# zserge/grayskull

Measured on AMD Instinct MI355X. Metric: Mpix/s (and % HBM roofline) for gs_sobel+gs_blur on 4K uint8, 1/2/4/8 GPU, higher is better.
Workload: dtype u8; 1 GPU; configs[1]: gs_blur(r=2) -> gs_sobel -> gs_otsu_threshold -> gs_threshold, 3840x2160 uint8, 512 frames on this GPU resident in HBM (512 in the job, weak scaling); frames_per_gpu=512, global_frames=512, chain_algorithmic_bytes_per_px_unfused=7

## Files before the change

grayskull_amd/__init__.py:

```python
import ctypes as C
import os

import numpy as np

from ._abi import (BLOB_DTYPE, CONTOUR_DTYPE, GsImage, GsLbpCascade, GsPoint, GsRect, KEYPOINT_DTYPE, MATCH_DTYPE, POINT_DTYPE,
                   RECT_DTYPE)
from .cascade import Cascade

_HERE = os.path.dirname(os.path.abspath(__file__))
HIP_LIBRARY = os.path.join(_HERE, "libgrayskull_hip.so")

__all__ = ["Grayskull", "Cascade", "lib", "BLOB_DTYPE", "CONTOUR_DTYPE", "KEYPOINT_DTYPE", "MATCH_DTYPE", "POINT_DTYPE", "RECT_DTYPE"]


def _ptr(a):
    if a is None:
        return None
    if isinstance(a, np.ndarray):
        if not a.flags["C_CONTIGUOUS"]:
            raise ValueError("array must be C-contiguous")
        return a.ctypes.data
    if hasattr(a, "data_ptr"):
        if not a.is_contiguous():
            raise ValueError("tensor must be contiguous")
        return a.data_ptr()
    if isinstance(a, int):
        return a
    raise TypeError("expected numpy array, torch tensor or raw address, got %r" % type(a))


def _img(a):
    if a.ndim != 2:
        raise ValueError("expected a 2-D (h, w) uint8 image")
    return GsImage(int(a.shape[1]), int(a.shape[0]), _ptr(a))


_SIGS = {
    "gs_blur": (None, [GsImage, GsImage, C.c_uint]),
    "gs_sobel": (None, [GsImage, GsImage]),
    "gs_erode": (None, [GsImage, GsImage]),
    "gs_dilate": (None, [GsImage, GsImage]),
    "gs_histogram": (None, [GsImage, C.c_void_p]),
    "gs_otsu_threshold": (C.c_uint8, [GsImage]),
    "gs_threshold": (None, [GsImage, C.c_uint8]),
    "gs_integral": (None, [GsImage, C.c_void_p]),
    "gs_lbp_window": (C.c_uint, [C.c_void_p, C.c_void_p, C.c_uint, C.c_uint, C.c_int, C.c_int,
                                 C.c_float]),
    "gs_lbp_detect": (C.c_uint, [C.c_void_p, C.c_void_p, C.c_uint, C.c_uint, C.c_void_p, C.c_uint,
                                 C.c_float, C.c_float, C.c_float, C.c_int]),
    "gs_fast": (C.c_uint, [GsImage, GsImage, C.c_void_p, C.c_uint, C.c_uint]),
    "gs_compute_orientation": (C.c_float, [GsImage, C.c_uint, C.c_uint, C.c_uint]),
    "gs_brief_descriptor": (None, [GsImage, C.c_void_p]),
    "gs_orb_extract": (C.c_uint, [GsImage, C.c_void_p, C.c_uint, C.c_uint, C.c_void_p]),
    "gs_match_orb": (C.c_uint, [C.c_void_p, C.c_uint, C.c_void_p, C.c_uint, C.c_void_p, C.c_uint,
                                C.c_float]),
    "gs_compute_orientation_nostdlib": (C.c_float, [GsImage, C.c_uint, C.c_uint, C.c_uint]),
    "gs_brief_descriptor_nostdlib": (None, [GsImage, C.c_void_p]),
    "gs_orb_extract_nostdlib": (C.c_uint, [GsImage, C.c_void_p, C.c_uint, C.c_uint, C.c_void_p]),
    "gs_adaptive_threshold": (None, [GsImage, GsImage, C.c_uint, C.c_int]),
    "gs_filter": (None, [GsImage, GsImage, GsImage, C.c_uint]),
    "gs_downsample": (None, [GsImage, GsImage]),
    "gs_crop": (None, [GsImage, GsImage, GsRect]),
    "gs_copy": (None, [GsImage, GsImage]),
    "gs_resize_nn": (None, [GsImage, GsImage]),
    "gs_resize": (None, [GsImage, GsImage]),
    "gs_match_template": (None, [GsImage, GsImage, GsImage]),
    "gs_find_best_match": (GsPoint, [GsImage]),
    "gs_blobs": (C.c_uint, [GsImage, C.c_void_p, C.c_void_p, C.c_uint]),
    "gs_blob_corners": (None, [GsImage, C.c_void_p, C.c_void_p, C.c_void_p]),
    "gs_trace_contour": (None, [GsImage, GsImage, C.c_void_p]),
    "gs_perspective_correct": (None, [GsImage, GsImage, C.c_void_p]),
    "gsh_version": (C.c_char_p, []),
    "gsh_device_count": (C.c_int, []),
    "gsh_set_device": (None, [C.c_int]),
    "gsh_set_stream": (None, [C.c_void_p]),
    "gsh_get_stream": (C.c_void_p, []),
    "gsh_set_async": (None, [C.c_int]),
    "gsh_sync": (None, []),
    "gsh_tune": (None, [C.c_int, C.c_int]),
    "gsh_profile": (None, [C.c_int]),
    "gsh_profile_read": (C.c_uint, [C.POINTER(C.c_double)]),
    "gsh_fast_score_batch": (None, [C.c_void_p, C.c_void_p, C.c_uint, C.c_uint, C.c_uint, C.c_uint]),
    "gsh_shutdown": (None, []),
    "gsh_malloc": (C.c_void_p, [C.c_size_t]),
    "gsh_free": (None, [C.c_void_p]),
    "gsh_host_alloc": (C.c_void_p, [C.c_size_t]),
    "gsh_host_free": (None, [C.c_void_p]),
    "gsh_memset": (None, [C.c_void_p, C.c_int, C.c_size_t]),
    "gsh_upload": (None, [C.c_void_p, C.c_void_p, C.c_size_t]),
    "gsh_download": (None, [C.c_void_p, C.c_void_p, C.c_size_t]),
    "gsh_is_device_ptr": (C.c_int, [C.c_void_p]),
    "gsh_blur_batch": (None, [C.c_void_p, C.c_void_p, C.c_uint, C.c_uint, C.c_uint, C.c_uint]),
    "gsh_sobel_batch": (None, [C.c_void_p, C.c_void_p, C.c_uint, C.c_uint, C.c_uint]),
    "gsh_erode_batch": (None, [C.c_void_p, C.c_void_p, C.c_uint, C.c_uint, C.c_uint]),
    "gsh_dilate_batch": (None, [C.c_void_p, C.c_void_p, C.c_uint, C.c_uint, C.c_uint]),
    "gsh_morph_batch": (None, [C.c_void_p, C.c_void_p, C.c_void_p, C.c_uint, C.c_uint, C.c_uint, C.c_int, C.c_uint]),
    "gsh_histogram_batch": (None, [C.c_void_p, C.c_uint, C.c_uint, C.c_uint, C.c_void_p]),
    "gsh_otsu_batch": (None, [C.c_void_p, C.c_uint, C.c_uint, C.c_uint, C.c_void_p, C.c_void_p]),
    "gsh_threshold_batch": (None, [C.c_void_p, C.c_uint, C.c_uint, C.c_uint, C.c_uint8]),
    "gsh_threshold_batch_dev": (None, [C.c_void_p, C.c_uint, C.c_uint, C.c_uint, C.c_void_p]),
    "gsh_blur_sobel_batch": (None, [C.c_void_p, C.c_void_p, C.c_uint, C.c_uint, C.c_uint, C.c_uint]),
    "gsh_edge_pipeline_batch": (None, [C.c_void_p, C.c_void_p, C.c_void_p, C.c_uint, C.c_uint,
                                       C.c_uint, C.c_uint, C.c_void_p, C.c_void_p]),
    "gsh_integral_batch": (None, [C.c_void_p, C.c_uint, C.c_uint, C.c_uint, C.c_void_p]),
    "gsh_cascade_create": (C.c_void_p, [C.c_void_p]),
    "gsh_cascade_destroy": (None, [C.c_void_p]),
    "gsh_lbp_detect_batch": (None, [C.c_void_p, C.c_void_p, C.c_uint, C.c_uint, C.c_uint,
                                    C.c_void_p, C.c_void_p, C.c_uint, C.c_float, C.c_float,
                                    C.c_float, C.c_int]),
    "gsh_lbp_count_evaluated": (None, [C.c_void_p]),
    "gsh_lbp_window_count": (C.c_uint64, [C.c_void_p, C.c_uint, C.c_uint, C.c_float, C.c_float,
                                          C.c_float, C.c_int]),
    "gsh_fast_batch": (None, [C.c_void_p, C.c_void_p, C.c_uint, C.c_uint, C.c_uint, C.c_void_p,
                              C.c_void_p, C.c_uint, C.c_uint]),
    "gsh_orb_extract": (C.c_uint, [C.c_void_p, C.c_uint, C.c_uint, C.c_void_p, C.c_void_p,
                                   C.c_uint, C.c_uint]),
    "gsh_orb_extract_batch": (None, [C.c_void_p, C.c_uint, C.c_uint, C.c_uint, C.c_void_p, C.c_void_p, C.c_void_p,
                                     C.c_uint, C.c_uint]),
    "gsh_orb_extract_batch_nostdlib": (None, [C.c_void_p, C.c_uint, C.c_uint, C.c_uint, C.c_void_p, C.c_void_p, C.c_void_p,
                                              C.c_uint, C.c_uint]),
    "gsh_orb_pyramid_buffer_bytes": (C.c_size_t, [C.c_uint, C.c_uint, C.c_uint]),
    "gsh_orb_extract_pyramid": (C.c_uint, [C.c_void_p, C.c_uint, C.c_uint, C.c_void_p, C.c_void_p,
                                           C.c_uint, C.c_uint, C.c_uint]),
    "gsh_match_orb_dev": (None, [C.c_void_p, C.c_uint, C.c_void_p, C.c_uint, C.c_void_p,
                                 C.c_void_p, C.c_uint, C.c_float]),
    "gsh_adaptive_threshold_batch": (None, [C.c_void_p, C.c_void_p, C.c_uint, C.c_uint, C.c_uint,
                                            C.c_uint, C.c_int]),
    "gsh_filter_batch": (None, [C.c_void_p, C.c_void_p, C.c_uint, C.c_uint, C.c_uint, C.c_void_p,
                                C.c_uint, C.c_uint, C.c_uint]),
    "gsh_downsample_batch": (None, [C.c_void_p, C.c_void_p, C.c_uint, C.c_uint, C.c_uint]),
    "gsh_crop_batch": (None, [C.c_void_p, C.c_void_p, C.c_uint, C.c_uint, C.c_uint, GsRect]),
    "gsh_resize_batch": (None, [C.c_void_p, C.c_uint, C.c_uint, C.c_void_p, C.c_uint, C.c_uint, C.c_uint]),
    "gsh_resize_nn_batch": (None, [C.c_void_p, C.c_uint, C.c_uint, C.c_void_p, C.c_uint, C.c_uint, C.c_uint]),
    "gsh_crop_resize_batch": (None, [C.c_void_p, C.c_uint, C.c_uint, C.c_void_p, C.c_uint, C.c_uint, C.c_uint, C.c_void_p,
                                      C.c_void_p, C.c_uint, C.c_int]),
    "gsh_match_template_batch": (None, [C.c_void_p, C.c_uint, C.c_uint, C.c_uint, C.c_void_p, C.c_uint, C.c_uint, C.c_uint,
                                         C.c_void_p]),
    "gsh_find_best_match_batch": (None, [C.c_void_p, C.c_uint, C.c_uint, C.c_uint, C.c_void_p, C.c_void_p]),
    "gsh_locate_template_batch": (None, [C.c_void_p, C.c_uint, C.c_uint, C.c_uint, C.c_void_p, C.c_uint, C.c_uint, C.c_uint,
                                          C.c_void_p, C.c_void_p]),
    "gsh_blobs_batch": (None, [C.c_void_p, C.c_uint, C.c_uint, C.c_uint, C.c_void_p, C.c_void_p, C.c_void_p,
                                C.c_uint]),
    "gsh_blob_corners_batch": (None, [C.c_void_p, C.c_void_p, C.c_uint, C.c_uint, C.c_uint, C.c_void_p,
                                       C.c_void_p]),
    "gsh_perspective_correct_batch": (None, [C.c_void_p, C.c_uint, C.c_uint, C.c_void_p, C.c_uint, C.c_uint,
                                              C.c_uint, C.c_void_p]),
    "gsh_blob_largest_batch": (None, [C.c_void_p, C.c_uint, C.c_void_p, C.c_uint, C.c_void_p, C.c_void_p]),
    "gsh_blob_paint_batch": (None, [C.c_void_p, C.c_void_p, C.c_uint, C.c_uint, C.c_uint, C.c_void_p, C.c_uint,
                                    C.c_void_p]),
    "gsh_threshold_batch_dev_offset": (None, [C.c_void_p, C.c_uint, C.c_uint, C.c_uint, C.c_void_p, C.c_int]),
    "gsh_trace_contours_batch": (None, [C.c_void_p, C.c_void_p, C.c_uint, C.c_uint, C.c_uint, C.c_void_p, C.c_uint,
                                         C.c_void_p, C.c_void_p]),
    "gsh_blob_contour_starts_batch": (None, [C.c_void_p, C.c_uint, C.c_uint, C.c_uint, C.c_void_p, C.c_uint,
                                              C.c_void_p, C.c_void_p]),
    "gsh_synth_batch": (None, [C.c_void_p, C.c_uint, C.c_uint, C.c_uint, C.c_uint32]),
    "gsh_checksum_batch": (None, [C.c_void_p, C.c_size_t, C.c_uint, C.c_void_p]),
    "gsh_comm_init_all": (C.c_int, [C.POINTER(C.c_void_p), C.c_int, C.POINTER(C.c_int)]),
    "gsh_comm_destroy_all": (None, [C.POINTER(C.c_void_p), C.c_int]),
    "gsh_comm_rank": (C.c_int, [C.c_void_p]),
    "gsh_comm_world": (C.c_int, [C.c_void_p]),
    "gsh_comm_backend": (C.c_char_p, [C.c_void_p]),
    "gsh_comm_broadcast": (None, [C.c_void_p, C.c_void_p, C.c_size_t, C.c_int]),
    "gsh_comm_all_gather": (None, [C.c_void_p, C.c_void_p, C.c_void_p, C.c_size_t]),
    "gsh_comm_all_reduce_u64": (None, [C.c_void_p, C.c_void_p, C.c_size_t, C.c_int]),
    "gsh_comm_all_reduce_f64": (None, [C.c_void_p, C.c_void_p, C.c_size_t, C.c_int]),
}
EXPORTED_SYMBOLS = tuple(sorted(_SIGS))
_EXPERIMENT_SIGS = {
    "gsh_probe_strip_copy": (None, [C.c_void_p, C.c_void_p, C.c_uint, C.c_uint, C.c_uint]),
}


def _share_torch_hip_runtime():
    import importlib.util
    import sys
    if "torch" in sys.modules:
        return
    try:
        spec = importlib.util.find_spec("torch")
    except (ImportError, ValueError):
        spec = None
    if not spec or not spec.origin:
        return
    libdir = os.path.join(os.path.dirname(spec.origin), "lib")
    for name in ("libhsa-runtime64.so", "libamdhip64.so"):
        f = os.path.join(libdir, name)
        if os.path.exists(f):
            try:
                C.CDLL(f, mode=C.RTLD_GLOBAL)
            except OSError:
                return


class Grayskull:

    def __init__(self, path=None):
        path = path or HIP_LIBRARY
        if not os.path.exists(path):
            raise ImportError(
                "%s not found: build it with `python -c 'import __graft_entry__ as g; g.build()'` "
                "(hipcc --offload-arch=gfx950). grayskull_amd has no CPU fallback." % path)
        self.path = path
        if os.path.abspath(path) == os.path.abspath(HIP_LIBRARY):
            _share_torch_hip_runtime()
        self.c = C.CDLL(path)
        for name, (res, args) in _SIGS.items():
            f = getattr(self.c, name)
            f.restype, f.argtypes = res, args
        for name, (res, args) in _EXPERIMENT_SIGS.items():
            if hasattr(self.c, name):
                f = getattr(self.c, name)
                f.restype, f.argtypes = res, args

    def version(self):
        return self.c.gsh_version().decode()

    def device_count(self):
        return int(self.c.gsh_device_count())

    def set_device(self, i):
        self.c.gsh_set_device(int(i))

    def use_torch_stream(self):
        import torch
        self.c.gsh_set_stream(C.c_void_p(torch.cuda.current_stream().cuda_stream))

    def set_stream(self, handle):
        self.c.gsh_set_stream(C.c_void_p(handle))

    def set_async(self, on):
        self.c.gsh_set_async(1 if on else 0)

    def shutdown(self):
        self.c.gsh_shutdown()

    def sync(self):
        self.c.gsh_sync()

    def tune(self, key, value):
        self.c.gsh_tune(int(key), int(value))

    def profile(self, on):
        self.c.gsh_profile(int(on))

    def profile_read(self):
        ms = C.c_double(0.0)
        n = self.c.gsh_profile_read(C.byref(ms))
        return int(n), float(ms.value)

    def fast_score_batch(self, score, img, threshold):
        n, h, w = self._nhw(img)
        self.c.gsh_fast_score_batch(_ptr(score), _ptr(img), w, h, n, threshold)

    probe_fast_score = fast_score_batch

    @property
    def experiment(self):
        return hasattr(self.c, "gsh_probe_strip_copy")

    def probe_strip_copy(self, dst, src):
        n, h, w = self._nhw(src)
        self.c.gsh_probe_strip_copy(_ptr(dst), _ptr(src), w, h, n)

    def blur(self, dst, src, radius):
        self.c.gs_blur(_img(dst), _img(src), radius)

    def sobel(self, dst, src):
        self.c.gs_sobel(_img(dst), _img(src))

    def erode(self, dst, src):
        self.c.gs_erode(_img(dst), _img(src))

    def dilate(self, dst, src):
        self.c.gs_dilate(_img(dst), _img(src))

    def histogram(self, img):
        hist = np.zeros(256, np.uint32)
        self.c.gs_histogram(_img(img), hist.ctypes.data)
        return hist

    def otsu_threshold(self, img):
        return int(self.c.gs_otsu_threshold(_img(img)))

    def threshold(self, img, t):
        self.c.gs_threshold(_img(img), t)

    def adaptive_threshold(self, dst, src, radius, c):
        self.c.gs_adaptive_threshold(_img(dst), _img(src), radius, c)

    def filter(self, dst, src, kernel, norm):
        k = np.ascontiguousarray(kernel).astype(np.int8).view(np.uint8)
        self.c.gs_filter(_img(dst), _img(src), _img(k), norm)

    def downsample(self, dst, src):
        self.c.gs_downsample(_img(dst), _img(src))

    def crop(self, dst, src, x, y, w, h):
        self.c.gs_crop(_img(dst), _img(src), GsRect(x, y, w, h))

    def copy(self, dst, src):
        self.c.gs_copy(_img(dst), _img(src))

    def resize(self, dst, src, nearest=False):
        (self.c.gs_resize_nn if nearest else self.c.gs_resize)(_img(dst), _img(src))

    def match_template(self, img, tmpl, result):
        self.c.gs_match_template(_img(img), _img(tmpl), _img(result))

    def find_best_match(self, result):
        p = self.c.gs_find_best_match(_img(result))
        return int(p.x), int(p.y)

    def blobs(self, img, nblobs, labels=None):
        if labels is None:
            labels = np.zeros(img.shape, np.uint16)
        recs = np.zeros(max(nblobs, 1), BLOB_DTYPE)
        m = self.c.gs_blobs(_img(img), _ptr(labels), recs.ctypes.data, nblobs)
        return recs[:m].copy(), labels

    def blob_corners(self, img, labels, blob):
        b = np.ascontiguousarray(np.asarray(blob, BLOB_DTYPE).reshape(1))
        c = np.zeros(4, POINT_DTYPE)
        self.c.gs_blob_corners(_img(img), _ptr(labels), b.ctypes.data, c.ctypes.data)
        return [(int(p["x"]), int(p["y"])) for p in c]

    def perspective_correct(self, dst, src, corners):
        c = np.ascontiguousarray(np.asarray(corners, np.uint32).reshape(4, 2))
        self.c.gs_perspective_correct(_img(dst), _img(src), c.ctypes.data)

    def trace_contour(self, img, visited, start):
        c = np.zeros(1, CONTOUR_DTYPE)
        c["sx"], c["sy"] = int(start[0]) & 0xFFFFFFFF, int(start[1]) & 0xFFFFFFFF
        self.c.gs_trace_contour(_img(img), _img(visited), c.ctypes.data)
        return c[0]

    def integral(self, src, ii=None):
        if ii is None:
            ii = np.zeros(src.shape, np.uint32)
        self.c.gs_integral(_img(src), _ptr(ii))
        return ii

    def lbp_window(self, cascade, ii, x, y, scale):
        ih, iw = ii.shape
        return int(self.c.gs_lbp_window(C.addressof(cascade.as_struct()), _ptr(ii), iw, ih, x, y,
                                        scale))

    def lbp_detect(self, cascade, ii, max_rects, scale_factor, min_scale, max_scale, step):
        ih, iw = ii.shape
        rects = np.zeros(max(max_rects, 1), RECT_DTYPE)
        n = self.c.gs_lbp_detect(C.addressof(cascade.as_struct()), _ptr(ii), iw, ih,
                                 rects.ctypes.data, max_rects, scale_factor, min_scale, max_scale,
                                 step)
        return rects[:n].copy()

    def fast(self, img, scoremap, nkps, threshold):
        kps = np.zeros(max(nkps, 1), KEYPOINT_DTYPE)
        n = self.c.gs_fast(_img(img), _img(scoremap), kps.ctypes.data, nkps, threshold)
        return kps[:n].copy()

    def compute_orientation(self, img, x, y, r=15):
        return float(self.c.gs_compute_orientation(_img(img), x, y, r))

    def brief_descriptor(self, img, x, y, angle):
        kp = np.zeros(1, KEYPOINT_DTYPE)
        kp["x"], kp["y"], kp["angle"] = x, y, angle
        self.c.gs_brief_descriptor(_img(img), kp.ctypes.data)
        return kp["desc"][0].copy()

    def orb_extract(self, img, nkps, threshold, scoremap):
        kps = np.zeros(max(nkps, 1), KEYPOINT_DTYPE)
        n = self.c.gs_orb_extract(_img(img), kps.ctypes.data, nkps, threshold, _ptr(scoremap))
        return kps[:n].copy()

    def compute_orientation_nostdlib(self, img, x, y, r=15):
        return float(self.c.gs_compute_orientation_nostdlib(_img(img), x, y, r))

    def brief_descriptor_nostdlib(self, img, x, y, angle):
        kp = np.zeros(1, KEYPOINT_DTYPE)
        kp["x"], kp["y"], kp["angle"] = x, y, angle
        self.c.gs_brief_descriptor_nostdlib(_img(img), kp.ctypes.data)
        return kp["desc"][0].copy()

    def orb_extract_nostdlib(self, img, nkps, threshold, scoremap):
        kps = np.zeros(max(nkps, 1), KEYPOINT_DTYPE)
        n = self.c.gs_orb_extract_nostdlib(_img(img), kps.ctypes.data, nkps, threshold, _ptr(scoremap))
        return kps[:n].copy()

    def match_orb(self, k1, k2, max_matches, max_distance):
        k1 = np.ascontiguousarray(k1, KEYPOINT_DTYPE)
        k2 = np.ascontiguousarray(k2, KEYPOINT_DTYPE)
        out = np.zeros(max(max_matches, 1), MATCH_DTYPE)
        n = self.c.gs_match_orb(k1.ctypes.data, len(k1), k2.ctypes.data, len(k2), out.ctypes.data,
                                max_matches, max_distance)
        return out[:n].copy()

    @staticmethod
    def _nhw(a):
        if a.ndim != 3:
            raise ValueError("expected (n, h, w)")
        return int(a.shape[0]), int(a.shape[1]), int(a.shape[2])

    def blur_batch(self, dst, src, radius):
        n, h, w = self._nhw(src)
        self.c.gsh_blur_batch(_ptr(dst), _ptr(src), w, h, n, radius)

    def sobel_batch(self, dst, src):
        n, h, w = self._nhw(src)
        self.c.gsh_sobel_batch(_ptr(dst), _ptr(src), w, h, n)

    def erode_batch(self, dst, src):
        n, h, w = self._nhw(src)
        self.c.gsh_erode_batch(_ptr(dst), _ptr(src), w, h, n)

    def dilate_batch(self, dst, src):
        n, h, w = self._nhw(src)
        self.c.gsh_dilate_batch(_ptr(dst), _ptr(src), w, h, n)

    def morph_batch(self, dst, src, iterations, dilate, tmp=None):
        n, h, w = self._nhw(src)
        self.c.gsh_morph_batch(_ptr(dst), _ptr(src), _ptr(tmp), w, h, n, 1 if dilate else 0, int(iterations))

    def histogram_batch(self, img, hist):
        n, h, w = self._nhw(img)
        self.c.gsh_histogram_batch(_ptr(img), w, h, n, _ptr(hist))

    def otsu_batch(self, img, hist_scratch, thr):
        n, h, w = self._nhw(img)
        self.c.gsh_otsu_batch(_ptr(img), w, h, n, _ptr(hist_scratch), _ptr(thr))

    def threshold_batch(self, img, t):
        n, h, w = self._nhw(img)
        if isinstance(t, int):
            self.c.gsh_threshold_batch(_ptr(img), w, h, n, t)
        else:
            self.c.gsh_threshold_batch_dev(_ptr(img), w, h, n, _ptr(t))

    def blur_sobel_batch(self, dst, src, radius):
        n, h, w = self._nhw(src)
        self.c.gsh_blur_sobel_batch(_ptr(dst), _ptr(src), w, h, n, radius)

    def edge_pipeline_batch(self, dst, tmp, src, radius, hist_scratch, thr):
        n, h, w = self._nhw(src)
        self.c.gsh_edge_pipeline_batch(_ptr(dst), _ptr(tmp) if tmp is not None else None, _ptr(src), w, h, n, radius,
                                       _ptr(hist_scratch), _ptr(thr))

    def integral_batch(self, src, ii):
        n, h, w = self._nhw(src)
        self.c.gsh_integral_batch(_ptr(src), w, h, n, _ptr(ii))

    def cascade_create(self, cascade):
        return DeviceCascade(self, cascade)

    def lbp_detect_batch(self, dcascade, ii, rects, counts, max_rects, scale_factor, min_scale,
                         max_scale, step):
        n, h, w = self._nhw(ii)
        self.c.gsh_lbp_detect_batch(dcascade.handle, _ptr(ii), w, h, n, _ptr(rects), _ptr(counts),
                                    max_rects, scale_factor, min_scale, max_scale, step)

    def lbp_count_evaluated(self, counter):
        self.c.gsh_lbp_count_evaluated(_ptr(counter) if counter is not None else None)

    def lbp_window_count(self, cascade, iw, ih, scale_factor, min_scale, max_scale, step):
        return int(self.c.gsh_lbp_window_count(C.addressof(cascade.as_struct()), iw, ih,
                                               scale_factor, min_scale, max_scale, step))

    def fast_batch(self, img, scoremap, kps, counts, nkps, threshold):
        n, h, w = self._nhw(img)
        self.c.gsh_fast_batch(_ptr(img), _ptr(scoremap), w, h, n, _ptr(kps), _ptr(counts), nkps,
                              threshold)

    def orb_extract_dev(self, img, scoremap, nkps, threshold):
        h, w = int(img.shape[0]), int(img.shape[1])
        kps = np.zeros(max(nkps, 1), KEYPOINT_DTYPE)
        n = self.c.gsh_orb_extract(_ptr(img), w, h, _ptr(scoremap), kps.ctypes.data, nkps, threshold)
        return kps[:n].copy()

    def orb_extract_batch_dev(self, imgs, scoremaps, nkps, threshold):
        n, h, w = self._nhw(imgs)
        kps = np.zeros((n, max(nkps, 1)), KEYPOINT_DTYPE)
        counts = np.zeros(n, np.uint32)
        self.c.gsh_orb_extract_batch(_ptr(imgs), w, h, n, _ptr(scoremaps), kps.ctypes.data, counts.ctypes.data, nkps,
                                     threshold)
        return [kps[f, :int(counts[f])].copy() for f in range(n)]

    def orb_pyramid_buffer_bytes(self, w, h, n_levels):
        return int(self.c.gsh_orb_pyramid_buffer_bytes(w, h, n_levels))

    def orb_extract_batch_nostdlib(self, imgs, scoremaps, kps, counts, nkps, threshold):
        n, h, w = self._nhw(imgs)
        self.c.gsh_orb_extract_batch_nostdlib(_ptr(imgs), w, h, n, _ptr(scoremaps), _ptr(kps), _ptr(counts), nkps,
                                              threshold)

    def orb_extract_pyramid_dev(self, img, buffer, nkps, threshold, n_levels):
        h, w = int(img.shape[0]), int(img.shape[1])
        kps = np.zeros(max(nkps, 1), KEYPOINT_DTYPE)
        n = self.c.gsh_orb_extract_pyramid(_ptr(img), w, h, _ptr(buffer), kps.ctypes.data, nkps, threshold,
                                           n_levels)
        return kps[:n].copy()

    def match_orb_dev(self, k1, n1, k2, n2, matches, count, max_matches, max_distance):
        self.c.gsh_match_orb_dev(_ptr(k1), n1, _ptr(k2), n2, _ptr(matches), _ptr(count),
                                 max_matches, max_distance)

    def adaptive_threshold_batch(self, dst, src, radius, c):
        n, h, w = self._nhw(src)
        self.c.gsh_adaptive_threshold_batch(_ptr(dst), _ptr(src), w, h, n, radius, c)

    def filter_batch(self, dst, src, kernel, norm):
        n, h, w = self._nhw(src)
        k = np.ascontiguousarray(kernel).astype(np.int8)
        self.c.gsh_filter_batch(_ptr(dst), _ptr(src), w, h, n, k.ctypes.data, k.shape[1], k.shape[0],
                                norm)

    def downsample_batch(self, dst, src):
        n, h, w = self._nhw(src)
        self.c.gsh_downsample_batch(_ptr(dst), _ptr(src), w, h, n)

    def crop_batch(self, dst, src, x, y, w, h):
        n, sh, sw = self._nhw(src)
        self.c.gsh_crop_batch(_ptr(dst), _ptr(src), sw, sh, n, GsRect(x, y, w, h))

    def resize_batch(self, dst, src, nearest=False):
        n, sh, sw = self._nhw(src)
        _, dh, dw = self._nhw(dst)
        (self.c.gsh_resize_nn_batch if nearest else self.c.gsh_resize_batch)(_ptr(dst), dw, dh, _ptr(src), sw, sh, n)

    def crop_resize_batch(self, dst, src, rois, frame_of=None, nearest=False):
        n, sh, sw = self._nhw(src)
        npatches, dh, dw = self._nhw(dst)
        self.c.gsh_crop_resize_batch(_ptr(dst), dw, dh, _ptr(src), sw, sh, n, _ptr(rois), _ptr(frame_of), npatches,
                                     1 if nearest else 0)

    @staticmethod
    def _templates(tmpl, n):
        if tmpl.ndim == 2:
            return int(tmpl.shape[1]), int(tmpl.shape[0]), 1
        if tmpl.ndim != 3:
            raise ValueError("expected a (th, tw) or an (n, th, tw) uint8 template")
        return int(tmpl.shape[2]), int(tmpl.shape[1]), int(tmpl.shape[0])

    def match_template_batch(self, result, img, tmpl):
        n, ih, iw = self._nhw(img)
        tw, th, ntmpl = self._templates(tmpl, n)
        self.c.gsh_match_template_batch(_ptr(img), iw, ih, n, _ptr(tmpl), tw, th, ntmpl, _ptr(result))

    def find_best_match_batch(self, result, best, score=None):
        n, rh, rw = self._nhw(result)
        self.c.gsh_find_best_match_batch(_ptr(result), rw, rh, n, _ptr(best), _ptr(score))

    def locate_template_batch(self, img, tmpl, best, score=None):
        n, ih, iw = self._nhw(img)
        tw, th, ntmpl = self._templates(tmpl, n)
        self.c.gsh_locate_template_batch(_ptr(img), iw, ih, n, _ptr(tmpl), tw, th, ntmpl, _ptr(best), _ptr(score))

    def blobs_batch(self, img, labels, blobs, counts, nblobs):
        n, h, w = self._nhw(img)
        self.c.gsh_blobs_batch(_ptr(img), w, h, n, _ptr(labels), _ptr(blobs), _ptr(counts), nblobs)

    def blob_corners_batch(self, img, labels, blobs, corners):
        n, h, w = self._nhw(img)
        self.c.gsh_blob_corners_batch(_ptr(img), _ptr(labels), w, h, n, _ptr(blobs), _ptr(corners))

    def perspective_correct_batch(self, dst, src, corners):
        n, sh, sw = self._nhw(src)
        _, dh, dw = self._nhw(dst)
        self.c.gsh_perspective_correct_batch(_ptr(dst), dw, dh, _ptr(src), sw, sh, n, _ptr(corners))

    def blob_largest_batch(self, blobs, counts, largest, index=None):
        self.c.gsh_blob_largest_batch(_ptr(blobs), int(blobs.shape[1]), _ptr(counts), int(blobs.shape[0]), _ptr(largest),
                                      _ptr(index))

    def threshold_batch_dev_offset(self, img, thr, offset):
        n, h, w = self._nhw(img)
        self.c.gsh_threshold_batch_dev_offset(_ptr(img), w, h, n, _ptr(thr), int(offset))

    def blob_paint_batch(self, dst, img, blobs, counts):
        n, h, w = self._nhw(img)
        self.c.gsh_blob_paint_batch(_ptr(dst), _ptr(img), w, h, n, _ptr(blobs), int(blobs.shape[1]), _ptr(counts))

    def trace_contours_batch(self, img, visited, contours, counts=None, status=None):
        n, h, w = self._nhw(img)
        self.c.gsh_trace_contours_batch(_ptr(img), _ptr(visited), w, h, n, _ptr(contours), int(contours.shape[1]),
                                        _ptr(counts), _ptr(status))

    def blob_contour_starts_batch(self, labels, blobs, counts, contours):
        n, h, w = self._nhw(labels)
        self.c.gsh_blob_contour_starts_batch(_ptr(labels), w, h, n, _ptr(blobs), int(blobs.shape[1]), _ptr(counts),
                                             _ptr(contours))

    def synth_batch(self, dst, seed0):
        n, h, w = self._nhw(dst)
        self.c.gsh_synth_batch(_ptr(dst), w, h, n, seed0)

    def checksum_batch(self, img, sums):
        n = int(img.shape[0])
        frame_bytes = int(np.prod(img.shape[1:])) * (img.element_size() if hasattr(img, "element_size") else img.itemsize)
        self.c.gsh_checksum_batch(_ptr(img), frame_bytes, n, _ptr(sums))


class DeviceCascade:

    def __init__(self, gs, cascade):
        self._gs, self._keep = gs, cascade
        self.handle = gs.c.gsh_cascade_create(C.addressof(cascade.as_struct()))

    def close(self):
        if self.handle:
            self._gs.c.gsh_cascade_destroy(self.handle)
            self.handle = None

    def __del__(self):
        try:
            self.close()
        except Exception:
            pass


_default = None


def lib():
    global _default
    if _default is None:
        _default = Grayskull()
    return _default


def __getattr__(name):
    if name.startswith("_"):
        raise AttributeError(name)
    return getattr(lib(), name)
```

grayskull_amd/csrc/gs_fused.cpp:

```cpp
#include "k_fused.h"

#ifndef GS_FUSED_MINW
#define GS_FUSED_MINW 1
#endif

namespace gs {

void launch_blur_sobel_hist(unsigned radius, dim3 grid, dim3 block, hipStream_t st, uint8_t *dst,
                            const uint8_t *src, unsigned w, unsigned h, unsigned T, size_t frame_bytes,
                            unsigned *partial) {
  if (radius == 1) GS_LAUNCH(k_blur_sobel_hist16<1>, grid, block, 0, st, dst, src, w, h, T, frame_bytes, partial);
  else if (radius == 2) GS_LAUNCH(k_blur_sobel_hist16<2>, grid, block, 0, st, dst, src, w, h, T, frame_bytes, partial);
  else GS_LAUNCH(k_blur_sobel_hist16<3>, grid, block, 0, st, dst, src, w, h, T, frame_bytes, partial);
}

void launch_blur_sobel(unsigned radius, dim3 grid, dim3 block, hipStream_t st, uint8_t *dst, const uint8_t *src,
                       unsigned w, unsigned h, unsigned T, size_t frame_bytes, int rg) {
  unsigned *none = nullptr;
  if (rg == 1) {
    if (radius == 1) GS_LAUNCH((k_blur_sobel_hist16<1, false, 1>), grid, block, 0, st, dst, src, w, h, T, frame_bytes, none);
    else if (radius == 2) GS_LAUNCH((k_blur_sobel_hist16<2, false, 1>), grid, block, 0, st, dst, src, w, h, T, frame_bytes, none);
    else GS_LAUNCH((k_blur_sobel_hist16<3, false, 1>), grid, block, 0, st, dst, src, w, h, T, frame_bytes, none);
    return;
  }
  if (rg == 2) {
    if (radius == 1) GS_LAUNCH((k_blur_sobel_hist16<1, false, 2>), grid, block, 0, st, dst, src, w, h, T, frame_bytes, none);
    else if (radius == 2) GS_LAUNCH((k_blur_sobel_hist16<2, false, 2>), grid, block, 0, st, dst, src, w, h, T, frame_bytes, none);
    else GS_LAUNCH((k_blur_sobel_hist16<3, false, 2>), grid, block, 0, st, dst, src, w, h, T, frame_bytes, none);
    return;
  }
  if (radius == 1) GS_LAUNCH((k_blur_sobel_hist16<1, false>), grid, block, 0, st, dst, src, w, h, T, frame_bytes, none);
  else if (radius == 2) GS_LAUNCH((k_blur_sobel_hist16<2, false, 0, GS_FUSED_MINW>), grid, block, 0, st, dst, src, w, h, T, frame_bytes, none);
  else GS_LAUNCH((k_blur_sobel_hist16<3, false>), grid, block, 0, st, dst, src, w, h, T, frame_bytes, none);
}

}
```

grayskull_amd/csrc/gs_internal.h:

```cpp
#ifndef GS_INTERNAL_H
#define GS_INTERNAL_H
#include <math.h>
#include <stdio.h>
#include <stdlib.h>
#include <string.h>

#include <algorithm>
#include <atomic>
#include <condition_variable>
#include <functional>
#include <map>
#include <mutex>
#include <thread>
#include <vector>


#include "../../include/grayskull_hip.h"

#define GS_COMMA ,
#define GS_ASSERT(cond)                                 \
  do {                                                  \
    if (!(cond)) {                                      \
      fprintf(stderr, "Assertion failed: %s\n", #cond); \
      abort();                                          \
    }                                                   \
  } while (0)

#define GS_HIP(call)                                                                   \
  do {                                                                                 \
    hipError_t e_ = (call);                                                            \
    if (e_ != hipSuccess) {                                                            \
      fprintf(stderr, "grayskull_hip: %s failed: %s (%s:%d)\n", #call,                 \
              hipGetErrorString(e_), __FILE__, __LINE__);                              \
      abort();                                                                         \
    }                                                                                  \
  } while (0)

#include "prims.h"
#include "lbp_types.h"
#include "k_strip.h"

namespace gs {
void launch_blur_sobel_hist(unsigned radius, dim3 grid, dim3 block, hipStream_t st, uint8_t *dst,
                            const uint8_t *src, unsigned w, unsigned h, unsigned T, size_t frame_bytes,
                            unsigned *partial);
void launch_blur_sobel(unsigned radius, dim3 grid, dim3 block, hipStream_t st, uint8_t *dst, const uint8_t *src,
                       unsigned w, unsigned h, unsigned T, size_t frame_bytes, int rg);
void launch_box(int mode, unsigned ring_radius, dim3 grid, unsigned threads, hipStream_t st, uint8_t *dst, const uint8_t *src, unsigned w,
                unsigned h, unsigned T, size_t frame_bytes, unsigned r, int c);
void launch_box_edge(int mode, dim3 grid, hipStream_t st, uint8_t *dst, const uint8_t *src, unsigned w, unsigned h, unsigned T,
                     size_t frame_bytes, unsigned r, int c);
unsigned box_blocks_per_cu(int mode, unsigned ring_radius, unsigned threads);
unsigned box_ring_max();
}
using namespace gs;

namespace gsi {

enum Slot { SL_IN = 0, SL_OUT, SL_AUX, SL_AUX2, SL_II, SL_PAD, SL_MASK, SL_CNT, SL_PFX, SL_TOT, SL_PRE,
            SL_HISTP, SL_HIST, SL_THR, SL_KPS, SL_MOM, SL_KIN, SL_DESC, SL_TAB, SL_JUMP, SL_LEV,
            SL_BEST, SL_NZ,
            SL_BLOB_BITS, SL_BLOB_PAR, SL_BLOB_STAT, SL_BLOB_ROW, SL_BLOB_LAB, SL_BLOB_REC, SL_COUNT };

constexpr unsigned kChunkFrames = 32, kMaxChunks = 256;
struct LbpGeomCache {
  unsigned iw = 0, ih = 0;
  float sf = 0, mn = 0, mx = 0;
  int step = 0;
  std::vector<LbpScale> scales;
  LbpScale *d_scales = nullptr;
  LbpGeom *d_geom = nullptr;
  size_t d_scales_cap = 0, d_geom_cap = 0;
  unsigned total_chunks = 0, max_chunks = 0;
  bool guard = false;
  unsigned long long nwindows = 0;
};
struct gsh_cascade_tables_deleter { void operator()(struct ::gsh_cascade *dc) const; };
#ifndef GS_EMU
#ifndef GS_EVENT_FLAGS
#define GS_EVENT_FLAGS hipEventDisableSystemFence
#endif
inline unsigned sync_event_flags() { return GS_EVENT_FLAGS; }
#ifndef GS_ORDER_EVENT_FLAGS
#define GS_ORDER_EVENT_FLAGS 0
#endif
inline unsigned order_event_flags() { return hipEventDisableTiming | GS_ORDER_EVENT_FLAGS; }
#endif
struct Topo {
  unsigned cus = 256, xcds = 8;
  unsigned simds() const { return cus * 4u; }
  bool eight_xcds() const { return xcds == 8u; }
};
struct Ctx {
  int device = 0;
  bool device_set = false;
  Topo topo;
  hipStream_t stream = nullptr;
  bool own_stream = false, user_stream = false, async = false;
  struct Buf { void *p = nullptr; size_t cap = 0; } slot[SL_COUNT];
  enum { PIN_A = 0, PIN_B, PIN_C, PIN_D, PIN_COUNT };
  Buf pin[PIN_COUNT];
  void *pinned(int i, size_t bytes) {
    ensure_device();
    Buf &b = pin[i];
    if (b.cap < bytes) {
      if (b.p) {
        sync();
        GS_HIP(hipHostFree(b.p));
      }
      const size_t cap = bytes + bytes / 4 + 256;
      GS_HIP(hipHostMalloc(&b.p, cap, 0));
      b.cap = cap;
    }
    return b.p;
  }
  bool jump_ready = false;
  bool lbp_lds_raised = false;
  std::map<unsigned long long, LbpGeomCache> geom_cache;
  struct ::gsh_cascade *dropin_cascade = nullptr;
  uint64_t dropin_cascade_hash = 0;
  void drop_geom() {
    for (auto &kv : geom_cache) {
      if (kv.second.d_scales) (void)hipFree(kv.second.d_scales);
      if (kv.second.d_geom) (void)hipFree(kv.second.d_geom);
    }
    geom_cache.clear();
  }
  ~Ctx() { release(); }
#ifndef GS_EMU
  static constexpr int kProfPairs = 4096;
  bool prof_on = false;
  hipEvent_t prof_ev[2 * kProfPairs] = {};
  unsigned prof_n = 0;
  void prof_mark(int which, hipStream_t on) {
    if (!prof_on || prof_n >= (unsigned)kProfPairs) return;
    hipEvent_t &e = prof_ev[2 * prof_n + which];
    if (!e) GS_HIP(hipEventCreateWithFlags(&e, sync_event_flags()));
    GS_HIP(hipEventRecord(e, on));
    if (which) prof_n++;
  }
  hipStream_t side = nullptr;
  hipEvent_t ev_join = nullptr, ev_chunk[kMaxChunks] = {};
  hipEvent_t ev_switch = nullptr;
  void ensure_side() {
    if (side) return;
    {
      int lo = 0, hi = 0, mine = 0;
      GS_HIP(hipDeviceGetStreamPriorityRange(&lo, &hi));
      if (hipStreamGetPriority(s(), &mine) != hipSuccess) mine = 0;
      GS_HIP(hipStreamCreateWithPriority(&side, hipStreamNonBlocking, mine == lo && lo != hi ? hi : lo));
    }
    GS_HIP(hipEventCreateWithFlags(&ev_join, order_event_flags()));
    for (auto &e : ev_chunk) GS_HIP(hipEventCreateWithFlags(&e, order_event_flags()));
  }
#endif

  void ensure_device() {
    if (device_set) return;
    int n = 0;
#ifndef GS_EMU
    hipError_t e = hipGetDeviceCount(&n);
    if (e != hipSuccess || n <= 0) {
      fprintf(stderr, "grayskull_hip: no HIP device visible (%s); there is no CPU fallback\n",
              e == hipSuccess ? "device count 0" : hipGetErrorString(e));
      abort();
    }
#endif
    GS_HIP(hipSetDevice(device));
    device_set = true;
#ifndef GS_EMU
    int v = 0;
    if (hipDeviceGetAttribute(&v, hipDeviceAttributeMultiprocessorCount, device) == hipSuccess && v > 0) topo.cus = (unsigned)v;
    if (hipDeviceGetAttribute(&v, hipDeviceAttributeNumberOfXccs, device) == hipSuccess && v > 0) topo.xcds = (unsigned)v;
    else (void)hipGetLastError();
#endif
  }
  hipStream_t s() {
    ensure_device();
    if (user_stream) return stream;
    if (!own_stream) {
      GS_HIP(hipStreamCreate(&stream));
      own_stream = true;
    }
    return stream;
  }
  void sync() { GS_HIP(hipStreamSynchronize(s())); }
  void *scratch(int i, size_t bytes) {
    ensure_device();
    Buf &b = slot[i];
    if (b.cap < bytes) {
      if (b.p) {
        sync();
        GS_HIP(hipFree(b.p));
      }
      size_t cap = bytes + bytes / 4 + 256;
      GS_HIP(hipMalloc(&b.p, cap));
      b.cap = cap;
    }
    return b.p;
  }
  void release() {
    for (auto &b : slot) {
      if (b.p) (void)hipFree(b.p);
      b.p = nullptr, b.cap = 0;
    }
    for (auto &b : pin) {
      if (b.p) (void)hipHostFree(b.p);
      b.p = nullptr, b.cap = 0;
    }
    jump_ready = false;
    lbp_lds_raised = false;
    drop_geom();
    if (dropin_cascade) gsh_cascade_tables_deleter()(dropin_cascade);
    dropin_cascade = nullptr;
#ifndef GS_EMU
    for (auto &e : prof_ev) {
      if (e) (void)hipEventDestroy(e);
      e = nullptr;
    }
    prof_n = 0;
    if (ev_switch) (void)hipEventDestroy(ev_switch);
    ev_switch = nullptr;
    if (side) {
      (void)hipStreamDestroy(side), (void)hipEventDestroy(ev_join);
      for (auto &e : ev_chunk) (void)hipEventDestroy(e), e = nullptr;
      side = nullptr, ev_join = nullptr;
    }
#endif
    if (own_stream) (void)hipStreamDestroy(stream);
    own_stream = false;
    if (!user_stream) stream = nullptr;
  }
};
Ctx &ctx();

#ifdef GS_EMU
extern "C" void emu_device_pointers(int on);
extern "C" int emu_device_pointers_on(void);
#endif
inline bool is_dev(const void *p) {
#ifdef GS_EMU
  return p && emu_device_pointers_on();
#else
  if (!p) return false;
  ctx().ensure_device();
  hipPointerAttribute_t a;
  hipError_t e = hipPointerGetAttributes(&a, p);
  if (e != hipSuccess) {
    (void)hipGetLastError();
    return false;
  }
  return a.type == hipMemoryTypeDevice || a.type == hipMemoryTypeManaged;
#endif
}

inline const void *stage_in(const void *p, size_t bytes, int slot) {
  if (is_dev(p)) return p;
  void *d = ctx().scratch(slot, bytes);
  GS_HIP(hipMemcpyAsync(d, p, bytes, hipMemcpyHostToDevice, ctx().s()));
  return d;
}
inline void finish(bool any_host_output) {
  if (any_host_output || !ctx().async) ctx().sync();
}
inline dim3 grid2d(unsigned w, unsigned h, unsigned n) { return dim3((w + 63) / 64, (h + 3) / 4, n); }
inline bool al16(const void *p) { return ((uintptr_t)p & 15) == 0; }

struct TuneTable {
  std::atomic<int> v[32];
  TuneTable() {
    for (auto &e : v) e.store(0, std::memory_order_relaxed);
  }
  int operator[](int k) const { return v[k].load(std::memory_order_relaxed); }
  void set(int k, int x) { v[k].store(x, std::memory_order_relaxed); }
};
extern TuneTable g_tune;
inline const Topo &topo() {
  ctx().ensure_device();
  return ctx().topo;
}
extern thread_local unsigned long long *g_lbp_evaluated;

struct StripCfg {
  dim3 grid, block;
  unsigned T;
  size_t xcd_flag = 0;
};
StripCfg strip_cfg(unsigned w, unsigned rows, unsigned n, unsigned waves_per_simd = 5, unsigned halo_rows = 2,
                   unsigned short_T = 8, int rg = -1);
inline bool strip_ok(unsigned w, unsigned h) {
  return w >= 32 && (unsigned long long)w * h < 0x7fff0000ull;
}
inline bool ragged(unsigned w) { return (w & 15u) != 0u; }
inline int strip_mode(unsigned w, const void *src) {
  const int direct = ragged(w) ? 1 : 0;
  if ((w & 3u) == 0u && ((uintptr_t)src & 3u) == 0u) return direct;
  const unsigned strips = (w + 15) / 16;
  const unsigned lanes2 = strips + strip_realign_shift(w) + strip_realign_helper(w), lanes1 = strips + (direct ? strip_ragged_shift(w) : 0u);
  if ((lanes2 + 63) / 64 > (lanes1 + 63) / 64) return direct;
  return 2;
}
inline bool strip_ok16(unsigned w, unsigned h, const void *a, const void *b) {
  return w % 16 == 0 && (unsigned long long)w * h < 0x7fffffffull && al16(a) && al16(b);
}
inline unsigned max_frames_per_launch() { return g_tune[8] > 0 ? (unsigned)g_tune[8] : 32768u; }
#define kMaxZ (max_frames_per_launch())

#define GS_VALID(i) ((i).data && (i).w > 0 && (i).h > 0)

void launch_sobel(uint8_t *dst, const uint8_t *src, unsigned w, unsigned h, unsigned n, bool keep_cols = true);
void launch_blur(uint8_t *dst, const uint8_t *src, unsigned w, unsigned h, unsigned n, unsigned radius);
bool launch_integral(const uint8_t *src, unsigned w, unsigned h, unsigned n, unsigned *ii, bool sq = false);
void launch_integral_pad(dim3 grid, hipStream_t st, const unsigned *ii, unsigned w, unsigned h, unsigned *padded);

}
using namespace gs;
using namespace gsi;
#endif
```

grayskull_amd/csrc/gs_stencil.cpp:

```cpp
#include "gs_internal.h"

#include "k_geom.h"
#include "k_integral.h"
#include "k_pointwise.h"
#include "k_resize.h"
#include "k_stencil.h"
#include "k_tmatch.h"

namespace gsi {

StripCfg strip_cfg(unsigned w, unsigned rows, unsigned n, unsigned waves_per_simd, unsigned halo_rows, unsigned short_T, int rg) {
  StripCfg c;
  const unsigned strips = (w + 15) / 16 + (rg == 2 ? strip_realign_shift(w) + strip_realign_helper(w) : rg == 1 ? strip_ragged_shift(w) : (w & 15u) ? 1u : 0u);
  const unsigned long long waves_x = (strips + 63) / 64;
  unsigned long long t;
  if (g_tune[0] > 0) {
    t = (unsigned long long)g_tune[0];
  } else if (waves_per_simd >= 5) {
    t = std::max(short_T, 2u * halo_rows);
  } else {
    const unsigned long long cap = (unsigned long long)topo().simds() * waves_per_simd, wn = waves_x * n;
    const unsigned long long nb_max = rows / 8 ? rows / 8 : 1;
    unsigned long long nb = cap / wn;
    if (nb < 1) nb = 1;
// ... 341 lines not shown
    x ^= x >> 17;
    x ^= x << 5;
    return x;
  };
  for (int b = 0; b < 32; b++) J.col[0][b] = step(1u << b);
  for (int k = 1; k < 32; k++)
    for (int b = 0; b < 32; b++) {
      uint32_t v = J.col[k - 1][b], r = 0;
      for (int q = 0; q < 32; q++)
        if ((v >> q) & 1u) r ^= J.col[k - 1][q];
      J.col[k][b] = r;
    }
}

void launch_integral_pad(dim3 grid, hipStream_t st, const unsigned *ii, unsigned w, unsigned h, unsigned *padded) {
  GS_LAUNCH(k_integral_pad, grid, dim3(64, 4), 0, st, ii, w, h, padded);
}

constexpr unsigned kResizeLdsSmall = 16u * 1024u, kResizeLdsMax = 48u * 1024u;
static unsigned resize_extent(unsigned c, unsigned s, unsigned d) {
  return (unsigned)std::min<unsigned long long>(s, ((unsigned long long)c * s + d - 1) / d + 3);
}
struct ResizePlan { unsigned band, lds; };
static ResizePlan resize_plan(unsigned dw, unsigned dh, unsigned sw, unsigned sh, bool windows) {
  ResizePlan pl = {16u, 0u};
  const bool dense = (unsigned long long)sw * sh <= 4ull * dw * dh || g_tune[25] == 2;
  if (g_tune[25] != 1 && (windows || dense)) {
    if (windows) {
      pl.lds = kResizeLdsSmall;
    } else {
      const unsigned pitch = (resize_extent(std::min(dw, 256u), sw, dw) + 3u) & ~3u;
      for (unsigned band = 16; band >= 4 && !pl.lds; band >>= 1) {
        const unsigned long long need = (unsigned long long)pitch * resize_extent(std::min(band, dh), sh, dh);
        if (need <= (band > 4 ? kResizeLdsSmall : kResizeLdsMax)) pl.band = band, pl.lds = (unsigned)need;
      }
    }
  }
  if ((dh + pl.band - 1) / pl.band > 65535u) pl.band = (((dh + 65534u) / 65535u) + 3u) & ~3u;
  return pl;
}
static void launch_resize(uint8_t *dst, unsigned dw, unsigned dh, const uint8_t *src, unsigned sw, unsigned sh, unsigned n,
                          const unsigned *rois, const unsigned *frame_of, unsigned count, bool nearest) {
  const ResizePlan pl = resize_plan(dw, dh, sw, sh, rois != nullptr);
  ResizeArgs a;
  a.dst = dst, a.src = src, a.rois = rois, a.frame_of = frame_of;
  a.dw = dw, a.dh = dh, a.sw = sw, a.sh = sh, a.n = n;
  a.band = pl.band, a.lds = pl.lds, a.any_density = g_tune[25] == 2 ? 1u : 0u;
  const bool nt = (unsigned long long)dw * dh * count > (256ull << 20);
  hipStream_t st = ctx().s();
  for (unsigned f0 = 0; f0 < count; f0 += kMaxZ) {
    const dim3 grid((dw + 255) / 256, (dh + pl.band - 1) / pl.band, std::min(kMaxZ, count - f0));
    a.z0 = f0;
    if (nearest && nt) GS_LAUNCH((k_resize_tile<true, true>), grid, dim3(64, 4), pl.lds, st, a);
    else if (nearest) GS_LAUNCH((k_resize_tile<true, false>), grid, dim3(64, 4), pl.lds, st, a);
    else if (nt) GS_LAUNCH((k_resize_tile<false, true>), grid, dim3(64, 4), pl.lds, st, a);
    else GS_LAUNCH((k_resize_tile<false, false>), grid, dim3(64, 4), pl.lds, st, a);
  }
}
static void launch_crop(uint8_t *dst, const uint8_t *src, unsigned sw, unsigned sh, unsigned n, struct gs_rect roi) {
  GS_ASSERT(roi.x <= sw && roi.w <= sw - roi.x && roi.y <= sh && roi.h <= sh - roi.y);
  const size_t sfb = (size_t)sw * sh, dfb = (size_t)roi.w * roi.h;
  const bool nt = (unsigned long long)dfb * n > (256ull << 20);
  hipStream_t st = ctx().s();
  for (unsigned f0 = 0; f0 < n; f0 += kMaxZ) {
    const dim3 grid(((roi.w + 15) / 16 + 63) / 64, (roi.h + 3) / 4, std::min(kMaxZ, n - f0));
    if (nt) GS_LAUNCH(k_crop_rows<true>, grid, dim3(64, 4), 0, st, dst + dfb * f0, src + sfb * f0, sw, sh, roi.x, roi.y, roi.w, roi.h);
    else GS_LAUNCH(k_crop_rows<false>, grid, dim3(64, 4), 0, st, dst + dfb * f0, src + sfb * f0, sw, sh, roi.x, roi.y, roi.w, roi.h);
  }
}
static bool apart(const uint8_t *a, size_t na, const uint8_t *b, size_t nb) { return a + na <= b || b + nb <= a; }

struct TmForm {
  bool split, band;
  unsigned istride;
  size_t lds;
};
static TmForm tm_form(unsigned tw, unsigned th, unsigned rw, unsigned rh, unsigned frames) {
  TmForm f;
  const unsigned nkc = (tw + 31 + 31) / 32;
  f.split = g_tune[20] == 3 || (g_tune[20] != 2 && g_tune[20] != 8 && (unsigned long long)((rw + 127) / 128) * ((rh + 63) / 64) * frames < 512);
  f.istride = (f.split ? 32 : 96) + 32 * nkc + 16;
  f.band = !f.split && g_tune[20] != 2 && th > kTmBand;
  const unsigned rows = f.band ? kTmBand : th;
  f.lds = std::max<size_t>((size_t)((f.split ? 31 : 63) + rows) * f.istride + (size_t)rows * (32 * nkc + 48) + 16, f.split ? 32768 : 0);
  return f;
}
enum TmRoute { TM_MFMA, TM_DOT, TM_PX };
static TmRoute tm_route(unsigned iw, unsigned ih, unsigned tw, unsigned th) {
  const size_t ib = (size_t)iw * ih, tb = (size_t)tw * th;
  const unsigned nkc = (tw + 31 + 31) / 32;
  const TmForm one = tm_form(tw, th, iw - tw + 1, ih - th + 1, 1);
  if (g_tune[20] != 1 && tw >= 16 && nkc <= 9 && th >= 4 && (tb >= 512 || g_tune[20] == 2 || g_tune[20] == 3 || g_tune[20] == 8) && tb <= 32768 &&
      one.lds <= 150 * 1024 && ib < 0x7fffffffull)
    return TM_MFMA;
  return tw <= kTmplTile - 3 ? TM_DOT : TM_PX;
}
constexpr size_t kTmScratchBudget = (size_t)128 << 20;
static unsigned tm_chunk_frames(TmRoute route, unsigned iw, unsigned ih, unsigned rw, unsigned rh, unsigned n, bool locate) {
  const size_t per = route == TM_MFMA ? ((size_t)ih * (iw + 1) + (size_t)rw * rh) * 4 : locate ? (size_t)rw * rh : 0;
  size_t c = std::min<size_t>(n, kMaxZ);
  if (per) c = std::min(c, std::max<size_t>(1, kTmScratchBudget / per));
  if (g_tune[26] > 0) c = std::min<size_t>(c, (size_t)g_tune[26]);
  return (unsigned)c;
}
static void tm_launch(const uint8_t *s, unsigned iw, unsigned ih, unsigned nn, const uint8_t *t, unsigned tw, unsigned th, unsigned ntmpl,
                      uint8_t *d, unsigned long long *keys) {
  const unsigned rw = iw - tw + 1, rh = ih - th + 1;
  const size_t ib = (size_t)iw * ih, tb = (size_t)tw * th, rb = (size_t)rw * rh;
  const TmRoute route = tm_route(iw, ih, tw, th);
  hipStream_t st = ctx().s();
  if (route == TM_MFMA) {
    TmForm f = tm_form(tw, th, rw, rh, nn);
    if (f.lds > 150 * 1024) f = tm_form(tw, th, rw, rh, 1);
    const bool tm_split = f.split, tm_band = f.band;
    const unsigned nkc = (tw + 31 + 31) / 32, istride = f.istride, tstride = 32 * nkc + 48;
    const size_t tm_lds = f.lds, tpb = (size_t)th * tstride;
    unsigned *rowp = (unsigned *)ctx().scratch(SL_II, (size_t)nn * ih * (iw + 1) * 4);
    unsigned *s2 = (unsigned *)ctx().scratch(SL_PAD, (size_t)nn * rb * 4);
    uint8_t *tpad = (uint8_t *)ctx().scratch(SL_PRE, ntmpl * tpb + (size_t)ntmpl * 4 + 16);
    unsigned *tsqp = (unsigned *)(tpad + ((ntmpl * tpb + 3) & ~(size_t)3));
    GS_LAUNCH(k_tm_prep, dim3(ntmpl), dim3(1024), 0, st, t, tw, th, tstride, tpad, tsqp);
    if (g_tune[20] != 4 && (ib >= (4u << 20) || g_tune[20] == 5) && launch_integral(s, iw, ih, nn, rowp, true)) {
      GS_LAUNCH(k_tm_s2_corners, dim3((rw + 255) / 256, rh, nn), dim3(256), 0, st, (const unsigned *)rowp, iw, ih, tw, th, rw, rh, s2);
    } else {
      GS_LAUNCH(k_tm_rowprefix, dim3((ih + 3) / 4, 1, nn), dim3(64, 4), 0, st, s, iw, ih, rowp);
      GS_LAUNCH(k_tm_colsq, dim3((rw + 63) / 64, (rh + kTmRun - 1) / kTmRun, nn), dim3(64), 0, st, (const unsigned *)rowp, iw, ih, tw, th,
                rw, rh, s2);
    }
#ifndef GS_EMU
    static std::atomic<unsigned long long> lds_raised{0};
    const unsigned long long dev_bit = 1ull << ((unsigned)ctx().device & 63u);
    if (ctx().device >= 64 || !(lds_raised.load(std::memory_order_acquire) & dev_bit)) {
#define GS_TM_FNS(S) (const void *)k_match_template_mfma<S, 2>, (const void *)k_match_template_mfma<S, 3>, (const void *)k_match_template_mfma<S, 4>, \
                     (const void *)k_match_template_mfma<S, 5>, (const void *)k_match_template_mfma<S, 6>, (const void *)k_match_template_mfma<S, 7>, \
                     (const void *)k_match_template_mfma<S, 8>, (const void *)k_match_template_mfma<S, 9>
      const void *fns[] = {GS_TM_FNS(1), GS_TM_FNS(4),
                           (const void *)k_match_template_mfma<1, 2, true>, (const void *)k_match_template_mfma<1, 3, true>, (const void *)k_match_template_mfma<1, 4, true>,
                           (const void *)k_match_template_mfma<1, 5, true>, (const void *)k_match_template_mfma<1, 6, true>, (const void *)k_match_template_mfma<1, 7, true>,
                           (const void *)k_match_template_mfma<1, 8, true>, (const void *)k_match_template_mfma<1, 9, true>};
#undef GS_TM_FNS
      for (const void *fn : fns) GS_HIP(hipFuncSetAttribute(fn, hipFuncAttributeMaxDynamicSharedMemorySize, 160 * 1024));
      lds_raised.fetch_or(dev_bit, std::memory_order_release);
    }
#endif
    TmArgs ta{s, iw, ih, (const uint8_t *)tpad, (const unsigned *)tsqp, tw, th, s2, d, rw, rh, nkc, istride, tstride,
              ntmpl > 1 ? (unsigned)tpb : 0u, ntmpl > 1 ? 1u : 0u, keys};
    const dim3 gs4((rw + 63) / 64, (rh + 31) / 32, nn), gs1((rw + 127) / 128, (rh + 63) / 64, nn);
    GS_ASSERT(nkc >= 2 && nkc <= 9);
    switch (nkc * 4 + (tm_split ? 1u : tm_band ? 2u : 0u)) {
#define GS_TM_CASE(K)                                                                                   \
  case K * 4: GS_LAUNCH((k_match_template_mfma<1, K>), gs1, dim3(256), tm_lds, st, ta); break;          \
  case K * 4 + 1: GS_LAUNCH((k_match_template_mfma<4, K>), gs4, dim3(256), tm_lds, st, ta); break;      \
  case K * 4 + 2: GS_LAUNCH((k_match_template_mfma<1, K, true>), gs1, dim3(256), tm_lds, st, ta); break;
      GS_TM_CASE(2) GS_TM_CASE(3) GS_TM_CASE(4) GS_TM_CASE(5) GS_TM_CASE(6) GS_TM_CASE(7) GS_TM_CASE(8) GS_TM_CASE(9)
#undef GS_TM_CASE
    }
    return;
  }
  GS_ASSERT(d != nullptr);
  const dim3 g((rw + 63) / 64, (rh + 3) / 4, nn);
  const unsigned tstep = ntmpl > 1 ? (unsigned)tb : 0u;
  if (route == TM_DOT) {
    unsigned long long *tsq = (unsigned long long *)ctx().scratch(SL_PFX, (size_t)ntmpl * 8);
    GS_LAUNCH(k_sum_squares, dim3(ntmpl), dim3(256), 0, st, t, (unsigned long long)tb, tsq);
    const size_t twp = ((size_t)tw + 3) & ~(size_t)3;
    const size_t lds = std::min<size_t>(twp * th, (kTmplTile / twp) * twp);
    if (iw % 4 == 0 && ((uintptr_t)s & 3) == 0 && ib < 0x7fffffffull)
      GS_LAUNCH(k_match_template4, dim3((rw + 255) / 256, (rh + 3) / 4, nn), dim3(64, 4), lds, st, s, iw, ih, t, tw, th, tstep,
                (const unsigned long long *)tsq, d, rw, rh);
    else
      GS_LAUNCH(k_match_template, g, dim3(64, 4), lds, st, s, iw, ih, t, tw, th, tstep, (const unsigned long long *)tsq, d, rw, rh);
  } else {
    GS_LAUNCH(k_match_template_px, g, dim3(64, 4), 0, st, s, iw, ih, t, tw, th, tstep, d, rw, rh);
  }
}
static void tm_argmax(const uint8_t *maps, unsigned rw, unsigned rh, unsigned n, unsigned long long *keys) {
  const unsigned long long rb = (unsigned long long)rw * rh;
  for (unsigned f0 = 0; f0 < n; f0 += kMaxZ) {
    const unsigned nn = std::min(kMaxZ, n - f0);
    GS_LAUNCH(k_argmax_first, dim3((unsigned)((rb + 2047) / 2048), nn), dim3(256), 0, ctx().s(), maps + (size_t)rb * f0, rb,
              (unsigned long long *)nullptr, keys + f0);
  }
}
static void tm_batch(const uint8_t *img, unsigned iw, unsigned ih, unsigned n, const uint8_t *tmpl, unsigned tw, unsigned th, unsigned ntmpl,
                     uint8_t *result, struct gs_point *best, uint8_t *score) {
  if (n == 0) return;
  GS_ASSERT(img && iw > 0 && ih > 0 && tmpl && tw > 0 && th > 0 && (result || best));
  GS_ASSERT(iw >= tw && ih >= th);
  GS_ASSERT(ntmpl == 1 || ntmpl == n);
  const unsigned rw = iw - tw + 1, rh = ih - th + 1;
  const size_t ib = (size_t)iw * ih, tb = (size_t)tw * th, rb = (size_t)rw * rh;
  const TmRoute route = tm_route(iw, ih, tw, th);
  const unsigned chunk = tm_chunk_frames(route, iw, ih, rw, rh, n, result == nullptr);
  hipStream_t st = ctx().s();
  unsigned long long *keys = nullptr;
  if (!result) {
    keys = (unsigned long long *)ctx().scratch(SL_BEST, (size_t)n * 8);
    GS_HIP(hipMemsetAsync(keys, 0, (size_t)n * 8, st));
  }
  for (unsigned f0 = 0; f0 < n; f0 += chunk) {
    const unsigned nn = std::min(chunk, n - f0);
    const uint8_t *s = img + ib * f0, *t = ntmpl > 1 ? tmpl + tb * f0 : tmpl;
    const unsigned nt = ntmpl > 1 ? nn : 1u;
    if (result) tm_launch(s, iw, ih, nn, t, tw, th, nt, result + rb * f0, nullptr);
    else if (route == TM_MFMA) tm_launch(s, iw, ih, nn, t, tw, th, nt, nullptr, keys + f0);
    else {
      uint8_t *maps = (uint8_t *)ctx().scratch(SL_OUT, (size_t)nn * rb);
      tm_launch(s, iw, ih, nn, t, tw, th, nt, maps, nullptr);
      tm_argmax(maps, rw, rh, nn, keys + f0);
    }
  }
  if (!result) GS_LAUNCH(k_best_from_keys, dim3((n + 255) / 256), dim3(256), 0, st, (const unsigned long long *)keys, n, rw, (unsigned *)best, score);
}

}

extern "C" {

#ifdef GS_EXPERIMENT
void gsh_probe_strip_copy(uint8_t *dst, const uint8_t *src, unsigned w, unsigned h, unsigned n) {
  GS_ASSERT(dst && src && w >= 32);
  const StripCfg c = strip_cfg(w, h, n, 5, 2, g_tune[0] > 0 ? (unsigned)g_tune[0] : 8u, ragged(w) ? 1 : 0);
  if (g_tune[23] == 1) GS_LAUNCH((k_strip_copy<0, true>), c.grid, c.block, 0, ctx().s(), dst, src, w, h, c.T, (size_t)w * h | c.xcd_flag);
  else if (ragged(w)) GS_LAUNCH(k_strip_copy<1>, c.grid, c.block, 0, ctx().s(), dst, src, w, h, c.T, (size_t)w * h | c.xcd_flag);
  else GS_LAUNCH(k_strip_copy<0>, c.grid, c.block, 0, ctx().s(), dst, src, w, h, c.T, (size_t)w * h | c.xcd_flag);
}
#endif
void gsh_blur_batch(uint8_t *dst, const uint8_t *src, unsigned w, unsigned h, unsigned n,
                    unsigned radius) {
  GS_ASSERT(dst && src && w > 0 && h > 0);
  launch_blur(dst, src, w, h, n, radius);
}
void gsh_sobel_batch(uint8_t *dst, const uint8_t *src, unsigned w, unsigned h, unsigned n) {
  GS_ASSERT(dst && src && w > 0 && h > 0);
  launch_sobel(dst, src, w, h, n);
}
void gsh_erode_batch(uint8_t *dst, const uint8_t *src, unsigned w, unsigned h, unsigned n) {
  GS_ASSERT(dst && src && w > 0 && h > 0);
  launch_morph<false>(dst, src, w, h, n);
}
void gsh_dilate_batch(uint8_t *dst, const uint8_t *src, unsigned w, unsigned h, unsigned n) {
  GS_ASSERT(dst && src && w > 0 && h > 0);
  launch_morph<true>(dst, src, w, h, n);
}
void gsh_morph_batch(uint8_t *dst, const uint8_t *src, uint8_t *tmp, unsigned w, unsigned h, unsigned n, int dilate,
                     unsigned iterations) {
  GS_ASSERT(dst && src && w > 0 && h > 0);
  GS_ASSERT(iterations >= 1);
  if (n == 0) return;
  const size_t nb = (size_t)w * h * n;
  GS_ASSERT(dst + nb <= src || src + nb <= dst);
  if (tmp && iterations > 4) {
    GS_ASSERT(tmp + nb <= dst || dst + nb <= tmp);
    GS_ASSERT(tmp + nb <= src || src + nb <= tmp);
  }
  if (dilate) launch_morph_iter<true>(dst, src, tmp, w, h, n, iterations);
  else launch_morph_iter<false>(dst, src, tmp, w, h, n, iterations);
}

void gsh_histogram_batch(const uint8_t *img, unsigned w, unsigned h, unsigned n, unsigned *hist) {
  GS_ASSERT(img && hist && w > 0 && h > 0);
  launch_histogram(img, (size_t)(w * h), n, hist);
}
void gsh_otsu_batch(const uint8_t *img, unsigned w, unsigned h, unsigned n, unsigned *hist_scratch,
                    uint8_t *thr) {
  GS_ASSERT(img && hist_scratch && thr && w > 0 && h > 0);
  launch_otsu(img, w, h, n, hist_scratch, thr);
}
void gsh_threshold_batch(uint8_t *img, unsigned w, unsigned h, unsigned n, uint8_t thresh) {
  GS_ASSERT(img && w > 0 && h > 0);
  launch_threshold(img, (size_t)(w * h), n, nullptr, thresh);
}
void gsh_threshold_batch_dev(uint8_t *img, unsigned w, unsigned h, unsigned n, const uint8_t *thr) {
  GS_ASSERT(img && thr && w > 0 && h > 0);
  launch_threshold(img, (size_t)(w * h), n, thr, 0);
}
void gsh_threshold_batch_dev_offset(uint8_t *img, unsigned w, unsigned h, unsigned n, const uint8_t *thr, int offset) {
  GS_ASSERT(img && thr && w > 0 && h > 0);
  launch_threshold(img, (size_t)(w * h), n, thr, 0, nullptr, offset);
}
void gsh_blur_sobel_batch(uint8_t *dst, const uint8_t *src, unsigned w, unsigned h, unsigned n,
                          unsigned radius) {
  GS_ASSERT(dst && src && w > 0 && h > 0);
  if (n == 0) return;
  const size_t fb = (size_t)w * h;
  hipStream_t st = ctx().s();
  if (radius >= 1 && radius <= 3 && strip_ok(w, h) && h >= 3 &&
      h > 2 * radius) {
    for (unsigned f0 = 0; f0 < n; f0 += kMaxZ) {
      const unsigned nn = std::min(kMaxZ, n - f0);
      const int rg = strip_mode(w, src + fb * f0);
      const StripCfg c = strip_cfg(w, h - 2, nn, 3, 2, 8, rg);
      launch_blur_sobel(radius, dim3(c.grid.x, c.grid.y, nn), c.block, st, dst + fb * f0, src + fb * f0, w, h,
                        c.T, fb, rg);
      GS_LAUNCH(k_zero_frame, dim3((2 * w + 2 * h + 255) / 256, nn), dim3(256), 0, st, dst + fb * f0, w, h, fb);
    }
    return;
  }
  uint8_t *t = (uint8_t *)ctx().scratch(SL_AUX, fb * n);
  launch_blur(t, src, w, h, n, radius);
  GS_HIP(hipMemsetAsync(dst, 0, fb * n, st));
  if (w >= 3 && h >= 3) launch_sobel(dst, t, w, h, n, true);
}
void gsh_edge_pipeline_batch(uint8_t *dst, uint8_t *tmp, const uint8_t *src, unsigned w, unsigned h,
                             unsigned n, unsigned radius, unsigned *hist_scratch, uint8_t *thr) {
  GS_ASSERT(dst && src && hist_scratch && thr && w > 0 && h > 0);
  const size_t fb = (size_t)w * h;
  hipStream_t st = ctx().s();
  auto zero_frame = [&]() {
    for (unsigned f0 = 0; f0 < n; f0 += kMaxZ)
      GS_LAUNCH(k_zero_frame, dim3((2 * w + 2 * h + 255) / 256, std::min(kMaxZ, n - f0)), dim3(256), 0,
                st, dst + fb * f0, w, h, fb);
  };
  if (!tmp && radius >= 1 && radius <= 3 && strip_ok16(w, h, dst, src) && w >= 32 &&
      h >= 3 && h > 2 * radius) {
    const int tune_chunk = g_tune[5];
    const unsigned per = tune_chunk < 0 ? n : tune_chunk > 0 ? (unsigned)tune_chunk : kChunkFrames;
    std::vector<unsigned> sizes;
    for (unsigned rem = n; rem; rem -= std::min(rem, per)) sizes.push_back(std::min(rem, per));
    auto cfg_for = [&](unsigned nn) { return strip_cfg(w, h - 2, std::min(kMaxZ, nn), 3);  };
    unsigned bpf_max = 0;
    for (unsigned nn : sizes) {
      const StripCfg c = cfg_for(nn);
      bpf_max = std::max(bpf_max, c.grid.x * c.grid.y);
    }
    unsigned *partial = (unsigned *)ctx().scratch(SL_HISTP, (size_t)n * bpf_max * 256 * 4);
    auto run_fused = [&](hipStream_t on, unsigned f0, unsigned nn) {
      const StripCfg c = cfg_for(nn);
      for (unsigned g0 = f0; g0 < f0 + nn; g0 += kMaxZ) {
        const unsigned m = std::min(kMaxZ, f0 + nn - g0);
        const dim3 grid(c.grid.x, c.grid.y, m);
        uint8_t *d = dst + fb * g0;
        const uint8_t *sp = src + fb * g0;
        unsigned *pp = partial + (size_t)g0 * bpf_max * 256;
#ifndef GS_EMU
        ctx().prof_mark(0, on);
#endif
        launch_blur_sobel_hist(radius, grid, c.block, on, d, sp, w, h, c.T, fb, pp);
#ifndef GS_EMU
        ctx().prof_mark(1, on);
#endif
      }
    };
    auto run_rest = [&](hipStream_t on, unsigned f0, unsigned nn) {
      const StripCfg c = cfg_for(nn);
      const unsigned bpf = c.grid.x * c.grid.y;
      for (unsigned g0 = f0; g0 < f0 + nn; g0 += kMaxZ) {
        const unsigned m = std::min(kMaxZ, f0 + nn - g0);
        const unsigned *pp = partial + (size_t)g0 * bpf_max * 256;
        GS_LAUNCH(k_otsu, dim3(m), dim3(256), 0, on, hist_scratch + (size_t)g0 * 256, w * h, thr + g0, pp, bpf,
                  2 * w + 2 * (h - 2));
      }
      launch_threshold(dst + fb * f0, fb, nn, thr + f0, 0, on);
      for (unsigned g0 = f0; g0 < f0 + nn; g0 += kMaxZ) {
        const unsigned m = std::min(kMaxZ, f0 + nn - g0);
        GS_LAUNCH(k_zero_frame, dim3((2 * w + 2 * h + 255) / 256, m), dim3(256), 0, on, dst + fb * g0, w, h, fb);
      }
    };
#ifdef GS_EMU
    const bool split = false;
#else
    const bool split = sizes.size() > 1 && sizes.size() <= kMaxChunks;
#endif
    if (!split) {
      run_fused(st, 0, n);
      run_rest(st, 0, n);
      return;
    }
#ifndef GS_EMU
    Ctx &cx = ctx();
    cx.ensure_side();
    unsigned f0 = 0;
    for (size_t i = 0; i < sizes.size(); i++) {
      const unsigned nn = sizes[i];
      run_fused(st, f0, nn);
      if (i + 1 == sizes.size()) {
        GS_HIP(hipEventRecord(cx.ev_join, cx.side));
        GS_HIP(hipStreamWaitEvent(st, cx.ev_join, 0));
        run_rest(st, f0, nn);
      } else {
        GS_HIP(hipEventRecord(cx.ev_chunk[i], st));
        GS_HIP(hipStreamWaitEvent(cx.side, cx.ev_chunk[i], 0));
        run_rest(cx.side, f0, nn);
      }
      f0 += nn;
    }
#endif
    return;
  }
  if (!tmp && radius >= 1 && radius <= 3 && strip_ok(w, h) && h >= 3 &&
      h > 2 * radius) {
    gsh_blur_sobel_batch(dst, src, w, h, n, radius);
    launch_otsu(dst, w, h, n, hist_scratch, thr);
    launch_threshold(dst, fb, n, thr, 0);
    return;
  }
  uint8_t *t = tmp ? tmp : (uint8_t *)ctx().scratch(SL_AUX, fb * n);
  launch_blur(t, src, w, h, n, radius);
  if (w < 3 || h < 3) GS_HIP(hipMemsetAsync(dst, 0, fb * n, st));
  launch_sobel(dst, t, w, h, n, false);
  if (w >= 3 && h >= 3) zero_frame();
  launch_otsu(dst, w, h, n, hist_scratch, thr);
  launch_threshold(dst, fb, n, thr, 0);
}

void gsh_integral_batch(const uint8_t *src, unsigned w, unsigned h, unsigned n, unsigned *ii) {
  GS_ASSERT(src && ii && w > 0 && h > 0);
  launch_integral(src, w, h, n, ii);
}

void gsh_adaptive_threshold_batch(uint8_t *dst, const uint8_t *src, unsigned w, unsigned h,
                                  unsigned n, unsigned radius, int c) {
  GS_ASSERT(dst && src && w > 0 && h > 0);
  if (n) launch_box_generic<1>(dst, src, w, h, n, radius, c);
}
void gsh_filter_batch(uint8_t *dst, const uint8_t *src, unsigned w, unsigned h, unsigned n,
                      const int8_t *kernel_host, unsigned kw, unsigned kh, unsigned norm) {
  GS_ASSERT(dst && src && kernel_host && w > 0 && h > 0 && kw > 0 && kh > 0 && norm > 0);
  hipStream_t st = ctx().s();
  int8_t *dk = (int8_t *)ctx().scratch(SL_TAB, (size_t)kw * kh);
  GS_HIP(hipMemcpyAsync(dk, kernel_host, (size_t)kw * kh, hipMemcpyHostToDevice, st));
  ctx().sync();
  const size_t fb = (size_t)w * h;
  unsigned abs_sum = 0;
  for (unsigned i = 0; i < kw * kh; i++) abs_sum += (unsigned)std::abs((int)kernel_host[i]);
  if (kw == 3 && kh == 3 && abs_sum <= 128 && norm <= 256 && strip_ok(w, h)) {
    FilterK fk;
    for (int r = 0; r < 3; r++)
      for (int c = 0; c < 3; c++) fk.k[r][c] = ((uint32_t)(uint16_t)(int16_t)kernel_host[r * 3 + c]) * 0x10001u;
    fk.mul = (0x1000000u + norm - 1u) / norm;
    fk.cap = std::min(255u * norm, 32767u) * 0x10001u;
    fk.neg_is_255 = norm > 1 ? 0xffffffffu : 0u;
    for (unsigned f0 = 0; f0 < n; f0 += kMaxZ) {
      const unsigned nn = std::min(kMaxZ, n - f0);
      const int rg = strip_mode(w, src + fb * f0);
      const StripCfg c = strip_cfg(w, h, nn, 6, 2, 8, rg);
      uint8_t *d = dst + fb * f0;
      const uint8_t *s = src + fb * f0;
      const size_t fa = fb | c.xcd_flag;
      if (norm == 1) {
        if (rg == 1) GS_LAUNCH((k_filter16<1, true>), c.grid, c.block, 0, st, d, s, w, h, c.T, fa, fk);
        else if (rg == 2) GS_LAUNCH((k_filter16<2, true>), c.grid, c.block, 0, st, d, s, w, h, c.T, fa, fk);
        else GS_LAUNCH((k_filter16<0, true>), c.grid, c.block, 0, st, d, s, w, h, c.T, fa, fk);
      } else if (rg == 1) GS_LAUNCH(k_filter16<1>, c.grid, c.block, 0, st, d, s, w, h, c.T, fa, fk);
      else if (rg == 2) GS_LAUNCH(k_filter16<2>, c.grid, c.block, 0, st, d, s, w, h, c.T, fa, fk);
      else GS_LAUNCH(k_filter16<0>, c.grid, c.block, 0, st, d, s, w, h, c.T, fa, fk);
    }
    return;
  }
  for (unsigned f0 = 0; f0 < n; f0 += kMaxZ) {
    const unsigned nn = std::min(kMaxZ, n - f0);
    GS_LAUNCH(k_filter_px, grid2d(w, h, nn), dim3(64, 4), 0, st, dst + fb * f0, src + fb * f0, w, h,
              fb, (const int8_t *)dk, kw, kh, norm);
  }
}
void gsh_downsample_batch(uint8_t *dst, const uint8_t *src, unsigned sw, unsigned sh, unsigned n) {
  GS_ASSERT(dst && src && sw > 1 && sh > 1);
  hipStream_t st = ctx().s();
  const size_t sfb = (size_t)sw * sh, dfb = (size_t)(sw / 2) * (sh / 2);
  for (unsigned f0 = 0; f0 < n; f0 += kMaxZ) {
    const unsigned nn = std::min(kMaxZ, n - f0);
    if (sw >= 16)
      GS_LAUNCH(k_downsample8, dim3(((sw / 2 + 7) / 8 + 63) / 64, (sh / 2 + 3) / 4, nn), dim3(64, 4), 0, st,
                dst + dfb * f0, src + sfb * f0, sw, sh);
    else
      GS_LAUNCH(k_downsample_px, grid2d(sw / 2, sh / 2, nn), dim3(64, 4), 0, st, dst + dfb * f0,
                src + sfb * f0, sw, sh);
  }
}

void gsh_crop_batch(uint8_t *dst, const uint8_t *src, unsigned sw, unsigned sh, unsigned n, struct gs_rect roi) {
  if (n == 0) return;
  GS_ASSERT(dst && src && sw > 0 && sh > 0 && roi.w > 0 && roi.h > 0);
  GS_ASSERT(roi.x <= sw && roi.w <= sw - roi.x && roi.y <= sh && roi.h <= sh - roi.y);
  GS_ASSERT(apart(dst, (size_t)roi.w * roi.h * n, src, (size_t)sw * sh * n));
  launch_crop(dst, src, sw, sh, n, roi);
}
static void resize_batch(uint8_t *dst, unsigned dw, unsigned dh, const uint8_t *src, unsigned sw, unsigned sh, unsigned n,
                         bool nearest) {
  if (n == 0) return;
  GS_ASSERT(dst && src && dw > 0 && dh > 0 && sw > 0 && sh > 0);
  GS_ASSERT(apart(dst, (size_t)dw * dh * n, src, (size_t)sw * sh * n));
  launch_resize(dst, dw, dh, src, sw, sh, n, nullptr, nullptr, n, nearest);
}
void gsh_resize_batch(uint8_t *dst, unsigned dw, unsigned dh, const uint8_t *src, unsigned sw, unsigned sh, unsigned n) {
  resize_batch(dst, dw, dh, src, sw, sh, n, false);
}
void gsh_resize_nn_batch(uint8_t *dst, unsigned dw, unsigned dh, const uint8_t *src, unsigned sw, unsigned sh, unsigned n) {
  resize_batch(dst, dw, dh, src, sw, sh, n, true);
}
void gsh_crop_resize_batch(uint8_t *dst, unsigned dw, unsigned dh, const uint8_t *src, unsigned sw, unsigned sh, unsigned n,
                           const struct gs_rect *rois_dev, const unsigned *frame_of_dev, unsigned npatches, int nearest) {
  if (n == 0 || npatches == 0) return;
  GS_ASSERT(dst && src && rois_dev && dw > 0 && dh > 0 && sw > 0 && sh > 0);
  GS_ASSERT(apart(dst, (size_t)dw * dh * npatches, src, (size_t)sw * sh * n));
  launch_resize(dst, dw, dh, src, sw, sh, n, (const unsigned *)rois_dev, frame_of_dev, npatches, nearest != 0);
}

void gsh_match_template_batch(const uint8_t *img, unsigned iw, unsigned ih, unsigned n, const uint8_t *tmpl, unsigned tw, unsigned th,
                              unsigned ntmpl, uint8_t *result) {
  if (n == 0) return;
  GS_ASSERT(result != NULL);
  tm_batch(img, iw, ih, n, tmpl, tw, th, ntmpl, result, nullptr, nullptr);
}
void gsh_find_best_match_batch(const uint8_t *result, unsigned rw, unsigned rh, unsigned n, struct gs_point *best, uint8_t *score) {
  if (n == 0) return;
  GS_ASSERT(result && rw > 0 && rh > 0 && best);
  hipStream_t st = ctx().s();
  unsigned long long *keys = (unsigned long long *)ctx().scratch(SL_BEST, (size_t)n * 8);
  GS_HIP(hipMemsetAsync(keys, 0, (size_t)n * 8, st));
  tm_argmax(result, rw, rh, n, keys);
  GS_LAUNCH(k_best_from_keys, dim3((n + 255) / 256), dim3(256), 0, st, (const unsigned long long *)keys, n, rw, (unsigned *)best, score);
}
void gsh_locate_template_batch(const uint8_t *img, unsigned iw, unsigned ih, unsigned n, const uint8_t *tmpl, unsigned tw, unsigned th,
                               unsigned ntmpl, struct gs_point *best, uint8_t *score) {
  if (n == 0) return;
  GS_ASSERT(best != NULL);
  tm_batch(img, iw, ih, n, tmpl, tw, th, ntmpl, nullptr, best, score);
}


void gsh_synth_batch(uint8_t *dst, unsigned w, unsigned h, unsigned n, uint32_t seed0) {
  GS_ASSERT(dst && w > 0 && h > 0);
  if (!n) return;
  hipStream_t st = ctx().s();
  bool &jump_ready = ctx().jump_ready;
  SynthJump *dj = (SynthJump *)ctx().scratch(SL_JUMP, sizeof(SynthJump));
  if (!jump_ready) {
    SynthJump J;
    synth_jump_table(J);
    GS_HIP(hipMemcpyAsync(dj, &J, sizeof J, hipMemcpyHostToDevice, st));
    ctx().sync();
    jump_ready = true;
  }
  const unsigned nlev = ((w + 31) / 32) * ((h + 31) / 32);
  const size_t npx = (size_t)w * h;
  for (unsigned f0 = 0; f0 < n; f0 += kMaxZ) {
    const unsigned nn = std::min(kMaxZ, n - f0);
    uint8_t *lev = (uint8_t *)ctx().scratch(SL_LEV, (size_t)nlev * nn);
    const unsigned per = 256 * kSynthRun;
    GS_LAUNCH(k_synth_levels, dim3((nlev + per - 1) / per, nn), dim3(256), 0, st, lev, nlev,
              seed0 + f0, (const SynthJump *)dj);
    GS_LAUNCH(k_synth_pixels, dim3((unsigned)((npx + per - 1) / per), nn), dim3(256), 0, st,
              dst + npx * f0, (const uint8_t *)lev, w, h, seed0 + f0, (const SynthJump *)dj);
  }
}
void gsh_checksum_batch(const uint8_t *img, size_t frame_bytes, unsigned n, uint64_t *sums) {
  GS_ASSERT(img && sums && frame_bytes > 0);
  if (!n) return;
  hipStream_t st = ctx().s();
  GS_HIP(hipMemsetAsync(sums, 0, (size_t)n * 8, st));
  const unsigned bx = (unsigned)std::max<size_t>(1, std::min<size_t>((frame_bytes + 4095) / 4096, 256));
  for (unsigned f0 = 0; f0 < n; f0 += kMaxZ) {
    const unsigned nn = std::min(kMaxZ, n - f0);
    GS_LAUNCH(k_checksum, dim3(bx, nn), dim3(256), 0, st, img + frame_bytes * f0, frame_bytes,
              (unsigned long long *)sums + f0);
  }
}


static void unary_full(struct gs_image dst, struct gs_image src,
                       void (*run)(uint8_t *, const uint8_t *, unsigned, unsigned, unsigned,
                                   unsigned, int),
                       unsigned p0, int p1) {
  const size_t nb = (size_t)src.w * src.h;
  const uint8_t *s = (const uint8_t *)stage_in(src.data, nb, SL_IN);
  const bool dhost = !is_dev(dst.data);
  uint8_t *d = dhost ? (uint8_t *)ctx().scratch(SL_OUT, nb) : dst.data;
  run(d, s, src.w, src.h, 1, p0, p1);
  if (dhost) GS_HIP(hipMemcpyAsync(dst.data, d, nb, hipMemcpyDeviceToHost, ctx().s()));
  finish(dhost);
}

void gs_blur(struct gs_image dst, struct gs_image src, unsigned radius) {
  GS_ASSERT(GS_VALID(src) && GS_VALID(dst) && dst.w == src.w && dst.h == src.h);
  unary_full(dst, src, [](uint8_t *d, const uint8_t *s, unsigned w, unsigned h, unsigned n,
                          unsigned r, int) { launch_blur(d, s, w, h, n, r); }, radius, 0);
}
void gs_erode(struct gs_image dst, struct gs_image src) {
  GS_ASSERT(GS_VALID(dst) && GS_VALID(src) && dst.w == src.w && dst.h == src.h);
  unary_full(dst, src, [](uint8_t *d, const uint8_t *s, unsigned w, unsigned h, unsigned n,
                          unsigned, int) { launch_morph<false>(d, s, w, h, n); }, 0, 0);
}
void gs_dilate(struct gs_image dst, struct gs_image src) {
  GS_ASSERT(GS_VALID(dst) && GS_VALID(src) && dst.w == src.w && dst.h == src.h);
  unary_full(dst, src, [](uint8_t *d, const uint8_t *s, unsigned w, unsigned h, unsigned n,
                          unsigned, int) { launch_morph<true>(d, s, w, h, n); }, 0, 0);
}
void gs_adaptive_threshold(struct gs_image dst, struct gs_image src, unsigned radius, int c) {
  GS_ASSERT(GS_VALID(dst) && GS_VALID(src) && dst.w == src.w && dst.h == src.h);
  unary_full(dst, src, [](uint8_t *d, const uint8_t *s, unsigned w, unsigned h, unsigned n,
                          unsigned r, int cc) { launch_box_generic<1>(d, s, w, h, n, r, cc); },
             radius, c);
}

void gs_sobel(struct gs_image dst, struct gs_image src) {
  GS_ASSERT(GS_VALID(dst) && GS_VALID(src) && dst.w == src.w && dst.h == src.h);
  const unsigned w = src.w, h = src.h;
  if (w < 3 || h < 3) return;
  const size_t nb = (size_t)w * h;
  const uint8_t *s = (const uint8_t *)stage_in(src.data, nb, SL_IN);
  const bool dhost = !is_dev(dst.data);
  uint8_t *d = dhost ? (uint8_t *)ctx().scratch(SL_OUT, nb) : dst.data;
  if (dhost) {
    std::vector<uint8_t> cols(2 * (size_t)h);
    for (unsigned y = 1; y + 1 < h; y++) cols[2 * y] = dst.data[(size_t)y * w], cols[2 * y + 1] = dst.data[(size_t)y * w + w - 1];
    uint8_t *dc = (uint8_t *)ctx().scratch(SL_AUX2, 2 * (size_t)h);
    GS_HIP(hipMemcpyAsync(dc, cols.data(), 2 * (size_t)h, hipMemcpyHostToDevice, ctx().s()));
    GS_LAUNCH(k_put_cols, dim3((2 * h + 255) / 256), dim3(256), 0, ctx().s(), d, (const uint8_t *)dc, w, h);
    ctx().sync();
  }
  launch_sobel(d, s, w, h, 1, true);
  if (dhost)
    GS_HIP(hipMemcpyAsync(dst.data + w, d + w, (size_t)w * (h - 2), hipMemcpyDeviceToHost, ctx().s()));
  finish(dhost);
}

void gs_filter(struct gs_image dst, struct gs_image src, struct gs_image kernel, unsigned norm) {
  GS_ASSERT(GS_VALID(src) && GS_VALID(dst) && dst.w == src.w && dst.h == src.h && norm > 0);
  const size_t nb = (size_t)src.w * src.h, kb = (size_t)kernel.w * kernel.h;
  std::vector<int8_t> k(std::max<size_t>(1, kb), 0);
  unsigned kw = kernel.w, kh = kernel.h;
  if (GS_VALID(kernel)) {
    if (is_dev(kernel.data)) gsh_download(k.data(), kernel.data, kb);
    else memcpy(k.data(), kernel.data, kb);
  } else {
    kw = kh = 1;
    k[0] = 0;
  }
  const uint8_t *s = (const uint8_t *)stage_in(src.data, nb, SL_IN);
  const bool dhost = !is_dev(dst.data);
  uint8_t *d = dhost ? (uint8_t *)ctx().scratch(SL_OUT, nb) : dst.data;
  gsh_filter_batch(d, s, src.w, src.h, 1, k.data(), kw, kh, norm);
  if (dhost) GS_HIP(hipMemcpyAsync(dst.data, d, nb, hipMemcpyDeviceToHost, ctx().s()));
  finish(dhost);
}

void gs_downsample(struct gs_image dst, struct gs_image src) {
  GS_ASSERT(GS_VALID(src) && GS_VALID(dst) && dst.w == src.w / 2 && dst.h == src.h / 2);
  const size_t nb = (size_t)src.w * src.h, db = (size_t)dst.w * dst.h;
  const uint8_t *s = (const uint8_t *)stage_in(src.data, nb, SL_IN);
  const bool dhost = !is_dev(dst.data);
  uint8_t *d = dhost ? (uint8_t *)ctx().scratch(SL_OUT, db) : dst.data;
  gsh_downsample_batch(d, s, src.w, src.h, 1);
  if (dhost) GS_HIP(hipMemcpyAsync(dst.data, d, db, hipMemcpyDeviceToHost, ctx().s()));
  finish(dhost);
}

void gs_crop(struct gs_image dst, struct gs_image src, struct gs_rect roi) {
  GS_ASSERT(GS_VALID(dst) && GS_VALID(src) && roi.x + roi.w <= src.w && roi.y + roi.h <= src.h &&
            dst.w == roi.w && dst.h == roi.h);
  const size_t nb = (size_t)src.w * src.h, db = (size_t)dst.w * dst.h;
  const uint8_t *s = (const uint8_t *)stage_in(src.data, nb, SL_IN);
  const bool dhost = !is_dev(dst.data);
  uint8_t *d = dhost ? (uint8_t *)ctx().scratch(SL_OUT, db) : dst.data;
  if (roi.x <= src.w && roi.w <= src.w - roi.x && roi.y <= src.h && roi.h <= src.h - roi.y)
    launch_crop(d, s, src.w, src.h, 1, roi);
  else
    GS_LAUNCH(k_crop_wrapped, dim3((roi.w + 63) / 64, (roi.h + 3) / 4), dim3(64, 4), 0, ctx().s(), d, s, src.w, src.h, roi.x,
              roi.y, roi.w, roi.h);
  if (dhost) GS_HIP(hipMemcpyAsync(dst.data, d, db, hipMemcpyDeviceToHost, ctx().s()));
  finish(dhost);
}
void gs_copy(struct gs_image dst, struct gs_image src) {
  const struct gs_rect all = {0, 0, src.w, src.h};
  gs_crop(dst, src, all);
}
static void resize_common(struct gs_image dst, struct gs_image src, bool nearest) {
  const size_t nb = (size_t)src.w * src.h, db = (size_t)dst.w * dst.h;
  const uint8_t *s = (const uint8_t *)stage_in(src.data, nb, SL_IN);
  const bool dhost = !is_dev(dst.data);
  uint8_t *d = dhost ? (uint8_t *)ctx().scratch(SL_OUT, db) : dst.data;
  launch_resize(d, dst.w, dst.h, s, src.w, src.h, 1, nullptr, nullptr, 1, nearest);
  if (dhost) GS_HIP(hipMemcpyAsync(dst.data, d, db, hipMemcpyDeviceToHost, ctx().s()));
  finish(dhost);
}
void gs_resize_nn(struct gs_image dst, struct gs_image src) {
  GS_ASSERT(GS_VALID(dst) && GS_VALID(src));
  resize_common(dst, src, true);
}
void gs_resize(struct gs_image dst, struct gs_image src) {
  GS_ASSERT(GS_VALID(dst) && GS_VALID(src));
  resize_common(dst, src, false);
}
void gs_match_template(struct gs_image img, struct gs_image tmpl, struct gs_image result) {
  GS_ASSERT(GS_VALID(img) && GS_VALID(tmpl) && GS_VALID(result));
// ... 79 lines not shown
```

grayskull_amd/csrc/k_fused.h:

```cpp
#ifndef GS_K_FUSED_H
#define GS_K_FUSED_H
#include "k_strip.h"

namespace gs {

constexpr uint32_t blur_k24(unsigned cx, unsigned cy) { return (0x1000000u + cx * cy - 1u) / (cx * cy); }

template <int R, unsigned CX>
GS_DEV uint32_t blur_mul_for_rows(unsigned cy) {
  uint32_t m = blur_k24(CX, 2 * R + 1);
#pragma unroll
  for (unsigned c = R + 1; c < 2 * R + 1; c++) m = cy == c ? blur_k24(CX, c) : m;
  return m;
}

template <int R>
GS_DEV void blur_hsum10(const uint32_t (&U)[12], uint32_t (&H)[10]) {
  uint32_t A[13];
  if constexpr (R >= 3) A[0] = alignbit(U[0], 0u, 16), A[12] = alignbit(0u, U[11], 16);
#pragma unroll
  for (int j = 0; j <= 10; j++) A[j + 1] = alignbit(U[j + 1], U[j], 16);
  if constexpr (R == 1) {
#pragma unroll
    for (int k = 0; k < 10; k++) H[k] = add2(A[k + 1], U[k + 1], A[k + 2]);
  } else {
    uint32_t Q[11];
#pragma unroll
    for (int j = 0; j <= 10; j++) Q[j] = add2(U[j], A[j + 1]);
#pragma unroll
    for (int k = 0; k < 10; k++) {
      const int j = k + 1;
      uint32_t t = add2(Q[j - 1], Q[j], U[j + 1]);
      if constexpr (R >= 3) t = add2(t, A[j - 1], A[j + 2]);
      H[k] = t;
    }
  }
}

#ifndef GS_FUSED_SPARE
#define GS_FUSED_SPARE(hist) true
#endif
#ifndef GS_FUSED_VGPR_ATTR
#define GS_FUSED_VGPR_ATTR
#endif
template <int R, bool HIST = true, int RG = 0, int MINW = 1>
__global__ __launch_bounds__(256, MINW) GS_FUSED_VGPR_ATTR void k_blur_sobel_hist16(uint8_t *dst, const uint8_t *src,
                                                           unsigned w, unsigned h, unsigned T,
                                                           size_t frame_bytes, unsigned *partial) {
  constexpr bool RAGGED = RG != 0;
  static_assert(!(HIST && RAGGED), "ragged rows take the histogram as a separate pass");
  constexpr int N = 2 * R + 1;
  __shared__ unsigned lh[HIST ? 256 * 32 : 1];
  const unsigned tid = threadIdx.y * blockDim.x + threadIdx.x, copy = tid & 31u;
  if constexpr (HIST) {
    for (unsigned i = tid; i < 256 * 32; i += 256) lh[i] = 0;
    __syncthreads();
  }
  const Strip<false, RG> S(src, dst, w, h, frame_bytes);
  const int y0 = 1 + (int)(S.band * T);
  if (y0 < (int)h - 1 && !S.wave_outside()) {
    const int nrows = ((int)h - 1 - y0) < (int)T ? ((int)h - 1 - y0) : (int)T;
    const bool first = S.x0 == 0, last = S.x0 + 16 == w, inimg = S.in_image();
    bool edge[R + 2][R];
    if constexpr (RAGGED) {
      static_for<R + 2>([&](auto Q) {
        constexpr int q = decltype(Q)::value;
        const int d = (int)w - 1 - (int)(S.x0 + 16 - R + q);
        static_for<R>([&](auto I) { edge[q][decltype(I)::value] = inimg && d == decltype(I)::value; });
      });
    }
    constexpr bool SPARE = R <= 2 && GS_FUSED_SPARE(HIST);
    constexpr int NS = SPARE ? N + 1 : N, P0 = SPARE ? 1 : 0;
    uint32_t ring[NS][10], V[10];
    SobelState st;
    auto blurred = [&](int b, uint32_t(&UB)[12]) {
      const int ya = b - R < 0 ? 0 : b - R, yb = b + R > (int)h - 1 ? (int)h - 1 : b + R;
      const unsigned cy = (unsigned)(yb - ya + 1);
      const uint32_t mC = blur_mul_for_rows<R, N>(cy);
      uint32_t mL[R], mR[R + 2];
      static_for<R>([&](auto Q) {
        constexpr int q = decltype(Q)::value;
        mL[q] = first ? blur_mul_for_rows<R, R + 1 + q>(cy) : mC;
        mR[q] = last ? blur_mul_for_rows<R, 2 * R - q>(cy) : mC;
      });
      mR[R] = mR[R + 1] = mC;
      if constexpr (RAGGED) {
        static_for<R + 2>([&](auto Q) {
          constexpr int q = decltype(Q)::value;
          uint32_t m = mC;
          static_for<R>([&](auto I) { m = edge[q][decltype(I)::value] ? blur_mul_for_rows<R, R + 1 + decltype(I)::value>(cy) : m; });
          mR[q] = m;
        });
      }
      UB[0] = 0, UB[11] = 0;
#pragma unroll
      for (int k = 0; k < 10; k++) {
        uint32_t pr[2];
#pragma unroll
        for (int hlf = 0; hlf < 2; hlf++) {
          const int q = 2 * k - 2 + hlf;
          const uint32_t sv = hlf ? (V[k] >> 16) : (V[k] & 0xffffu);
          constexpr int qr = RAGGED ? 18 : 16;
          const uint32_t m = (q >= 0 && q < R) ? mL[(q >= 0 && q < R) ? q : 0]
                             : (q >= 16 - R && q < qr) ? mR[(q >= 16 - R && q < qr) ? q - (16 - R) : 0]
                                                       : mC;
          pr[hlf] = sv * m;
        }
        UB[k + 1] = perm_b32(pr[1], pr[0], 0x0c070c03u);
      }
    };
#pragma unroll
    for (int k = 0; k < 10; k++) V[k] = 0;
    uint32_t UB0[12], UB1[12];
    static_for<N>([&](auto K) {
      constexpr int kk = decltype(K)::value;
      uint32_t U[12];
      S.unpack(S.load(y0 - 1 - R + kk), U);
      blur_hsum10<R>(U, ring[kk + P0]);
#pragma unroll
      for (int k = 0; k < 10; k++) V[k] = add2(V[k], ring[kk + P0][k]);
    });
    blurred(y0 - 1, UB0);
    {
      uint32_t U[12], Hn[10];
      S.unpack(S.load(y0 + R), U);
      blur_hsum10<R>(U, Hn);
#pragma unroll
      for (int k = 0; k < 10; k++) V[k] = sub2(add2(V[k], Hn[k]), ring[P0][k]), ring[0][k] = Hn[k];
    }
    blurred(y0, UB1);
    st.init(UB0, UB1);
    const uint32_t cb = copy << 2;
    const unsigned inc_in = inimg ? 1u : 0u, inc_first = (inimg && !first) ? 1u : 0u, inc_last = (inimg && !last) ? 1u : 0u;

    uint32_t Mp[8] = {0, 0, 0, 0, 0, 0, 0, 0};
    unsigned livep = 0;
    auto hist_lo = [&](int k, uint32_t &through) {
      const unsigned inc = (k == 0 ? inc_first : inc_in) & livep;
      lds_add_through(lh, mad_u32_u16_lo(Mp[k], 128u, cb), inc, through);
    };
    auto hist_hi = [&](int k, uint32_t &through) {
      const unsigned inc = (k == 7 ? inc_last : inc_in) & livep;
      lds_add_through(lh, mad_u32_u16_hi(Mp[k], 128u, cb), inc, through);
    };

    strip_rows<NS, false, false>(S, y0, nrows, R + 1, S.load(y0 + R + 1), [&](auto I, int i, const uint32_t(&U)[12]) {
      constexpr int fr = (decltype(I)::value + 1) % NS, old = (decltype(I)::value + 1 + P0) % NS;
      uint32_t UB[12], M[8], Hn[10];
      blur_hsum10<R>(U, Hn);
#pragma unroll
      for (int k = 0; k < 10; k++) {
        V[k] = sub2(add2(V[k], Hn[k]), ring[old][k]), ring[fr][k] = Hn[k];
        if constexpr (HIST) {
          if (k >= 1 && k <= 8) hist_lo(k - 1, V[k]);
        }
      }
      blurred(y0 + i + 1, UB);
      auto hook = [&](int j, uint32_t &c) {
        if (j <= 8) hist_hi(j - 1, c);
      };
      U4 o;
      if constexpr (NS % 2 == 0) {
        if constexpr (HIST) o = st.template step<decltype(I)::value & 1>(UB, M, hook);
        else o = st.template step<decltype(I)::value & 1>(UB);
      } else {
        if constexpr (HIST) o = st.step_shift(UB, M, hook);
        else o = st.step_shift(UB);
      }
      if constexpr (HIST) {
#pragma unroll
        for (int k = 0; k < 8; k++) Mp[k] = M[k];
        livep = i < nrows ? 1u : 0u;
      }
      return o;
    });
    if constexpr (HIST) {
      uint32_t t = 0;
#pragma unroll
      for (int k = 0; k < 8; k++) hist_lo(k, t), hist_hi(k, t);
    }
  }
  if constexpr (HIST) {
    lds_drain();
    __syncthreads();
    unsigned acc = 0;
#pragma unroll 8
    for (unsigned k = 0; k < 32; k++) acc += lh[tid * 32u + ((k + tid) & 31u)];
    const size_t blk = (size_t)blockIdx.z * gridDim.x * gridDim.y + (size_t)blockIdx.y * gridDim.x + blockIdx.x;
    partial[blk * 256u + tid] = acc;
  }
}

}
#endif
```

grayskull_amd/csrc/k_pointwise.h:

```cpp
#ifndef GS_K_POINTWISE_H
#define GS_K_POINTWISE_H
#include "k_stencil.h"

namespace gs {

struct Chunking {
  uintptr_t a0;
  size_t lo, hi;
  size_t nchunks;
};
__host__ __device__ inline Chunking make_chunking(const void *base, size_t n) {
  Chunking c;
  c.a0 = (uintptr_t)base & ~(uintptr_t)15;
  c.lo = (uintptr_t)base - c.a0;
  c.hi = c.lo + n;
  c.nchunks = (c.hi + 15) / 16;
  return c;
}

GS_DEV uint32_t swar_gt_u8(uint32_t x, uint32_t trep) {
  const uint32_t Hb = 0x80808080u;
  uint32_t d = (trep | Hb) - (x & ~Hb);
  uint32_t ge = ((trep & ~x) | (~(trep ^ x) & d)) & Hb;
  uint32_t gt = ~ge & Hb;
  return (gt >> 7) * 0xffu;
}

__global__ __launch_bounds__(256) void k_threshold(uint8_t *img, size_t frame_bytes,
                                                   const uint8_t *thr_dev, unsigned thr_const, int thr_off = 0) {
  uint8_t *base = img + (size_t)blockIdx.y * frame_bytes;
  const unsigned t = thr_dev ? ((unsigned)((int)thr_dev[blockIdx.y] + thr_off) & 0xffu) : thr_const;
  const uint32_t trep = t * 0x01010101u;
  const Chunking c = make_chunking(base, frame_bytes);
  for (size_t i = (size_t)blockIdx.x * 256u + threadIdx.x; i < c.nchunks;
       i += (size_t)gridDim.x * 256u) {
    const size_t b0 = i * 16, b1 = b0 + 16;
    uint8_t *p = (uint8_t *)(c.a0 + b0);
    if (b0 >= c.lo && b1 <= c.hi) {
#ifndef GS_EMU
      typedef unsigned int v4u __attribute__((ext_vector_type(4)));
      const v4u q = __builtin_nontemporal_load((const v4u *)p);
      U4 v{q.x, q.y, q.z, q.w};
#else
      U4 v = *(U4 *)p;
#endif
      v.x = swar_gt_u8(v.x, trep), v.y = swar_gt_u8(v.y, trep);
      v.z = swar_gt_u8(v.z, trep), v.w = swar_gt_u8(v.w, trep);
#ifndef GS_EMU
      __builtin_nontemporal_store(v4u{v.x, v.y, v.z, v.w}, (v4u *)p);
#else
      *(U4 *)p = v;
#endif
    } else {
      const size_t s = b0 < c.lo ? c.lo : b0, e = b1 > c.hi ? c.hi : b1;
      for (size_t k = s; k < e; k++) {
        uint8_t *q = (uint8_t *)(c.a0 + k);
        *q = *q > t ? 255 : 0;
      }
    }
  }
}

#ifndef GS_HIST_DEPTH
#define GS_HIST_DEPTH 3
#endif
constexpr unsigned kHistDepth = GS_HIST_DEPTH;
constexpr size_t kHistMaxFrame = (size_t)1 << 30;
GS_DEV void hist_count16(unsigned *lh, unsigned copy, const U4 &v, unsigned inc) {
  const uint32_t d[4] = {v.x, v.y, v.z, v.w};
#pragma unroll
  for (int k = 0; k < 16; k++) atomicAdd(&lh[((d[k >> 2] >> (8 * (k & 3))) & 0xffu) * 32u + copy], inc);
}
template <unsigned BT, bool NT = false>
__global__ __launch_bounds__(BT) void k_hist_partial(const uint8_t *img, size_t frame_bytes,
                                                     unsigned *partial) {
  __shared__ unsigned lh[256 * 32];
  const unsigned tid = threadIdx.x, copy = tid & 31u;
  for (unsigned i = tid; i < 256 * 32 / 4; i += BT) ((U4 *)lh)[i] = U4{0, 0, 0, 0};
  __syncthreads();
  const uint8_t *base = img + (size_t)blockIdx.y * frame_bytes;
  const Chunking c = make_chunking(base, frame_bytes);
  const size_t c0 = c.lo ? 1 : 0, c1 = c.hi / 16;
  const size_t stride = (size_t)gridDim.x * BT, first = c0 + (size_t)blockIdx.x * BT;
  if (first < c1) {
    const uintptr_t b0 = c.a0 + c0 * 16;
    const uint32_t end = uniform((uint32_t)(c1 - c0) * 16u);
    const BufRsrc src = make_buf((const void *)(((uintptr_t)uniform((uint32_t)(b0 >> 32)) << 32) | uniform((uint32_t)b0)), end);
    const unsigned iters = (unsigned)((c1 - first + stride - 1) / stride);
    const unsigned padded = (iters + kHistDepth - 1) / kHistDepth * kHistDepth;
    const uint32_t mine = ((uint32_t)blockIdx.x * BT + tid) * 16u, step = (uint32_t)stride * 16u;
    U4 q[kHistDepth];
#pragma unroll
    for (unsigned k = 0; k < kHistDepth; k++) {
      q[k] = buf_load16_pol<NT>(src, mine + k * step);
      sched_fence();
    }
    uint32_t off = mine;
    for (unsigned it = 0; it < padded; it += kHistDepth) {
#pragma unroll
      for (unsigned k = 0; k < kHistDepth; k++) {
        hist_count16(lh, copy, q[k], off < end ? 1u : 0u);
        q[k] = buf_load16_pol<NT>(src, off + kHistDepth * step);
        off += step;
        sched_fence();
      }
    }
  }
  if (blockIdx.x == 0 && tid < 16) {
    const size_t head_end = c.hi < 16 ? c.hi : 16;
    if (c.lo && c.lo + tid < head_end) atomicAdd(&lh[(unsigned)*(const uint8_t *)(c.a0 + c.lo + tid) * 32u + copy], 1u);
    if (c1 >= c0 && c1 * 16 + tid < c.hi) atomicAdd(&lh[(unsigned)*(const uint8_t *)(c.a0 + c1 * 16 + tid) * 32u + copy], 1u);
  }
  __syncthreads();
  if (tid < 256u) {
    unsigned s = 0;
#pragma unroll 8
    for (unsigned k = 0; k < 32; k++) s += lh[tid * 32u + ((k + tid) & 31u)];
    partial[((size_t)blockIdx.y * gridDim.x + blockIdx.x) * 256u + tid] = s;
  }
}

__global__ __launch_bounds__(256) void k_hist_reduce(const unsigned *partial, unsigned bpf,
                                                     unsigned *hist, unsigned extra0) {
  const unsigned *p = partial + (size_t)blockIdx.x * bpf * 256u + threadIdx.x;
  unsigned acc[8] = {threadIdx.x == 0 ? extra0 : 0u, 0, 0, 0, 0, 0, 0, 0};
  unsigned b = 0;
  for (; b + 8 <= bpf; b += 8) {
#pragma unroll
    for (unsigned k = 0; k < 8; k++) acc[k] += p[(size_t)(b + k) * 256u];
  }
  for (; b < bpf; b++) acc[0] += p[(size_t)b * 256u];
  hist[(size_t)blockIdx.x * 256u + threadIdx.x] = ((acc[0] + acc[1]) + (acc[2] + acc[3])) + ((acc[4] + acc[5]) + (acc[6] + acc[7]));
}

__global__ __launch_bounds__(256) void k_otsu(unsigned *hist, unsigned npix, uint8_t *thr,
                                              const unsigned *partial = nullptr, unsigned bpf = 0, unsigned extra0 = 0) {
#ifndef GS_EMU
#pragma clang fp contract(off)
#endif
  __shared__ float prod[256];
  __shared__ float pre[256];
  __shared__ unsigned wsum[4];
  __shared__ float bv[4];
  __shared__ unsigned bt[4];
  const unsigned t = threadIdx.x, lane = t & 63u, wv = t >> 6;
  unsigned hv;
  if (partial) {
    const unsigned *p = partial + (size_t)blockIdx.x * bpf * 256u + t;
    unsigned acc[8] = {t == 0 ? extra0 : 0u, 0, 0, 0, 0, 0, 0, 0};
    unsigned b = 0;
    for (; b + 8 <= bpf; b += 8) {
#pragma unroll
      for (unsigned k = 0; k < 8; k++) acc[k] += p[(size_t)(b + k) * 256u];
    }
    for (; b < bpf; b++) acc[0] += p[(size_t)b * 256u];
    hv = ((acc[0] + acc[1]) + (acc[2] + acc[3])) + ((acc[4] + acc[5]) + (acc[6] + acc[7]));
    hist[(size_t)blockIdx.x * 256u + t] = hv;
  } else {
    hv = hist[(size_t)blockIdx.x * 256u + t];
  }
  prod[t] = (float)t * (float)hv;
  const unsigned inc = wave_incl_scan(hv);
  if (lane == 63) wsum[wv] = inc;
  __syncthreads();
  if (t == 0) {
    float s = 0;
    for (int i = 0; i < 256; i += 8) {
      float v[8];
#pragma unroll
      for (int k = 0; k < 8; k++) v[k] = prod[i + k];
#pragma unroll
      for (int k = 0; k < 8; k++) {
        s += v[k];
        pre[i + k] = s;
      }
    }
  }
  unsigned wb = inc;
  for (unsigned k = 0; k < wv; k++) wb += wsum[k];
  __syncthreads();
  const float sum = pre[255], sumB = pre[t];
  const unsigned wf = npix - wb;
  float var = -2.0f;
  if (wb != 0 && wf != 0) {
    const float mB = sumB / (float)wb;
    const float mF = (sum - sumB) / (float)wf;
    var = (float)wb * (float)wf * (mB - mF) * (mB - mF);
  }
  float v = var;
  unsigned a = t;
#pragma unroll
  for (int d = 32; d >= 1; d >>= 1) {
    const float ov = __builtin_bit_cast(float, shfl(__builtin_bit_cast(uint32_t, v), (int)(lane ^ (unsigned)d)));
    const unsigned oa = shfl(a, (int)(lane ^ (unsigned)d));
    if (ov > v || (ov == v && oa < a)) v = ov, a = oa;
  }
  if (lane == 0) bv[wv] = v, bt[wv] = a;
  __syncthreads();
  if (t == 0) {
    for (int k = 1; k < 4; k++)
      if (bv[k] > v || (bv[k] == v && bt[k] < a)) v = bv[k], a = bt[k];
    thr[blockIdx.x] = (uint8_t)(v > -1.0f ? a : 0u);
  }
}

__global__ __launch_bounds__(256) void k_zero_frame(uint8_t *img, unsigned w, unsigned h,
                                                    size_t frame_bytes) {
  const unsigned i = blockIdx.x * 256u + threadIdx.x;
  uint8_t *f = img + (size_t)blockIdx.y * frame_bytes;
  if (i < w) f[i] = 0;
  else if (i < 2 * w) f[(size_t)(h - 1) * w + (i - w)] = 0;
  else if (i < 2 * w + h) f[(size_t)(i - 2 * w) * w] = 0;
  else if (i < 2 * w + 2 * h) f[(size_t)(i - 2 * w - h) * w + (w - 1)] = 0;
}

__global__ __launch_bounds__(256) void k_checksum(const uint8_t *img, size_t frame_bytes,
                                                  unsigned long long *sums) {
  const uint8_t *base = img + (size_t)blockIdx.y * frame_bytes;
  unsigned long long acc = 0;
  for (size_t i = (size_t)blockIdx.x * 256u + threadIdx.x; i < frame_bytes;
       i += (size_t)gridDim.x * 256u)
    acc += (unsigned long long)(i + 1) * ((unsigned long long)base[i] + 1ull);
  uint32_t lo = (uint32_t)acc, hi = (uint32_t)(acc >> 32);
#pragma unroll
  for (int d = 32; d >= 1; d >>= 1) {
    const uint32_t olo = shfl(lo, (int)(lane_id() ^ (unsigned)d));
    const uint32_t ohi = shfl(hi, (int)(lane_id() ^ (unsigned)d));
    const unsigned long long t =
        (((unsigned long long)hi << 32) | lo) + (((unsigned long long)ohi << 32) | olo);
    lo = (uint32_t)t, hi = (uint32_t)(t >> 32);
  }
  if (lane_id() == 0) atomicAdd(&sums[blockIdx.y], ((unsigned long long)hi << 32) | lo);
}

struct SynthJump { uint32_t col[32][32]; };

GS_DEV uint32_t xs32(uint32_t x) {
  x ^= x << 13;
  x ^= x >> 17;
  x ^= x << 5;
  return x;
}
GS_DEV uint32_t xs_jump(const SynthJump *J, uint32_t s, uint64_t steps) {
  for (int k = 0; k < 32 && steps; k++, steps >>= 1)
    if (steps & 1) {
      uint32_t r = 0;
      for (int b = 0; b < 32; b++)
        if ((s >> b) & 1u) r ^= J->col[k][b];
      s = r;
    }
  return s;
}
constexpr unsigned kSynthRun = 256;
__global__ __launch_bounds__(256) void k_synth_levels(uint8_t *levels, unsigned nlev,
                                                      uint32_t seed0, const SynthJump *J) {
  const unsigned f = blockIdx.y;
  const unsigned i0 = (blockIdx.x * 256u + threadIdx.x) * kSynthRun;
  if (i0 >= nlev) return;
  uint32_t seed = seed0 + f;
  uint32_t s = xs_jump(J, seed ? seed : 1u, i0);
  for (unsigned i = i0; i < i0 + kSynthRun && i < nlev; i++) {
    s = xs32(s);
    levels[(size_t)f * nlev + i] = (uint8_t)(s & 0xff);
  }
}
__global__ __launch_bounds__(256) void k_synth_pixels(uint8_t *dst, const uint8_t *levels,
                                                      unsigned w, unsigned h, uint32_t seed0,
                                                      const SynthJump *J) {
  const unsigned f = blockIdx.y;
  const unsigned bw = (w + 31) / 32, bh = (h + 31) / 32, nlev = bw * bh;
  const size_t npx = (size_t)w * h;
  const size_t i0 = ((size_t)blockIdx.x * 256u + threadIdx.x) * kSynthRun;
  if (i0 >= npx) return;
  uint32_t seed = seed0 + f;
  uint32_t s = xs_jump(J, seed ? seed : 1u, (uint64_t)nlev + i0);
  const uint8_t *lv = levels + (size_t)f * nlev;
  uint8_t *out = dst + (size_t)f * npx;
  const bool aligned = (((uintptr_t)out) & 3) == 0;
  uint32_t packed = 0;
  for (size_t i = i0; i < i0 + kSynthRun && i < npx; i++) {
    s = xs32(s);
    const unsigned x = (unsigned)(i % w), y = (unsigned)(i / w);
    int v = (int)lv[(y / 32) * bw + x / 32] + (int)(s & 15u) - 8;
    const uint32_t b = (uint32_t)(v < 0 ? 0 : v > 255 ? 255 : v);
    if (aligned && i0 + kSynthRun <= npx) {
      packed |= b << (8 * (i & 3));
      if ((i & 3) == 3) *(uint32_t *)(out + i - 3) = packed, packed = 0;
    } else {
      out[i] = (uint8_t)b;
    }
  }
}

}
#endif
```

grayskull_amd/csrc/k_strip.h:

```cpp
#ifndef GS_K_STRIP_H
#define GS_K_STRIP_H
#include <type_traits>

#include "prims.h"

#ifndef GS_SOBEL_SAT
#define GS_SOBEL_SAT 1
#endif
#ifndef GS_BLUR_NOEXIT
#define GS_BLUR_NOEXIT 0
#endif
#ifndef GS_STRIP_PF
#define GS_STRIP_PF 1
#endif
#ifndef GS_SOBEL_NOEXIT
#define GS_SOBEL_NOEXIT 1
#endif

namespace gs {

template <int N, class F> GS_DEV void static_for(F &&f) {
  if constexpr (N > 0) {
    static_for<N - 1>(f);
    f(std::integral_constant<int, N - 1>{});
  }
}


constexpr uint32_t kRowOOB = 0x7fffffffu;
constexpr size_t kStripXcdFlag = (size_t)1 << 63;
__host__ __device__ inline unsigned strip_ragged_shift(unsigned w) {
  const unsigned t = (w - 1u) >> 4;
  return ((w & 15u) != 0u && (t & 63u) == 1u && t > 1u) ? 1u : 0u;
}
__host__ __device__ inline unsigned strip_realign_shift(unsigned w) {
  const unsigned t = (w - 1u) >> 4, l = t & 63u;
  return ((w & 15u) != 0u && (l == 1u || l == 63u) && t > 1u) ? 1u : 0u;
}
__host__ __device__ inline unsigned strip_realign_helper(unsigned w) {
  return ((w & 15u) != 0u || (((w - 1u) >> 4) & 63u) == 0u) ? 1u : 0u;
}
struct RawRow { U4 v; uint32_t hh; uint32_t hh2 = 0, p = 0; };

template <bool INVERT = false, int RG = 0> struct Strip {
  static constexpr bool RAGGED = RG != 0;
  BufRsrc src, dst;
  unsigned w, h, x0, lane, band, gid;
  uint32_t col_off, halo_off;
  bool sel_l = false, sel_r = false;
  uint32_t halo_shift = 0;
  uint32_t keep_r = 0xffffffffu;
  uint32_t src_off = kOOB, bp = 0, mask_l = 0xffffffffu, mask_r = 0xffffffffu;
  GS_DEV Strip(const uint8_t *s, uint8_t *d, unsigned w_, unsigned h_, size_t frame_bytes)
      : src(make_buf(s + (size_t)blockIdx.z * (frame_bytes & ~kStripXcdFlag), frame_bytes & ~kStripXcdFlag)),
        dst(make_buf(d + (size_t)blockIdx.z * (frame_bytes & ~kStripXcdFlag), frame_bytes & ~kStripXcdFlag)), w(w_), h(h_) {
    lane = threadIdx.x & 63u;
    gid = blockIdx.x * blockDim.x + threadIdx.x;
    band = uniform(blockIdx.y * blockDim.y + threadIdx.y);
    if (frame_bytes & kStripXcdFlag) band = (blockIdx.y & 7u) * (gridDim.y >> 3) + (blockIdx.y >> 3);
    if constexpr (RG == 0) {
      x0 = gid * 16u;
      col_off = x0 < w ? x0 : kOOB;
      halo_off = kOOB;
      if (lane == 0 && x0 > 0 && x0 < w) halo_off = x0 - 4;
      if (lane == 63 && x0 + 16 < w) halo_off = x0 + 16;
    } else {
      const unsigned t = (w - 1u) >> 4, m = w & 15u;
      gid -= RG == 2 ? strip_realign_shift(w) : strip_ragged_shift(w);
      const bool tail = m != 0u && gid == t, in = gid <= t;
      x0 = tail ? w - 16u : gid * 16u;
      keep_r = tail ? 0u : 0xffffffffu;
      col_off = in ? x0 : kOOB;
      halo_off = kOOB;
      uint32_t right = kOOB;
      if (in && x0 > 0 && (lane == 0 || tail)) halo_off = x0 - 4, sel_l = lane != 0;
      if (gid < t && (lane == 63 || (m != 0u && gid + 1u == t))) right = x0 + 16, sel_r = lane != 63;
      if (RG == 2 && m == 0u && gid == t && lane != 0u) right = x0 + 16, sel_r = lane != 63;
      if constexpr (RG == 1) {
        if (right != kOOB) {
          const uint32_t at = right + 4u > w ? w - 4u : right;
          halo_off = at, halo_shift = 8u * (right - at);
        }
      } else {
        if (right != kOOB) halo_off = right;
        const size_t fb = frame_bytes & ~kStripXcdFlag;
        const uint8_t *base = s + (size_t)blockIdx.z * fb;
        bp = (uint32_t)((uintptr_t)base & 3u);
        src = make_buf(base - bp, (fb + bp + 3u) & ~(size_t)3u);
        src_off = in ? x0 : (strip_realign_helper(w) && gid == t + 1u) ? w : kOOB;
        mask_l = (in && x0 == 0u) ? 0u : 0xffffffffu;
        const int nv = (int)w - (int)(x0 + 16u);
        mask_r = !in || nv <= 0 ? 0u : nv >= 4 ? 0xffffffffu : (1u << (8 * nv)) - 1u;
      }
    }
  }
  GS_DEV bool wave_outside() const {
    if constexpr (RAGGED) return (int)uniform(gid - lane) > (int)((w - 1u) >> 4) + (RG == 2 ? 1 : 0);
    else return uniform(x0 - lane * 16u) >= w;
  }
  GS_DEV bool in_image() const { return col_off != kOOB; }
  GS_DEV uint32_t row_off(int y, bool ok = true) const {
    return (ok && (unsigned)y < h) ? (uint32_t)y * w : (RG == 2 ? kRowOOB - 3u : kRowOOB);
  }
  GS_DEV RawRow load(int y) const {
    const uint32_t row = row_off(y);
    RawRow r;
    if constexpr (RG == 2) {
      const uint32_t a = row + bp + src_off;
      r.v = buf_load16(src, a & ~3u);
      const U2 hx = buf_load8(src, (row + bp + halo_off) & ~3u);
      r.hh = hx.x, r.hh2 = hx.y, r.p = a & 3u;
      if (INVERT) {
        const uint32_t m = (unsigned)y < h ? 0xffffffffu : 0u;
        r.v = U4{r.v.x ^ m, r.v.y ^ m, r.v.z ^ m, r.v.w ^ m};
        r.hh ^= m, r.hh2 ^= m;
      }
      return r;
    }
    r.v = buf_load16(src, row + col_off);
    r.hh = buf_load4(src, row + halo_off);
    if (INVERT) {
      const bool ok = (unsigned)y < h && in_image();
      const uint32_t m = ok ? 0xffffffffu : 0u, hm = (ok && halo_off != kOOB) ? 0xffffffffu : 0u;
      r.v = U4{r.v.x ^ m, r.v.y ^ m, r.v.z ^ m, r.v.w ^ m};
      r.hh ^= hm;
    }
    if constexpr (RG == 1) r.hh >>= halo_shift;
    return r;
  }
  GS_DEV void store(int y, bool ok, U4 o) const {
    if (INVERT) o = U4{~o.x, ~o.y, ~o.z, ~o.w};
    buf_store16(dst, row_off(y, ok) + col_off, o);
  }
  GS_DEV void unpack(const RawRow &r, uint32_t (&U)[12]) const {
    uint32_t L = wave_shr1(r.v.w, r.hh);
    uint32_t R = wave_shl1(r.v.x, r.hh);
    if constexpr (RG == 2) {
      uint32_t R2 = wave_shl1(r.v.y, r.hh2);
      L = sel_l ? r.hh : L, R = sel_r ? r.hh : R, R2 = sel_r ? r.hh2 : R2;
      const uint32_t d0 = alignbyte(r.v.x, L, r.p) & mask_l, d1 = alignbyte(r.v.y, r.v.x, r.p), d2 = alignbyte(r.v.z, r.v.y, r.p),
                     d3 = alignbyte(r.v.w, r.v.z, r.p), d4 = alignbyte(R, r.v.w, r.p), d5 = alignbyte(R2, R, r.p) & mask_r;
      U[0] = unpack_lo(d0), U[1] = unpack_hi(d0);
      U[2] = unpack_lo(d1), U[3] = unpack_hi(d1);
      U[4] = unpack_lo(d2), U[5] = unpack_hi(d2);
      U[6] = unpack_lo(d3), U[7] = unpack_hi(d3);
      U[8] = unpack_lo(d4), U[9] = unpack_hi(d4);
      U[10] = unpack_lo(d5), U[11] = unpack_hi(d5);
      return;
    }
    if constexpr (RG == 1) L = sel_l ? r.hh : L, R = (sel_r ? r.hh : R) & keep_r;
    U[0] = unpack_lo(L), U[1] = unpack_hi(L);
    U[2] = unpack_lo(r.v.x), U[3] = unpack_hi(r.v.x);
    U[4] = unpack_lo(r.v.y), U[5] = unpack_hi(r.v.y);
    U[6] = unpack_lo(r.v.z), U[7] = unpack_hi(r.v.z);
    U[8] = unpack_lo(r.v.w), U[9] = unpack_hi(r.v.w);
    U[10] = unpack_lo(R), U[11] = unpack_hi(R);
  }
};

struct NoFin {
  GS_DEV U4 operator()(const U4 &o, int) const { return o; }
  GS_DEV void prefetch(int) {}
};
template <int RING, bool INVERT, bool EXITS = true, int RG = 0, class Body, class Fin = NoFin>
GS_DEV void strip_rows(const Strip<INVERT, RG> &S, int y0, int nrows, int lead, RawRow first, Body &&body,
                       Fin fin = Fin()) {
  RawRow raw = first;
#if GS_STRIP_PF == 2
  RawRow raw2 = S.load(y0 + lead + 1);
#endif
  U4 o_prev{0, 0, 0, 0};
  fin.prefetch(y0);
  int base = 0;
  for (; base < nrows; base += RING) {
    static_for<RING>([&](auto I) {
      const int i = base + decltype(I)::value;
      if constexpr (EXITS) {
        if (i >= nrows) return;
      }
      if constexpr (!EXITS) sched_fence();
      uint32_t U[12];
      S.unpack(raw, U);
      S.store(y0 + i - 1, i > 0 && i <= nrows, fin(o_prev, y0 + i - 1));
#if GS_STRIP_PF == 2
      raw = raw2, raw2 = S.load(y0 + i + lead + 2);
#else
      raw = S.load(y0 + i + lead + 1);
#endif
      fin.prefetch(y0 + i);
      if constexpr (!EXITS) sched_fence();
      o_prev = body(I, i, U);
    });
  }
  if constexpr (EXITS) S.store(y0 + nrows - 1, nrows > 0, fin(o_prev, y0 + nrows - 1));
  else S.store(y0 + base - 1, base == nrows && nrows > 0, fin(o_prev, y0 + base - 1));
}

GS_DEV void sobel_apairs(const uint32_t (&U)[12], uint32_t (&A)[10]) {
#pragma unroll
  for (int j = 1; j <= 9; j++) A[j] = alignbit(U[j + 1], U[j], 16);
}
GS_DEV void sobel_h1(const uint32_t (&U)[12], const uint32_t (&A)[10], uint32_t (&H1)[8]) {
#pragma unroll
  for (int k = 0; k < 8; k++) H1[k] = pk_mad2_u16(U[k + 2], add2(A[k + 1], A[k + 2]));
}

struct SobelKeepCols {
  BufRsrc dst;
  unsigned w, x0;
  bool first, last;
  uint32_t keep_off;
  uint32_t e = 0;
  bool bytes = false;
  template <int RG> GS_DEV SobelKeepCols(const Strip<false, RG> &S) : dst(S.dst), w(S.w), x0(S.x0) {
    first = S.in_image() && x0 == 0, last = S.in_image() && x0 + 16 == w;
    bytes = RG == 2;
    keep_off = first ? x0 : last ? x0 + (RG == 2 ? 15u : 12u) : kOOB;
  }
  GS_DEV void prefetch(int y) {
    if (bytes) e = buf_load1(dst, (uint32_t)y * w + keep_off);
    else e = buf_load4(dst, (uint32_t)y * w + keep_off);
  }
  GS_DEV U4 operator()(U4 o, int) const {
    o.x = first ? perm_b32(o.x, e, 0x07060500u) : o.x;
    o.w = last ? perm_b32(o.w, e, bytes ? 0x00060504u : 0x03060504u) : o.w;
    return o;
  }
};

struct SobelState {
  uint32_t Ap[10], Tp[10], H1[2][8];
  GS_DEV void init(const uint32_t (&U0)[12], const uint32_t (&U1)[12]) {
    uint32_t A0[10];
    sobel_apairs(U0, A0);
    sobel_apairs(U1, Ap);
    sobel_h1(U0, A0, H1[0]);
    sobel_h1(U1, Ap, H1[1]);
#pragma unroll
    for (int j = 1; j <= 9; j++) Tp[j] = add2(A0[j], Ap[j]);
  }
  struct NoHook { GS_DEV void operator()(int, uint32_t &) const {} };
  template <int PAR, class Hook = NoHook> GS_DEV void magnitude(const uint32_t (&U)[12], uint32_t (&m)[8], Hook hook = Hook()) {
    uint32_t A[10], C[10], H1n[8];
    sobel_apairs(U, A);
#pragma unroll
    for (int j = 1; j <= 9; j++) {
      const uint32_t Tn = add2(Ap[j], A[j]);
      C[j] = add2(Tp[j], Tn);
      Tp[j] = Tn, Ap[j] = A[j];
      hook(j, C[j]);
    }
    sobel_h1(U, A, H1n);
#pragma unroll
    for (int k = 0; k < 8; k++) {
      m[k] = add2(absdiff2(C[k + 2], C[k + 1]), absdiff2(H1n[k], H1[PAR][k]));
      H1[PAR][k] = H1n[k];
    }
  }
  template <int PAR> GS_DEV U4 step(const uint32_t (&U)[12]) {
#if GS_SOBEL_SAT
    uint32_t M[8];
    magnitude<PAR>(U, M);
#pragma unroll
    for (int k = 0; k < 8; k++) M[k] = pk_shl7_sat_u16(M[k]);
    return U4{pack_lohi_b1(M[0], M[1]), pack_lohi_b1(M[2], M[3]), pack_lohi_b1(M[4], M[5]),
              pack_lohi_b1(M[6], M[7])};
#else
    uint32_t M[8];
    return step<PAR>(U, M);
#endif
  }
  template <int PAR, class Hook = NoHook> GS_DEV U4 step(const uint32_t (&U)[12], uint32_t (&M)[8], Hook hook = Hook()) {
    magnitude<PAR>(U, M, hook);
#pragma unroll
    for (int k = 0; k < 8; k++) M[k] = pk_min_u16(pk_shr_u16(M[k], 1), 0x00ff00ffu);
    return U4{pack_lohi(M[0], M[1]), pack_lohi(M[2], M[3]), pack_lohi(M[4], M[5]),
              pack_lohi(M[6], M[7])};
  }
  GS_DEV void shift_history() {
#pragma unroll
    for (int k = 0; k < 8; k++) {
      const uint32_t t = H1[0][k];
      H1[0][k] = H1[1][k], H1[1][k] = t;
    }
  }
  template <class Hook = NoHook> GS_DEV U4 step_shift(const uint32_t (&U)[12], uint32_t (&M)[8], Hook hook = Hook()) {
    const U4 o = step<0>(U, M, hook);
    shift_history();
    return o;
  }
  GS_DEV U4 step_shift(const uint32_t (&U)[12]) {
    const U4 o = step<0>(U);
    shift_history();
    return o;
  }
};

template <int R> struct BlurMagic;
template <> struct BlurMagic<1> { static constexpr uint32_t mul = 1864136; };
template <> struct BlurMagic<2> { static constexpr uint32_t mul = 671089; };
template <> struct BlurMagic<3> { static constexpr uint32_t mul = 342393; };

template <int R>
GS_DEV void blur_hsum(const uint32_t (&U)[12], uint32_t (&H)[8]) {
  uint32_t A[11], P[11];
  constexpr int jlo = R >= 3 ? 0 : 1, jhi = R >= 3 ? 10 : 9;
#pragma unroll
  for (int j = jlo; j <= jhi; j++) {
    A[j] = alignbit(U[j + 1], U[j], 16);
    P[j] = add2(U[j], A[j]);
  }
#pragma unroll
  for (int k = 0; k < 8; k++) {
    const int j = k + 2;
    if constexpr (R == 1) H[k] = add2(A[j - 1], P[j]);
    else if constexpr (R == 2) H[k] = add2(P[j - 1], P[j], U[j + 1]);
    else H[k] = add2(add2(A[j - 2], P[j - 1], P[j]), P[j + 1]);
  }
}

}
#endif
```

grayskull_amd/csrc/prims.h:

```cpp
#ifndef GS_PRIMS_H
#define GS_PRIMS_H

#if !defined(GS_EXPERIMENT) && (defined(GS_FUSED_SPARE) || defined(GS_FUSED_VGPR_ATTR) || defined(GS_EVENT_FLAGS) ||       \
                                defined(GS_ORDER_EVENT_FLAGS) || defined(GS_LOAD_AUX) || defined(GS_STORE_AUX) ||         \
                                defined(GS_LBP_PREFETCH) || defined(GS_MAD2_OPAQUE) || defined(GS_LBP_TILE_ODD_STRIDE) ||   \
                                defined(GS_LBP_SENS))
#error "experiment hook set without -DGS_EXPERIMENT (make variant / make experiment add it)"
#endif

#ifdef GS_EMU
#include "hip_emu.h"
#define GS_DYN_LDS(name) char *name = emu::S().dyn_lds
#else
#include <hip/hip_runtime.h>
#define GS_LAUNCH(kernel, grid, block, shmem, stream, ...) \
  hipLaunchKernelGGL(kernel, (grid), (block), (shmem), (stream), __VA_ARGS__)
#define GS_DYN_LDS(name) extern __shared__ __attribute__((aligned(16))) char name[]
#endif

#include <stdint.h>
#include <string.h>

#define GS_DEV __device__ __forceinline__
#define GS_HD __host__ __device__ __forceinline__
#ifndef GS_MAD2_OPAQUE
#define GS_MAD2_OPAQUE 1
#endif

namespace gs {

constexpr int kWave = 64;

struct alignas(16) U4 { uint32_t x, y, z, w; };

constexpr uint32_t kOOB = 0x80000000u;

#ifdef GS_EMU
GS_DEV unsigned lane_id() { return emu::lane_id(); }
GS_DEV unsigned mbcnt(uint64_t m) { return (unsigned)__builtin_popcountll(m & ((1ull << emu::lane_id()) - 1ull)); }
GS_DEV uint64_t ballot(bool p) {
  return emu::wave_exchange(p ? 1 : 0, [](const uint64_t *s, const bool *v) {
    uint64_t m = 0;
    for (int i = 0; i < 64; i++)
      if (v[i] && s[i]) m |= 1ull << i;
    return m;
  });
}
GS_DEV uint32_t wave_shr1(uint32_t x, uint32_t fill) {
  unsigned l = lane_id();
  return emu::wave_exchange(x, [=](const uint64_t *s, const bool *v) {
    return (l > 0 && v[l - 1]) ? (uint32_t)s[l - 1] : fill;
  });
}
GS_DEV uint32_t wave_shl1(uint32_t x, uint32_t fill) {
  unsigned l = lane_id();
  return emu::wave_exchange(x, [=](const uint64_t *s, const bool *v) {
    return (l < 63 && v[l + 1]) ? (uint32_t)s[l + 1] : fill;
  });
}
GS_DEV uint32_t shfl(uint32_t x, int src) {
  return emu::wave_exchange(x, [=](const uint64_t *s, const bool *v) {
    return v[src & 63] ? (uint32_t)s[src & 63] : 0u;
  });
}
GS_DEV uint32_t perm_b32(uint32_t hi, uint32_t lo, uint32_t sel) {
  uint64_t src = ((uint64_t)hi << 32) | lo;
  uint32_t r = 0;
  for (int i = 0; i < 4; i++) {
    unsigned s = (sel >> (8 * i)) & 0xff;
    unsigned b = s <= 7 ? (unsigned)(src >> (8 * s)) & 0xff : (s == 0x0c ? 0u : (s >= 0x0d ? 0xffu : 0u));
    r |= b << (8 * i);
  }
  return r;
}
GS_DEV uint32_t alignbit(uint32_t hi, uint32_t lo, uint32_t sh) {
  return (uint32_t)((((uint64_t)hi << 32) | lo) >> (sh & 31));
}
struct BufRsrc { uint8_t *base; uint32_t n; };
GS_DEV BufRsrc make_buf(const void *base, size_t bytes) {
  return BufRsrc{(uint8_t *)base, (uint32_t)(bytes > 0x7fffffffu ? 0x7fffffffu : bytes)};
}
GS_DEV void emu_buf_check(const BufRsrc &b, uint32_t off, uint32_t sz) {
  if (off < b.n && off + sz > b.n) { fprintf(stderr, "emu: partially out-of-range buffer access\n"); abort(); }
}
GS_DEV U4 buf_load16(const BufRsrc &b, uint32_t off) {
  uint32_t d[4] = {0, 0, 0, 0};
  for (uint32_t k = 0; k < 4; k++) {
    const uint64_t o = (uint64_t)off + 4u * k;
    if (o >= b.n) continue;
    emu_buf_check(b, (uint32_t)o, 4);
    memcpy(&d[k], b.base + o, 4);
  }
  return U4{d[0], d[1], d[2], d[3]};
}
struct U2 { uint32_t x, y; };
GS_DEV U2 buf_load8(const BufRsrc &b, uint32_t off) {
  uint32_t d[2] = {0, 0};
  for (uint32_t k = 0; k < 2; k++) {
    const uint64_t o = (uint64_t)off + 4u * k;
    if (o >= b.n) continue;
    emu_buf_check(b, (uint32_t)o, 4);
    memcpy(&d[k], b.base + o, 4);
  }
  return U2{d[0], d[1]};
}
GS_DEV uint32_t buf_load1(const BufRsrc &b, uint32_t off) { return off < b.n ? b.base[off] : 0u; }
GS_DEV uint32_t buf_load4(const BufRsrc &b, uint32_t off) {
  uint32_t v = 0;
  emu_buf_check(b, off, 4);
  if (off < b.n) memcpy(&v, b.base + off, 4);
  return v;
}
template <bool NT> GS_DEV U4 buf_load16_pol(const BufRsrc &b, uint32_t off) { return buf_load16(b, off); }
template <bool NT> GS_DEV uint32_t buf_load4_pol(const BufRsrc &b, uint32_t off) { return buf_load4(b, off); }
GS_DEV void store_u32x4(void *p, const U4 &v) { memcpy(p, &v, 16); }
GS_DEV void store_u32x4_any(void *p, const U4 &v) { memcpy(p, &v, 16); }
GS_DEV U4 load_u32x4_any(const void *p) { U4 v; memcpy(&v, p, 16); return v; }
GS_DEV void store_u32x2_any(void *p, uint32_t lo, uint32_t hi) { memcpy(p, &lo, 4), memcpy((char *)p + 4, &hi, 4); }
GS_DEV void buf_store16(const BufRsrc &b, uint32_t off, const U4 &v) {
  emu_buf_check(b, off, 16);
  if (off < b.n) memcpy(b.base + off, &v, 16);
}
GS_DEV void buf_store16_wb(const BufRsrc &b, uint32_t off, const U4 &v) { buf_store16(b, off, v); }
GS_DEV void buf_store_n(const BufRsrc &b, uint32_t off, uint64_t v, uint32_t n) {
  emu_buf_check(b, off, n);
  if (off < b.n) memcpy(b.base + off, &v, n);
}
GS_DEV void buf_store8(const BufRsrc &b, uint32_t off, uint32_t lo, uint32_t hi) { buf_store_n(b, off, lo | ((uint64_t)hi << 32), 8); }
GS_DEV void buf_store4(const BufRsrc &b, uint32_t off, uint32_t v) { buf_store_n(b, off, v, 4); }
GS_DEV void buf_store2(const BufRsrc &b, uint32_t off, uint32_t v) { buf_store_n(b, off, v, 2); }
GS_DEV void buf_store1(const BufRsrc &b, uint32_t off, uint32_t v) { buf_store_n(b, off, v, 1); }
GS_DEV uint32_t alignbyte(uint32_t hi, uint32_t lo, uint32_t sh) {
  return (uint32_t)((((uint64_t)hi << 32) | lo) >> (8 * (sh & 3)));
}
GS_DEV uint32_t buf_gather4(const BufRsrc &b, uint32_t voff, uint32_t soff) { return buf_load4(b, voff + soff); }
GS_DEV uint32_t uniform(uint32_t x) { return x; }
#define GS_PK2(expr_lo, expr_hi) ((uint32_t)((expr_lo) & 0xffffu) | ((uint32_t)((expr_hi) & 0xffffu) << 16))
GS_DEV uint32_t pk_add_u16(uint32_t a, uint32_t b) { return GS_PK2((a & 0xffff) + (b & 0xffff), (a >> 16) + (b >> 16)); }
GS_DEV uint32_t pk_sub_u16(uint32_t a, uint32_t b) { return GS_PK2((a & 0xffff) - (b & 0xffff), (a >> 16) - (b >> 16)); }
GS_DEV uint32_t pk_mul_u16(uint32_t a, uint32_t b) { return GS_PK2((a & 0xffff) * (b & 0xffff), (a >> 16) * (b >> 16)); }
GS_DEV uint32_t pk_mad_u16(uint32_t a, uint32_t b, uint32_t c) { return GS_PK2((a & 0xffff) * (b & 0xffff) + (c & 0xffff), (a >> 16) * (b >> 16) + (c >> 16)); }
GS_DEV uint32_t pk_mad2_u16(uint32_t a, uint32_t c) { return GS_PK2(2 * (a & 0xffff) + (c & 0xffff), 2 * (a >> 16) + (c >> 16)); }
GS_DEV uint32_t pk_mad_u16_s(uint32_t a, uint32_t b, uint32_t c) { return pk_mad_u16(a, b, c); }
GS_DEV uint32_t udot4(uint32_t a, uint32_t b, uint32_t c) {
  for (int i = 0; i < 4; i++) c += ((a >> (8 * i)) & 0xffu) * ((b >> (8 * i)) & 0xffu);
  return c;
}
GS_DEV uint32_t udot2_ones(uint32_t a, uint32_t c) { return (a & 0xffffu) + (a >> 16) + c; }
GS_DEV uint32_t load_u32_unaligned(const uint8_t *p) {
  uint32_t v;
  memcpy(&v, p, 4);
  return v;
}
GS_DEV uint32_t mad_u32_u16_lo(uint32_t a, uint32_t b, uint32_t c) { return (a & 0xffffu) * (b & 0xffffu) + c; }
GS_DEV uint32_t mad_u32_u16_hi(uint32_t a, uint32_t b, uint32_t c) { return (a >> 16) * (b & 0xffffu) + c; }
GS_DEV void sched_fence() {}
#define GS_SCHED_GROUP(mask, n) ((void)0)
GS_DEV uint32_t opaque(uint32_t x) { return x; }
GS_DEV uint32_t push_ge_u32(uint32_t acc, uint32_t a, uint32_t b) { return acc * 2u + (a >= b ? 1u : 0u); }
GS_DEV uint32_t push_gt_u32(uint32_t acc, uint32_t a, uint32_t b) { return acc * 2u + (a > b ? 1u : 0u); }
GS_DEV void lds_add_through(unsigned *lds_base, uint32_t byte_off, uint32_t value, uint32_t &through) {
  (void)through;
  atomicAdd((unsigned *)((char *)lds_base + byte_off), value);
}
GS_DEV void lds_drain() {}
GS_DEV uint32_t pk_shl_u16(uint32_t a, unsigned s) { return GS_PK2((a & 0xffff) << s, (a >> 16) << s); }
GS_DEV uint32_t pk_shr_u16(uint32_t a, unsigned s) { return GS_PK2((a & 0xffff) >> s, (a >> 16) >> s); }
GS_DEV uint32_t pk_min_u16(uint32_t a, uint32_t b) {
  uint32_t al = a & 0xffff, bl = b & 0xffff, ah = a >> 16, bh = b >> 16;
  return GS_PK2(al < bl ? al : bl, ah < bh ? ah : bh);
}
GS_DEV uint32_t pk_subsat_u16(uint32_t a, uint32_t b) {
  uint32_t al = a & 0xffff, bl = b & 0xffff, ah = a >> 16, bh = b >> 16;
  return GS_PK2(al > bl ? al - bl : 0u, ah > bh ? ah - bh : 0u);
}
GS_DEV uint32_t pk_shl7_sat_u16(uint32_t a) {
  uint32_t al = (a & 0xffff) * 128u, ah = (a >> 16) * 128u;
  return GS_PK2(al > 0xffffu ? 0xffffu : al, ah > 0xffffu ? 0xffffu : ah);
}
GS_DEV uint32_t pk_max_u16(uint32_t a, uint32_t b) {
  uint32_t al = a & 0xffff, bl = b & 0xffff, ah = a >> 16, bh = b >> 16;
  return GS_PK2(al > bl ? al : bl, ah > bh ? ah : bh);
}
GS_DEV uint32_t pk_abs_i16(uint32_t a) {
  int al = (int16_t)(a & 0xffff), ah = (int16_t)(a >> 16);
  return GS_PK2((uint32_t)(al < 0 ? -al : al), (uint32_t)(ah < 0 ? -ah : ah));
}
GS_DEV uint32_t pk_max_i16(uint32_t a, uint32_t b) {
  int al = (int16_t)(a & 0xffff), ah = (int16_t)(a >> 16), bl = (int16_t)(b & 0xffff), bh = (int16_t)(b >> 16);
  return GS_PK2((uint32_t)(al > bl ? al : bl), (uint32_t)(ah > bh ? ah : bh));
}
GS_DEV uint32_t pk_sar_i16(uint32_t a, unsigned s) {
  int al = (int16_t)(a & 0xffff), ah = (int16_t)(a >> 16);
  return GS_PK2((uint32_t)(al >> s), (uint32_t)(ah >> s));
}
GS_DEV void mfma_i32_32x32x32_i8(const U4 &a, const U4 &b, int32_t (&c)[16]) {
  const unsigned l = lane_id();
  uint64_t A[64][2], B[64][2];
  const uint64_t av[2] = {a.x | ((uint64_t)a.y << 32), a.z | ((uint64_t)a.w << 32)};
  const uint64_t bv[2] = {b.x | ((uint64_t)b.y << 32), b.z | ((uint64_t)b.w << 32)};
  for (int h = 0; h < 2; h++) {
    emu::wave_exchange(av[h], [&](const uint64_t *s, const bool *v) { for (int i = 0; i < 64; i++) A[i][h] = v[i] ? s[i] : 0; return 0; });
    emu::wave_exchange(bv[h], [&](const uint64_t *s, const bool *v) { for (int i = 0; i < 64; i++) B[i][h] = v[i] ? s[i] : 0; return 0; });
  }
  auto byte_of = [](const uint64_t (&q)[2], int k) { return (int)(int8_t)((q[k >> 3] >> (8 * (k & 7))) & 0xff); };
  for (int r = 0; r < 16; r++) {
    const int row = (r & 3) + 8 * (r >> 2) + 4 * (int)(l >> 5), col = (int)(l & 31);
    int32_t acc = c[r];
    for (int g = 0; g < 2; g++)
      for (int k = 0; k < 16; k++) acc += byte_of(A[row + 32 * g], k) * byte_of(B[col + 32 * g], k);
    c[r] = acc;
  }
}
#else
GS_DEV unsigned lane_id() { return __builtin_amdgcn_mbcnt_hi(~0u, __builtin_amdgcn_mbcnt_lo(~0u, 0u)); }
GS_DEV unsigned mbcnt(uint64_t m) { return __builtin_amdgcn_mbcnt_hi((uint32_t)(m >> 32), __builtin_amdgcn_mbcnt_lo((uint32_t)m, 0u)); }
GS_DEV uint64_t ballot(bool p) { return __builtin_amdgcn_ballot_w64(p); }
GS_DEV uint32_t wave_shr1(uint32_t x, uint32_t fill) {
  return (uint32_t)__builtin_amdgcn_update_dpp((int)fill, (int)x, 0x138, 0xf, 0xf, false);
}
GS_DEV uint32_t wave_shl1(uint32_t x, uint32_t fill) {
  return (uint32_t)__builtin_amdgcn_update_dpp((int)fill, (int)x, 0x130, 0xf, 0xf, false);
}
GS_DEV uint32_t shfl(uint32_t x, int src) {
  return (uint32_t)__builtin_amdgcn_ds_bpermute((src & 63) << 2, (int)x);
}
GS_DEV uint32_t perm_b32(uint32_t hi, uint32_t lo, uint32_t sel) { return __builtin_amdgcn_perm(hi, lo, sel); }
GS_DEV uint32_t alignbit(uint32_t hi, uint32_t lo, uint32_t sh) { return __builtin_amdgcn_alignbit(hi, lo, sh); }

#ifndef GS_LOAD_AUX
#define GS_LOAD_AUX 0
#endif
#ifndef GS_STORE_AUX
#define GS_STORE_AUX 2
#endif
typedef unsigned int gs_u32x4 __attribute__((ext_vector_type(4)));
struct BufRsrc { __amdgpu_buffer_rsrc_t r; };
GS_DEV BufRsrc make_buf(const void *base, size_t bytes) {
  return BufRsrc{__builtin_amdgcn_make_buffer_rsrc((void *)base, 0, (int)(bytes > 0x7fffffffu ? 0x7fffffffu : bytes), 0x00020000)};
}
GS_DEV U4 buf_load16(const BufRsrc &b, uint32_t off) {
  const gs_u32x4 v = __builtin_amdgcn_raw_buffer_load_b128(b.r, (int)off, 0, GS_LOAD_AUX);
  return U4{v.x, v.y, v.z, v.w};
}
GS_DEV uint32_t buf_load4(const BufRsrc &b, uint32_t off) {
  return __builtin_amdgcn_raw_buffer_load_b32(b.r, (int)off, 0, GS_LOAD_AUX);
}
template <bool NT> GS_DEV U4 buf_load16_pol(const BufRsrc &b, uint32_t off) {
  const gs_u32x4 v = __builtin_amdgcn_raw_buffer_load_b128(b.r, (int)off, 0, NT ? 2 : GS_LOAD_AUX);
  return U4{v.x, v.y, v.z, v.w};
}
template <bool NT> GS_DEV uint32_t buf_load4_pol(const BufRsrc &b, uint32_t off) {
  return __builtin_amdgcn_raw_buffer_load_b32(b.r, (int)off, 0, NT ? 2 : GS_LOAD_AUX);
}
struct U2 { uint32_t x, y; };
GS_DEV U2 buf_load8(const BufRsrc &b, uint32_t off) {
  typedef unsigned int gs_u32x2_ __attribute__((ext_vector_type(2)));
  const gs_u32x2_ v = __builtin_amdgcn_raw_buffer_load_b64(b.r, (int)off, 0, GS_LOAD_AUX);
  return U2{v.x, v.y};
}
GS_DEV uint32_t buf_load1(const BufRsrc &b, uint32_t off) {
  return (uint32_t)__builtin_amdgcn_raw_buffer_load_b8(b.r, (int)off, 0, GS_LOAD_AUX);
}
GS_DEV uint32_t buf_gather4(const BufRsrc &b, uint32_t voff, uint32_t soff) {
  return __builtin_amdgcn_raw_buffer_load_b32(b.r, (int)voff, (int)soff, 0);
}
GS_DEV uint32_t uniform(uint32_t x) { return (uint32_t)__builtin_amdgcn_readfirstlane((int)x); }
GS_DEV void store_u32x4(void *p, const U4 &v) { *(gs_u32x4 *)p = gs_u32x4{v.x, v.y, v.z, v.w}; }
typedef gs_u32x4 gs_u32x4_a1 __attribute__((aligned(1)));
GS_DEV void store_u32x4_any(void *p, const U4 &v) { *(gs_u32x4_a1 *)p = gs_u32x4{v.x, v.y, v.z, v.w}; }
GS_DEV U4 load_u32x4_any(const void *p) {
  const gs_u32x4 v = *(const gs_u32x4_a1 *)p;
  return U4{v.x, v.y, v.z, v.w};
}
GS_DEV void store_u32x2_any(void *p, uint32_t lo, uint32_t hi) {
  typedef unsigned int u32x2_a1 __attribute__((ext_vector_type(2), aligned(1)));
  *(u32x2_a1 *)p = u32x2_a1{lo, hi};
}
GS_DEV void buf_store16(const BufRsrc &b, uint32_t off, const U4 &v) {
  __builtin_amdgcn_raw_buffer_store_b128(gs_u32x4{v.x, v.y, v.z, v.w}, b.r, (int)off, 0, GS_STORE_AUX);
}
GS_DEV void buf_store16_wb(const BufRsrc &b, uint32_t off, const U4 &v) {
  __builtin_amdgcn_raw_buffer_store_b128(gs_u32x4{v.x, v.y, v.z, v.w}, b.r, (int)off, 0, 0);
}
typedef unsigned int gs_u32x2 __attribute__((ext_vector_type(2)));
GS_DEV void buf_store8(const BufRsrc &b, uint32_t off, uint32_t lo, uint32_t hi) {
  __builtin_amdgcn_raw_buffer_store_b64(gs_u32x2{lo, hi}, b.r, (int)off, 0, 0);
}
GS_DEV void buf_store4(const BufRsrc &b, uint32_t off, uint32_t v) { __builtin_amdgcn_raw_buffer_store_b32(v, b.r, (int)off, 0, 0); }
GS_DEV void buf_store2(const BufRsrc &b, uint32_t off, uint32_t v) { __builtin_amdgcn_raw_buffer_store_b16((unsigned short)v, b.r, (int)off, 0, 0); }
GS_DEV void buf_store1(const BufRsrc &b, uint32_t off, uint32_t v) { __builtin_amdgcn_raw_buffer_store_b8((unsigned char)v, b.r, (int)off, 0, 0); }
GS_DEV uint32_t alignbyte(uint32_t hi, uint32_t lo, uint32_t sh) { return __builtin_amdgcn_alignbyte(hi, lo, sh); }
typedef unsigned short gs_u16x2 __attribute__((ext_vector_type(2)));
typedef short gs_i16x2 __attribute__((ext_vector_type(2)));
#define GS_U2(x) __builtin_bit_cast(gs_u16x2, (uint32_t)(x))
#define GS_I2(x) __builtin_bit_cast(gs_i16x2, (uint32_t)(x))
#define GS_R(x) __builtin_bit_cast(uint32_t, (x))
GS_DEV uint32_t pk_add_u16(uint32_t a, uint32_t b) { return GS_R((gs_u16x2)(GS_U2(a) + GS_U2(b))); }
GS_DEV uint32_t pk_sub_u16(uint32_t a, uint32_t b) { return GS_R((gs_u16x2)(GS_U2(a) - GS_U2(b))); }
GS_DEV uint32_t pk_mul_u16(uint32_t a, uint32_t b) { return GS_R((gs_u16x2)(GS_U2(a) * GS_U2(b))); }
GS_DEV uint32_t pk_mad_u16(uint32_t a, uint32_t b, uint32_t c) { return GS_R((gs_u16x2)(GS_U2(a) * GS_U2(b) + GS_U2(c))); }
GS_DEV uint32_t pk_mad2_u16(uint32_t a, uint32_t c) {
#if GS_MAD2_OPAQUE
  uint32_t two;
  asm("s_mov_b32 %0, 0x00020002" : "=s"(two));
  return pk_mad_u16(a, two, c);
#else
  uint32_t d;
  asm("v_pk_mad_u16 %0, %1, 2, %2 op_sel_hi:[1,0,1]" : "=v"(d) : "v"(a), "v"(c));
  return d;
#endif
}
GS_DEV void sched_fence() { __builtin_amdgcn_sched_barrier(0); }
#define GS_SCHED_GROUP(mask, n) __builtin_amdgcn_sched_group_barrier(mask, n, 0)
GS_DEV uint32_t opaque(uint32_t x) {
  asm volatile("" : "+v"(x));
  return x;
}
GS_DEV uint32_t push_ge_u32(uint32_t acc, uint32_t a, uint32_t b) {
  asm("v_cmp_ge_u32_e32 vcc, %1, %2\n\tv_addc_co_u32_e32 %0, vcc, %0, %0, vcc" : "+v"(acc) : "v"(a), "v"(b) : "vcc");
  return acc;
}
GS_DEV uint32_t push_gt_u32(uint32_t acc, uint32_t a, uint32_t b) {
  asm("v_cmp_gt_u32_e32 vcc, %1, %2\n\tv_addc_co_u32_e32 %0, vcc, %0, %0, vcc" : "+v"(acc) : "v"(a), "v"(b) : "vcc");
  return acc;
}
template <class T> GS_DEV uint32_t lds_address(T *p) {
  return (uint32_t)(uintptr_t)(__attribute__((address_space(3))) void *)p;
}
#ifdef GS_PLAIN_LDS_ATOMICS
GS_DEV void lds_add_through(unsigned *lds_base, uint32_t byte_off, uint32_t value, uint32_t &through) {
  (void)through;
  atomicAdd((unsigned *)((char *)lds_base + byte_off), value);
}
GS_DEV void lds_drain() {}
#else
GS_DEV void lds_add_through(unsigned *lds_base, uint32_t byte_off, uint32_t value, uint32_t &through) {
  asm volatile("ds_add_u32 %1, %2" : "+v"(through) : "v"(lds_address(lds_base) + byte_off), "v"(value) : "memory");
}
GS_DEV void lds_drain() { asm volatile("s_waitcnt lgkmcnt(0)" ::: "memory"); }
#endif
GS_DEV uint32_t pk_mad_u16_s(uint32_t a, uint32_t b, uint32_t c) {
  uint32_t d;
  asm("v_pk_mad_u16 %0, %1, %2, %3" : "=v"(d) : "v"(a), "s"(b), "v"(c));
  return d;
}
GS_DEV uint32_t udot4(uint32_t a, uint32_t b, uint32_t c) { return __builtin_amdgcn_udot4(a, b, c, false); }
GS_DEV uint32_t udot2_ones(uint32_t a, uint32_t c) {
  typedef unsigned short gs_u16x2 __attribute__((ext_vector_type(2)));
  return __builtin_amdgcn_udot2(__builtin_bit_cast(gs_u16x2, a), gs_u16x2{1, 1}, c, false);
}
GS_DEV uint32_t load_u32_unaligned(const uint8_t *p) {
  typedef uint32_t u32_unaligned __attribute__((aligned(1)));
  return *(const u32_unaligned *)p;
}
GS_DEV uint32_t mad_u32_u16_lo(uint32_t a, uint32_t b, uint32_t c) {
  uint32_t d;
  asm("v_mad_u32_u16 %0, %1, %2, %3 op_sel:[0,0,0,0]" : "=v"(d) : "v"(a), "s"(b), "v"(c));
  return d;
}
GS_DEV uint32_t mad_u32_u16_hi(uint32_t a, uint32_t b, uint32_t c) {
  uint32_t d;
  asm("v_mad_u32_u16 %0, %1, %2, %3 op_sel:[1,0,0,0]" : "=v"(d) : "v"(a), "s"(b), "v"(c));
  return d;
}
GS_DEV uint32_t pk_shl_u16(uint32_t a, unsigned s) { return GS_R((gs_u16x2)(GS_U2(a) << (unsigned short)s)); }
GS_DEV uint32_t pk_shr_u16(uint32_t a, unsigned s) { return GS_R((gs_u16x2)(GS_U2(a) >> (unsigned short)s)); }
GS_DEV uint32_t pk_min_u16(uint32_t a, uint32_t b) { return GS_R(__builtin_elementwise_min(GS_U2(a), GS_U2(b))); }
GS_DEV uint32_t pk_max_u16(uint32_t a, uint32_t b) { return GS_R(__builtin_elementwise_max(GS_U2(a), GS_U2(b))); }
GS_DEV uint32_t pk_subsat_u16(uint32_t a, uint32_t b) { return GS_R(__builtin_elementwise_sub_sat(GS_U2(a), GS_U2(b))); }
GS_DEV uint32_t pk_shl7_sat_u16(uint32_t a) {
  uint32_t d;
  asm("v_pk_mad_u16 %0, %1, %2, 0 clamp" : "=v"(d) : "v"(a), "s"(0x00800080u));
  return d;
}
GS_DEV uint32_t pk_abs_i16(uint32_t a) { return GS_R(__builtin_elementwise_abs(GS_I2(a))); }
GS_DEV uint32_t pk_max_i16(uint32_t a, uint32_t b) { return GS_R(__builtin_elementwise_max(GS_I2(a), GS_I2(b))); }
GS_DEV uint32_t pk_sar_i16(uint32_t a, unsigned s) { return GS_R((gs_i16x2)(GS_I2(a) >> (short)s)); }
GS_DEV void mfma_i32_32x32x32_i8(const U4 &a, const U4 &b, int32_t (&c)[16]) {
  typedef int gs_i32x4 __attribute__((ext_vector_type(4)));
  typedef int gs_i32x16 __attribute__((ext_vector_type(16)));
  gs_i32x16 acc;
#pragma unroll
  for (int r = 0; r < 16; r++) acc[r] = c[r];
  acc = __builtin_amdgcn_mfma_i32_32x32x32_i8(gs_i32x4{(int)a.x, (int)a.y, (int)a.z, (int)a.w},
                                              gs_i32x4{(int)b.x, (int)b.y, (int)b.z, (int)b.w}, acc, 0, 0, 0);
#pragma unroll
  for (int r = 0; r < 16; r++) c[r] = acc[r];
}
#endif

#ifndef GS_PLAIN_ADDS
#define GS_PLAIN_ADDS 1
#endif
#if GS_PLAIN_ADDS
GS_DEV uint32_t add2(uint32_t a, uint32_t b) { return a + b; }
GS_DEV uint32_t add2(uint32_t a, uint32_t b, uint32_t c) { return a + b + c; }
GS_DEV uint32_t sub2(uint32_t a, uint32_t b) { return a - b; }
#else
GS_DEV uint32_t add2(uint32_t a, uint32_t b) { return pk_add_u16(a, b); }
GS_DEV uint32_t add2(uint32_t a, uint32_t b, uint32_t c) { return pk_add_u16(pk_add_u16(a, b), c); }
GS_DEV uint32_t sub2(uint32_t a, uint32_t b) { return pk_sub_u16(a, b); }
#endif
GS_DEV uint32_t absdiff2(uint32_t a, uint32_t b) { return sub2(pk_max_u16(a, b), pk_min_u16(a, b)); }
GS_DEV unsigned umin(unsigned a, unsigned b) { return a < b ? a : b; }
GS_DEV unsigned umax(unsigned a, unsigned b) { return a > b ? a : b; }
GS_DEV uint32_t mul_u24(uint32_t a, uint32_t b) {
#ifdef GS_EMU
  return (a & 0xffffffu) * (b & 0xffffffu);
#else
  return __ockl_mul24_u32(a, b);
#endif
}
GS_DEV unsigned absdiff_u16(unsigned a, unsigned b) {
#ifdef GS_EMU
  return a > b ? a - b : b - a;
#else
  return __builtin_amdgcn_sad_u16(a, b, 0u);
#endif
}
template <int S0, int S1, int S2, int S3>
GS_DEV uint32_t quad_perm(uint32_t x) {
#ifdef GS_EMU
  const int sel[4] = {S0, S1, S2, S3};
  return (uint32_t)emu::quad_exchange(x, (unsigned)sel[lane_id() & 3u]);
#else
  return (uint32_t)__builtin_amdgcn_update_dpp(0, (int)x, S0 | (S1 << 2) | (S2 << 4) | (S3 << 6), 0xf, 0xf, false);
#endif
}
GS_DEV uint32_t readlane0(uint32_t x) { return shfl(x, 0); }

GS_DEV uint32_t wave_incl_scan(uint32_t v) {
#ifdef GS_EMU
  unsigned l = lane_id();
#pragma unroll
  for (int d = 1; d < 64; d <<= 1) {
    uint32_t t = shfl(v, (int)l - d);
    if ((int)l >= d) v += t;
  }
  return v;
#else
  v += (uint32_t)__builtin_amdgcn_update_dpp(0, (int)v, 0x111, 0xf, 0xf, false);
  v += (uint32_t)__builtin_amdgcn_update_dpp(0, (int)v, 0x112, 0xf, 0xf, false);
  v += (uint32_t)__builtin_amdgcn_update_dpp(0, (int)v, 0x114, 0xf, 0xf, false);
  v += (uint32_t)__builtin_amdgcn_update_dpp(0, (int)v, 0x118, 0xf, 0xf, false);
  v += (uint32_t)__builtin_amdgcn_update_dpp(0, (int)v, 0x142, 0xa, 0xf, false);
  v += (uint32_t)__builtin_amdgcn_update_dpp(0, (int)v, 0x143, 0xc, 0xf, false);
  return v;
#endif
}
GS_DEV uint32_t readlane_at(uint32_t x, unsigned k) {
#ifdef GS_EMU
  return shfl(x, (int)k);
#else
  return (uint32_t)__builtin_amdgcn_readlane((int)x, (int)k);
#endif
}
GS_DEV uint32_t readlane_last(uint32_t x) {
#ifdef GS_EMU
  return shfl(x, 63);
#else
  return (uint32_t)__builtin_amdgcn_readlane((int)x, 63);
#endif
}
GS_DEV void wave_sync() {
#ifdef GS_EMU
  (void)emu::wave_exchange(0, [](const uint64_t *, const bool *) { return 0; });
#else
  __builtin_amdgcn_fence(__ATOMIC_RELEASE, "wavefront");
  __builtin_amdgcn_wave_barrier();
  __builtin_amdgcn_fence(__ATOMIC_ACQUIRE, "wavefront");
#endif
}
GS_DEV uint32_t wave_sum(uint32_t v) {
#pragma unroll
  for (int d = 32; d >= 1; d >>= 1) v += shfl(v, (int)(lane_id() ^ (unsigned)d));
  return v;
}
GS_DEV int wave_sum_i(int v) { return (int)wave_sum((uint32_t)v); }

GS_DEV U4 shift_down_bytes(U4 v, unsigned nb) {
  uint32_t e0, e1, e2, e3;
  switch (nb >> 2) {
    case 0: e0 = v.x, e1 = v.y, e2 = v.z, e3 = v.w; break;
    case 1: e0 = v.y, e1 = v.z, e2 = v.w, e3 = 0u; break;
    case 2: e0 = v.z, e1 = v.w, e2 = 0u, e3 = 0u; break;
    default: e0 = v.w, e1 = 0u, e2 = 0u, e3 = 0u; break;
  }
  const uint32_t sel = 0x03020100u + 0x01010101u * (nb & 3u);
  return U4{perm_b32(e1, e0, sel), perm_b32(e2, e1, sel), perm_b32(e3, e2, sel), perm_b32(0u, e3, sel)};
}
GS_DEV void buf_store_first(const BufRsrc &b, uint32_t off, uint32_t ox, uint32_t oy, uint32_t oz, uint32_t ow, unsigned m) {
  const bool on = off != kOOB;
  uint64_t rest = ox | ((uint64_t)oy << 32);
  if (m & 8u) buf_store8(b, off, ox, oy), rest = oz | ((uint64_t)ow << 32);
  if (m & 4u) buf_store4(b, on ? off + (m & 8u) : kOOB, (uint32_t)rest), rest >>= 32;
  if (m & 2u) buf_store2(b, on ? off + (m & 12u) : kOOB, (uint32_t)rest), rest >>= 16;
  if (m & 1u) buf_store1(b, on ? off + (m & 14u) : kOOB, (uint32_t)rest);
}

GS_DEV uint32_t unpack_lo(uint32_t d) { return perm_b32(0, d, 0x0c010c00u); }
GS_DEV uint32_t unpack_hi(uint32_t d) { return perm_b32(0, d, 0x0c030c02u); }
GS_DEV uint32_t pack_lohi(uint32_t lo, uint32_t hi) { return perm_b32(hi, lo, 0x06040200u); }
GS_DEV uint32_t pack_lohi_b1(uint32_t lo, uint32_t hi) { return perm_b32(hi, lo, 0x07050301u); }

}
#endif
```

include/grayskull_hip.h:

```cpp
#ifndef GRAYSKULL_HIP_H
#define GRAYSKULL_HIP_H

#include <stddef.h>
#include <stdint.h>

#include "grayskull.h"

#ifdef __cplusplus
extern "C" {
#endif

const char *gsh_version(void);
int gsh_device_count(void);
void gsh_set_device(int ordinal);
void gsh_set_stream(void *hip_stream);
void *gsh_get_stream(void);
void gsh_set_async(int on);
void gsh_sync(void);
enum gsh_tune_key {
  GSH_TUNE_STRIP_BAND_ROWS = 0,
  GSH_TUNE_STRIP_BLOCK_SHAPE = 1,
  GSH_TUNE_RETIRED_2 = 2,
  GSH_TUNE_RETIRED_3 = 3,
  GSH_TUNE_LBP_PHASE_PRESET = 4,
  GSH_TUNE_PIPELINE_CHUNK = 5,
  GSH_TUNE_COMPARE = 6,
  GSH_TUNE_FAST_SCORE = 7,
  GSH_TUNE_FRAMES_PER_LAUNCH = 8,
  GSH_TUNE_LBP_ADAPTIVE = 9,
  GSH_TUNE_RETIRED_10 = 10,
  GSH_TUNE_HIST_BLOCKS = 11,
  GSH_TUNE_HIST_PIECE = 12,
  GSH_TUNE_LBP_XCD = 13,
  GSH_TUNE_LBP_KERNEL = 14,
  GSH_TUNE_LBP_TILE_SWITCH = 15,
  GSH_TUNE_EXPERIMENT_16 = 16,
  GSH_TUNE_RETIRED_17 = 17,
  GSH_TUNE_STRIP_XCD = 18,
  GSH_TUNE_FAST_NMS = 19,
  GSH_TUNE_TMATCH = 20,
  GSH_TUNE_RETIRED_21 = 21,
  GSH_TUNE_EXPERIMENT_22 = 22,
  GSH_TUNE_EXPERIMENT_23 = 23,
  GSH_TUNE_RETIRED_24 = 24,
  GSH_TUNE_GEOM_FORM = 25,
  GSH_TUNE_TMATCH_CHUNK = 26
};
void gsh_tune(int key, int value);
void gsh_profile(int on);
unsigned gsh_profile_read(double *total_ms);
#ifdef GS_EXPERIMENT
void gsh_probe_strip_copy(uint8_t *dst, const uint8_t *src, unsigned w, unsigned h, unsigned n);
#endif
void gsh_shutdown(void);

void *gsh_malloc(size_t bytes);
void gsh_free(void *dev);
void *gsh_host_alloc(size_t bytes);
void gsh_host_free(void *host);
void gsh_memset(void *dev, int byte, size_t bytes);
void gsh_upload(void *dev, const void *host, size_t bytes);
void gsh_download(void *host, const void *dev, size_t bytes);
int gsh_is_device_ptr(const void *p);

void gsh_blur_batch(uint8_t *dst, const uint8_t *src, unsigned w, unsigned h, unsigned n,
                    unsigned radius);
void gsh_sobel_batch(uint8_t *dst, const uint8_t *src, unsigned w, unsigned h, unsigned n);
void gsh_erode_batch(uint8_t *dst, const uint8_t *src, unsigned w, unsigned h, unsigned n);
void gsh_dilate_batch(uint8_t *dst, const uint8_t *src, unsigned w, unsigned h, unsigned n);
void gsh_morph_batch(uint8_t *dst, const uint8_t *src, uint8_t *tmp, unsigned w, unsigned h, unsigned n,
                     int dilate, unsigned iterations);

void gsh_histogram_batch(const uint8_t *img, unsigned w, unsigned h, unsigned n, unsigned *hist);
void gsh_otsu_batch(const uint8_t *img, unsigned w, unsigned h, unsigned n, unsigned *hist_scratch,
                    uint8_t *thr);
void gsh_threshold_batch(uint8_t *img, unsigned w, unsigned h, unsigned n, uint8_t thresh);
void gsh_threshold_batch_dev(uint8_t *img, unsigned w, unsigned h, unsigned n, const uint8_t *thr);
void gsh_threshold_batch_dev_offset(uint8_t *img, unsigned w, unsigned h, unsigned n, const uint8_t *thr,
                                    int offset);

void gsh_blur_sobel_batch(uint8_t *dst, const uint8_t *src, unsigned w, unsigned h, unsigned n,
                          unsigned radius);

void gsh_edge_pipeline_batch(uint8_t *dst, uint8_t *tmp, const uint8_t *src, unsigned w, unsigned h,
                             unsigned n, unsigned radius, unsigned *hist_scratch, uint8_t *thr);

void gsh_integral_batch(const uint8_t *src, unsigned w, unsigned h, unsigned n, unsigned *ii);

typedef struct gsh_cascade gsh_cascade;
gsh_cascade *gsh_cascade_create(const struct gs_lbp_cascade *c);
void gsh_cascade_destroy(gsh_cascade *dc);

void gsh_lbp_detect_batch(const gsh_cascade *dc, const unsigned *ii, unsigned iw, unsigned ih,
                          unsigned n, struct gs_rect *rects, unsigned *counts, unsigned max_rects,
                          float scale_factor, float min_scale, float max_scale, int step);
void gsh_lbp_count_evaluated(unsigned long long *counter_dev);
uint64_t gsh_lbp_window_count(const struct gs_lbp_cascade *c, unsigned iw, unsigned ih,
                              float scale_factor, float min_scale, float max_scale, int step);

void gsh_fast_score_batch(uint8_t *score, const uint8_t *img, unsigned w, unsigned h, unsigned n, unsigned threshold);
void gsh_fast_batch(const uint8_t *img, uint8_t *scoremap, unsigned w, unsigned h, unsigned n,
                    struct gs_keypoint *kps, unsigned *counts, unsigned nkps, unsigned threshold);

unsigned gsh_orb_extract(const uint8_t *img_dev, unsigned w, unsigned h, uint8_t *scoremap_dev,
                         struct gs_keypoint *kps_host, unsigned nkps, unsigned threshold);

void gsh_orb_extract_batch(const uint8_t *img_dev, unsigned w, unsigned h, unsigned n,
                           uint8_t *scoremap_dev, struct gs_keypoint *kps_host, unsigned *counts_host,
                           unsigned nkps, unsigned threshold);
void gsh_orb_extract_batch_nostdlib(const uint8_t *img_dev, unsigned w, unsigned h, unsigned n,
                                    uint8_t *scoremap_dev, struct gs_keypoint *kps_dev, unsigned *counts_dev,
                                    unsigned nkps, unsigned threshold);

size_t gsh_orb_pyramid_buffer_bytes(unsigned w, unsigned h, unsigned n_levels);
unsigned gsh_orb_extract_pyramid(const uint8_t *img_dev, unsigned w, unsigned h, uint8_t *buffer_dev,
                                 struct gs_keypoint *kps_host, unsigned nkps, unsigned threshold,
                                 unsigned n_levels);

void gsh_match_orb_dev(const struct gs_keypoint *k1, unsigned n1, const struct gs_keypoint *k2,
                       unsigned n2, struct gs_match *matches, unsigned *count,
                       unsigned max_matches, float max_distance);

void gsh_adaptive_threshold_batch(uint8_t *dst, const uint8_t *src, unsigned w, unsigned h,
                                  unsigned n, unsigned radius, int c);
void gsh_filter_batch(uint8_t *dst, const uint8_t *src, unsigned w, unsigned h, unsigned n,
                      const int8_t *kernel_host, unsigned kw, unsigned kh, unsigned norm);
void gsh_downsample_batch(uint8_t *dst, const uint8_t *src, unsigned sw, unsigned sh, unsigned n);

void gsh_crop_batch(uint8_t *dst, const uint8_t *src, unsigned sw, unsigned sh, unsigned n, struct gs_rect roi);
void gsh_resize_batch(uint8_t *dst, unsigned dw, unsigned dh, const uint8_t *src, unsigned sw, unsigned sh, unsigned n);
void gsh_resize_nn_batch(uint8_t *dst, unsigned dw, unsigned dh, const uint8_t *src, unsigned sw, unsigned sh, unsigned n);
void gsh_crop_resize_batch(uint8_t *dst, unsigned dw, unsigned dh, const uint8_t *src, unsigned sw, unsigned sh, unsigned n,
                           const struct gs_rect *rois_dev, const unsigned *frame_of_dev ,
                           unsigned npatches, int nearest);

void gsh_match_template_batch(const uint8_t *img, unsigned iw, unsigned ih, unsigned n,
                              const uint8_t *tmpl, unsigned tw, unsigned th, unsigned ntmpl, uint8_t *result);
void gsh_find_best_match_batch(const uint8_t *result, unsigned rw, unsigned rh, unsigned n,
                               struct gs_point *best, uint8_t *score);
void gsh_locate_template_batch(const uint8_t *img, unsigned iw, unsigned ih, unsigned n,
                               const uint8_t *tmpl, unsigned tw, unsigned th, unsigned ntmpl,
                               struct gs_point *best, uint8_t *score);

void gsh_blobs_batch(const uint8_t *img, unsigned w, unsigned h, unsigned n, gs_label *labels,
                     struct gs_blob *blobs, unsigned *counts, unsigned nblobs);
void gsh_blob_corners_batch(const uint8_t *img, const gs_label *labels, unsigned w, unsigned h,
                            unsigned n, const struct gs_blob *blobs, struct gs_point *corners);
void gsh_perspective_correct_batch(uint8_t *dst, unsigned dw, unsigned dh, const uint8_t *src,
                                   unsigned sw, unsigned sh, unsigned n,
                                   const struct gs_point *corners);
void gsh_blob_largest_batch(const struct gs_blob *blobs, unsigned nblobs, const unsigned *counts, unsigned n,
                            struct gs_blob *largest, unsigned *index);
void gsh_blob_paint_batch(uint8_t *dst, const uint8_t *img, unsigned w, unsigned h, unsigned n,
                          const struct gs_blob *blobs, unsigned nblobs, const unsigned *counts);

void gsh_trace_contours_batch(const uint8_t *img, uint8_t *visited, unsigned w, unsigned h, unsigned n,
                              struct gs_contour *contours, unsigned per_frame, const unsigned *counts,
                              uint8_t *status);
void gsh_blob_contour_starts_batch(const gs_label *labels, unsigned w, unsigned h, unsigned n,
                                   const struct gs_blob *blobs, unsigned nblobs, const unsigned *counts,
                                   struct gs_contour *contours);

void gsh_synth_batch(uint8_t *dst, unsigned w, unsigned h, unsigned n, uint32_t seed0);
void gsh_checksum_batch(const uint8_t *img, size_t frame_bytes, unsigned n, uint64_t *sums);

typedef struct gsh_comm gsh_comm;
int gsh_comm_init_all(gsh_comm **comms, int ndev, const int *devices);
void gsh_comm_destroy_all(gsh_comm **comms, int ndev);
int gsh_comm_rank(const gsh_comm *c);
int gsh_comm_world(const gsh_comm *c);
const char *gsh_comm_backend(const gsh_comm *c);
void gsh_comm_broadcast(gsh_comm *c, void *buf_dev, size_t bytes, int root);
void gsh_comm_all_gather(gsh_comm *c, const void *send_dev, void *recv_dev, size_t bytes_per_rank);
void gsh_comm_all_reduce_u64(gsh_comm *c, unsigned long long *buf_dev, size_t n, int op);
void gsh_comm_all_reduce_f64(gsh_comm *c, double *buf_dev, size_t n, int op);

#ifdef __cplusplus
}
#endif
#endif
```

Before: 1.393 million Mpix/s.

## Add coded 4-bit edge pipeline with sampled Otsu prediction and gated fallback

For radius-2 4K batches, a sampled pass first estimates each frame's Otsu threshold from a few row bands. The fused blur+sobel+hist kernel then writes 4-bit codes centred on that estimate into a double-buffered half-size plane instead of full bytes. A decode kernel expands the codes to a binary output when the real threshold falls inside the coded window. Otherwise the frame is recomputed by gated full-precision kernels on the side stream. The aim is to cut intermediate HBM write and read traffic, at the cost of an extra sampling pass, more stream synchronisation, and full recomputation on misses.

```diff
diff --git a/grayskull_amd/__init__.py b/grayskull_amd/__init__.py
--- a/grayskull_amd/__init__.py
+++ b/grayskull_amd/__init__.py
@@ -102,6 +102,7 @@
     "gsh_blur_sobel_batch": (None, [C.c_void_p, C.c_void_p, C.c_uint, C.c_uint, C.c_uint, C.c_uint]),
     "gsh_edge_pipeline_batch": (None, [C.c_void_p, C.c_void_p, C.c_void_p, C.c_uint, C.c_uint,
                                        C.c_uint, C.c_uint, C.c_void_p, C.c_void_p]),
+    "gsh_edge_pipeline_stats": (None, [C.POINTER(C.c_uint), C.POINTER(C.c_uint)]),
     "gsh_integral_batch": (None, [C.c_void_p, C.c_uint, C.c_uint, C.c_uint, C.c_void_p]),
     "gsh_cascade_create": (C.c_void_p, [C.c_void_p]),
     "gsh_cascade_destroy": (None, [C.c_void_p]),
@@ -204,7 +205,10 @@
         if os.path.abspath(path) == os.path.abspath(HIP_LIBRARY):
             _share_torch_hip_runtime()
         self.c = C.CDLL(path)
+        older_ab = os.path.basename(os.path.dirname(os.path.abspath(path))) == "build_variants"
         for name, (res, args) in _SIGS.items():
+            if older_ab and not hasattr(self.c, name):
+                continue
             f = getattr(self.c, name)
             f.restype, f.argtypes = res, args
         for name, (res, args) in _EXPERIMENT_SIGS.items():
@@ -444,6 +448,11 @@
         self.c.gsh_edge_pipeline_batch(_ptr(dst), _ptr(tmp) if tmp is not None else None, _ptr(src), w, h, n, radius,
                                        _ptr(hist_scratch), _ptr(thr))
 
+    def edge_pipeline_stats(self):
+        coded, fallback = C.c_uint(0), C.c_uint(0)
+        self.c.gsh_edge_pipeline_stats(C.byref(coded), C.byref(fallback))
+        return int(coded.value), int(fallback.value)
+
     def integral_batch(self, src, ii):
         n, h, w = self._nhw(src)
         self.c.gsh_integral_batch(_ptr(src), w, h, n, _ptr(ii))
diff --git a/grayskull_amd/csrc/gs_fused.cpp b/grayskull_amd/csrc/gs_fused.cpp
--- a/grayskull_amd/csrc/gs_fused.cpp
+++ b/grayskull_amd/csrc/gs_fused.cpp
@@ -12,6 +12,32 @@
   if (radius == 1) GS_LAUNCH(k_blur_sobel_hist16<1>, grid, block, 0, st, dst, src, w, h, T, frame_bytes, partial);
   else if (radius == 2) GS_LAUNCH(k_blur_sobel_hist16<2>, grid, block, 0, st, dst, src, w, h, T, frame_bytes, partial);
   else GS_LAUNCH(k_blur_sobel_hist16<3>, grid, block, 0, st, dst, src, w, h, T, frame_bytes, partial);
+}
+
+void launch_blur_sobel_sample(unsigned radius, dim3 grid, dim3 block, hipStream_t st, const uint8_t *src, unsigned w, unsigned h,
+                              size_t frame_bytes, unsigned *partial) {
+  uint8_t *none = const_cast<uint8_t *>(src);
+  if (radius == 1) GS_LAUNCH((k_blur_sobel_hist16<1, true, 0, 1, kFormSample>), grid, block, 0, st, none, src, w, h, 16u, frame_bytes, partial);
+  else if (radius == 2) GS_LAUNCH((k_blur_sobel_hist16<2, true, 0, 1, kFormSample>), grid, block, 0, st, none, src, w, h, 16u, frame_bytes, partial);
+  else GS_LAUNCH((k_blur_sobel_hist16<3, true, 0, 1, kFormSample>), grid, block, 0, st, none, src, w, h, 16u, frame_bytes, partial);
+}
+void launch_blur_sobel_codes(unsigned radius, dim3 grid, dim3 block, hipStream_t st, uint8_t *codes, const uint8_t *src, unsigned w,
+                             unsigned h, unsigned T, size_t frame_bytes, unsigned *partial, const uint8_t *centre) {
+  uint8_t *none = const_cast<uint8_t *>(src);
+  FusedForm fx;
+  fx.centre = centre, fx.codes = codes;
+  if (radius == 1) GS_LAUNCH((k_blur_sobel_hist16<1, true, 0, 1, kFormCodes>), grid, block, 0, st, none, src, w, h, T, frame_bytes, partial, fx);
+  else if (radius == 2) GS_LAUNCH((k_blur_sobel_hist16<2, true, 0, 1, kFormCodes>), grid, block, 0, st, none, src, w, h, T, frame_bytes, partial, fx);
+  else GS_LAUNCH((k_blur_sobel_hist16<3, true, 0, 1, kFormCodes>), grid, block, 0, st, none, src, w, h, T, frame_bytes, partial, fx);
+}
+void launch_blur_sobel_gated(unsigned radius, dim3 grid, dim3 block, hipStream_t st, uint8_t *dst, const uint8_t *src, unsigned w,
+                             unsigned h, unsigned T, size_t frame_bytes, const uint8_t *gate) {
+  unsigned *none = nullptr;
+  FusedForm fx;
+  fx.gate = gate;
+  if (radius == 1) GS_LAUNCH((k_blur_sobel_hist16<1, false, 0, 1, kFormGated>), grid, block, 0, st, dst, src, w, h, T, frame_bytes, none, fx);
+  else if (radius == 2) GS_LAUNCH((k_blur_sobel_hist16<2, false, 0, 1, kFormGated>), grid, block, 0, st, dst, src, w, h, T, frame_bytes, none, fx);
+  else GS_LAUNCH((k_blur_sobel_hist16<3, false, 0, 1, kFormGated>), grid, block, 0, st, dst, src, w, h, T, frame_bytes, none, fx);
 }
 
 void launch_blur_sobel(unsigned radius, dim3 grid, dim3 block, hipStream_t st, uint8_t *dst, const uint8_t *src,
diff --git a/grayskull_amd/csrc/gs_internal.h b/grayskull_amd/csrc/gs_internal.h
--- a/grayskull_amd/csrc/gs_internal.h
+++ b/grayskull_amd/csrc/gs_internal.h
@@ -46,6 +46,12 @@
                             unsigned *partial);
 void launch_blur_sobel(unsigned radius, dim3 grid, dim3 block, hipStream_t st, uint8_t *dst, const uint8_t *src,
                        unsigned w, unsigned h, unsigned T, size_t frame_bytes, int rg);
+void launch_blur_sobel_sample(unsigned radius, dim3 grid, dim3 block, hipStream_t st, const uint8_t *src, unsigned w, unsigned h,
+                              size_t frame_bytes, unsigned *partial);
+void launch_blur_sobel_codes(unsigned radius, dim3 grid, dim3 block, hipStream_t st, uint8_t *codes, const uint8_t *src, unsigned w,
+                             unsigned h, unsigned T, size_t frame_bytes, unsigned *partial, const uint8_t *centre);
+void launch_blur_sobel_gated(unsigned radius, dim3 grid, dim3 block, hipStream_t st, uint8_t *dst, const uint8_t *src, unsigned w,
+                             unsigned h, unsigned T, size_t frame_bytes, const uint8_t *gate);
 void launch_box(int mode, unsigned ring_radius, dim3 grid, unsigned threads, hipStream_t st, uint8_t *dst, const uint8_t *src, unsigned w,
                 unsigned h, unsigned T, size_t frame_bytes, unsigned r, int c);
 void launch_box_edge(int mode, dim3 grid, hipStream_t st, uint8_t *dst, const uint8_t *src, unsigned w, unsigned h, unsigned T,
@@ -60,9 +66,15 @@
 enum Slot { SL_IN = 0, SL_OUT, SL_AUX, SL_AUX2, SL_II, SL_PAD, SL_MASK, SL_CNT, SL_PFX, SL_TOT, SL_PRE,
             SL_HISTP, SL_HIST, SL_THR, SL_KPS, SL_MOM, SL_KIN, SL_DESC, SL_TAB, SL_JUMP, SL_LEV,
             SL_BEST, SL_NZ,
+            SL_CODES, SL_EDGE, SL_EDGE_STAT,
             SL_BLOB_BITS, SL_BLOB_PAR, SL_BLOB_STAT, SL_BLOB_ROW, SL_BLOB_LAB, SL_BLOB_REC, SL_COUNT };
 
 constexpr unsigned kChunkFrames = 32, kMaxChunks = 256;
+constexpr unsigned kCodedMinChunks = 16;
+constexpr size_t kCodedMinFrameBytes = (size_t)3840 * 2160;
+inline bool coded_by_rule(unsigned radius, size_t chunks, size_t frame_bytes) {
+  return radius == 2 && chunks >= kCodedMinChunks && frame_bytes >= kCodedMinFrameBytes;
+}
 struct LbpGeomCache {
   unsigned iw = 0, ih = 0;
   float sf = 0, mn = 0, mx = 0;
@@ -115,6 +127,7 @@
     return b.p;
   }
   bool jump_ready = false;
+  bool edge_stat_ready = false;
   bool lbp_lds_raised = false;
   std::map<unsigned long long, LbpGeomCache> geom_cache;
   struct ::gsh_cascade *dropin_cascade = nullptr;
@@ -141,6 +154,7 @@
   }
   hipStream_t side = nullptr;
   hipEvent_t ev_join = nullptr, ev_chunk[kMaxChunks] = {};
+  hipEvent_t ev_fork = nullptr, ev_sample = nullptr, ev_plane[2] = {};
   hipEvent_t ev_switch = nullptr;
   void ensure_side() {
     if (side) return;
@@ -152,6 +166,9 @@
     }
     GS_HIP(hipEventCreateWithFlags(&ev_join, order_event_flags()));
     for (auto &e : ev_chunk) GS_HIP(hipEventCreateWithFlags(&e, order_event_flags()));
+    GS_HIP(hipEventCreateWithFlags(&ev_fork, order_event_flags()));
+    GS_HIP(hipEventCreateWithFlags(&ev_sample, order_event_flags()));
+    for (auto &e : ev_plane) GS_HIP(hipEventCreateWithFlags(&e, order_event_flags()));
   }
 #endif
 
@@ -209,6 +226,7 @@
       b.p = nullptr, b.cap = 0;
     }
     jump_ready = false;
+    edge_stat_ready = false;
     lbp_lds_raised = false;
     drop_geom();
     if (dropin_cascade) gsh_cascade_tables_deleter()(dropin_cascade);
@@ -224,6 +242,9 @@
     if (side) {
       (void)hipStreamDestroy(side), (void)hipEventDestroy(ev_join);
       for (auto &e : ev_chunk) (void)hipEventDestroy(e), e = nullptr;
+      (void)hipEventDestroy(ev_fork), ev_fork = nullptr;
+      (void)hipEventDestroy(ev_sample), ev_sample = nullptr;
+      for (auto &e : ev_plane) (void)hipEventDestroy(e), e = nullptr;
       side = nullptr, ev_join = nullptr;
     }
 #endif
diff --git a/grayskull_amd/csrc/gs_stencil.cpp b/grayskull_amd/csrc/gs_stencil.cpp
--- a/grayskull_amd/csrc/gs_stencil.cpp
+++ b/grayskull_amd/csrc/gs_stencil.cpp
@@ -667,6 +667,24 @@
   GS_HIP(hipMemsetAsync(dst, 0, fb * n, st));
   if (w >= 3 && h >= 3) launch_sobel(dst, t, w, h, n, true);
 }
+static unsigned *edge_stats() {
+  Ctx &c = ctx();
+  unsigned *p = (unsigned *)c.scratch(SL_EDGE_STAT, 2 * sizeof(unsigned));
+  if (!c.edge_stat_ready) {
+    GS_HIP(hipMemsetAsync(p, 0, 2 * sizeof(unsigned), c.s()));
+    c.edge_stat_ready = true;
+  }
+  return p;
+}
+void gsh_edge_pipeline_stats(unsigned *coded, unsigned *fallback) {
+  unsigned v[2] = {0, 0};
+  unsigned *p = edge_stats();
+  GS_HIP(hipMemcpyAsync(v, p, sizeof v, hipMemcpyDeviceToHost, ctx().s()));
+  ctx().sync();
+  GS_HIP(hipMemsetAsync(p, 0, sizeof v, ctx().s()));
+  if (coded) *coded = v[0];
+  if (fallback) *fallback = v[1];
+}
 void gsh_edge_pipeline_batch(uint8_t *dst, uint8_t *tmp, const uint8_t *src, unsigned w, unsigned h,
                              unsigned n, unsigned radius, unsigned *hist_scratch, uint8_t *thr) {
   GS_ASSERT(dst && src && hist_scratch && thr && w > 0 && h > 0);
@@ -683,14 +701,47 @@
     const unsigned per = tune_chunk < 0 ? n : tune_chunk > 0 ? (unsigned)tune_chunk : kChunkFrames;
     std::vector<unsigned> sizes;
     for (unsigned rem = n; rem; rem -= std::min(rem, per)) sizes.push_back(std::min(rem, per));
+    if (n == 0) return;
+    GS_ASSERT(dst + fb * n <= src || src + fb * n <= dst);
     auto cfg_for = [&](unsigned nn) { return strip_cfg(w, h - 2, std::min(kMaxZ, nn), 3);  };
     unsigned bpf_max = 0;
     for (unsigned nn : sizes) {
       const StripCfg c = cfg_for(nn);
       bpf_max = std::max(bpf_max, c.grid.x * c.grid.y);
     }
-    unsigned *partial = (unsigned *)ctx().scratch(SL_HISTP, (size_t)n * bpf_max * 256 * 4);
-    auto run_fused = [&](hipStream_t on, unsigned f0, unsigned nn) {
+#ifdef GS_EMU
+    const bool split = false;
+#else
+    const bool split = sizes.size() > 1 && sizes.size() <= kMaxChunks;
+#endif
+    const bool coded = g_tune[27] == 2 || (g_tune[27] == 0 && split && h - 2 > 64 && coded_by_rule(radius, sizes.size(), fb));
+    const dim3 sblock = cfg_for(n).block;
+    const unsigned srows = h - 2 <= 64 ? h - 2 : 64, sbands = h - 2 <= 64 ? 1 : 4;
+    const dim3 sgrid((w / 16 + sblock.x - 1) / sblock.x, (sbands + sblock.y - 1) / sblock.y);
+    const unsigned bpf_s = coded ? sgrid.x * sgrid.y : 0;
+    unsigned *partial = (unsigned *)ctx().scratch(SL_HISTP, (size_t)n * (bpf_max + bpf_s) * 256 * 4);
+    unsigned *spartial = partial + (size_t)n * bpf_max * 256;
+    const unsigned nplanes = split ? 2 : 1;
+    const size_t plane_bytes = (size_t)(split ? sizes[0] : n) * (fb / 2);
+    uint8_t *planes = nullptr, *centre = nullptr, *miss = nullptr;
+    unsigned *shist = nullptr, *stats = nullptr;
+    if (coded) {
+      planes = (uint8_t *)ctx().scratch(SL_CODES, plane_bytes * nplanes);
+      const size_t nb = ((size_t)n + 255) & ~(size_t)255;
+      centre = (uint8_t *)ctx().scratch(SL_EDGE, 2 * nb + (size_t)n * 256 * 4);
+      miss = centre + nb, shist = (unsigned *)(centre + 2 * nb);
+      stats = edge_stats();
+    }
+    auto run_sample = [&](hipStream_t on, unsigned f0, unsigned nn) {
+      for (unsigned g0 = f0; g0 < f0 + nn; g0 += kMaxZ) {
+        const unsigned m = std::min(kMaxZ, f0 + nn - g0);
+        unsigned *pp = spartial + (size_t)g0 * bpf_s * 256;
+        launch_blur_sobel_sample(radius, dim3(sgrid.x, sgrid.y, m), sblock, on, src + fb * g0, w, h, fb, pp);
+        GS_LAUNCH(k_otsu, dim3(m), dim3(256), 0, on, shist + (size_t)g0 * 256, srows * (w - 2), centre + g0,
+                  (const unsigned *)pp, bpf_s, 0u);
+      }
+    };
+    auto run_fused = [&](hipStream_t on, unsigned f0, unsigned nn, uint8_t *plane) {
       const StripCfg c = cfg_for(nn);
       for (unsigned g0 = f0; g0 < f0 + nn; g0 += kMaxZ) {
         const unsigned m = std::min(kMaxZ, f0 + nn - g0);
@@ -701,13 +752,14 @@
 #ifndef GS_EMU
         ctx().prof_mark(0, on);
 #endif
-        launch_blur_sobel_hist(radius, grid, c.block, on, d, sp, w, h, c.T, fb, pp);
+        if (coded) launch_blur_sobel_codes(radius, grid, c.block, on, plane + (fb / 2) * (g0 - f0), sp, w, h, c.T, fb, pp, centre + g0);
+        else launch_blur_sobel_hist(radius, grid, c.block, on, d, sp, w, h, c.T, fb, pp);
 #ifndef GS_EMU
         ctx().prof_mark(1, on);
 #endif
       }
     };
-    auto run_rest = [&](hipStream_t on, unsigned f0, unsigned nn) {
+    auto run_rest = [&](hipStream_t on, unsigned f0, unsigned nn, const uint8_t *plane) {
       const StripCfg c = cfg_for(nn);
       const unsigned bpf = c.grid.x * c.grid.y;
       for (unsigned g0 = f0; g0 < f0 + nn; g0 += kMaxZ) {
@@ -716,37 +768,68 @@
         GS_LAUNCH(k_otsu, dim3(m), dim3(256), 0, on, hist_scratch + (size_t)g0 * 256, w * h, thr + g0, pp, bpf,
                   2 * w + 2 * (h - 2));
       }
-      launch_threshold(dst + fb * f0, fb, nn, thr + f0, 0, on);
+      if (coded) {
+        const unsigned bx = (unsigned)std::max<size_t>(1, std::min<size_t>((fb / 16 + 255) / 256, 2048));
+        for (unsigned g0 = f0; g0 < f0 + nn; g0 += kMaxZ) {
+          const unsigned m = std::min(kMaxZ, f0 + nn - g0);
+          GS_LAUNCH(k_decode_codes, dim3(bx, m), dim3(256), 0, on, dst + fb * g0, plane + (fb / 2) * (g0 - f0), fb,
+                    (const uint8_t *)(thr + g0), (const uint8_t *)(centre + g0), miss + g0, stats);
+        }
+      } else {
+        launch_threshold(dst + fb * f0, fb, nn, thr + f0, 0, on);
+      }
       for (unsigned g0 = f0; g0 < f0 + nn; g0 += kMaxZ) {
         const unsigned m = std::min(kMaxZ, f0 + nn - g0);
         GS_LAUNCH(k_zero_frame, dim3((2 * w + 2 * h + 255) / 256, m), dim3(256), 0, on, dst + fb * g0, w, h, fb);
       }
     };
-#ifdef GS_EMU
-    const bool split = false;
-#else
-    const bool split = sizes.size() > 1 && sizes.size() <= kMaxChunks;
-#endif
+    auto run_fallback = [&](hipStream_t on, unsigned f0, unsigned nn) {
+      const StripCfg c = cfg_for(nn);
+      for (unsigned g0 = f0; g0 < f0 + nn; g0 += kMaxZ) {
+        const unsigned m = std::min(kMaxZ, f0 + nn - g0);
+        launch_blur_sobel_gated(radius, dim3(c.grid.x, c.grid.y, m), c.block, on, dst + fb * g0, src + fb * g0, w, h, c.T, fb,
+                                miss + g0);
+        GS_LAUNCH(k_threshold_gated, dim3(64, m), dim3(256), 0, on, dst + fb * g0, fb, (const uint8_t *)(thr + g0),
+                  (const uint8_t *)(miss + g0));
+        GS_LAUNCH(k_zero_frame_gated, dim3((2 * w + 2 * h + 255) / 256, m), dim3(256), 0, on, dst + fb * g0, w, h, fb,
+                  (const uint8_t *)(miss + g0));
+      }
+    };
     if (!split) {
-      run_fused(st, 0, n);
-      run_rest(st, 0, n);
+      if (coded) run_sample(st, 0, n);
+      run_fused(st, 0, n, planes);
+      run_rest(st, 0, n, planes);
+      if (coded) run_fallback(st, 0, n);
       return;
     }
 #ifndef GS_EMU
     Ctx &cx = ctx();
     cx.ensure_side();
+    if (coded) {
+      GS_HIP(hipEventRecord(cx.ev_fork, st));
+      GS_HIP(hipStreamWaitEvent(cx.side, cx.ev_fork, 0));
+      run_sample(st, 0, sizes[0]);
+      run_sample(cx.side, sizes[0], n - sizes[0]);
+      GS_HIP(hipEventRecord(cx.ev_sample, cx.side));
+    }
     unsigned f0 = 0;
     for (size_t i = 0; i < sizes.size(); i++) {
       const unsigned nn = sizes[i];
-      run_fused(st, f0, nn);
+      uint8_t *plane = coded ? planes + plane_bytes * (i % nplanes) : nullptr;
+      if (coded && i == 1) GS_HIP(hipStreamWaitEvent(st, cx.ev_sample, 0));
+      if (coded && i >= nplanes) GS_HIP(hipStreamWaitEvent(st, cx.ev_plane[i % nplanes], 0));
+      run_fused(st, f0, nn, plane);
       if (i + 1 == sizes.size()) {
+        if (coded) run_fallback(cx.side, 0, f0);
         GS_HIP(hipEventRecord(cx.ev_join, cx.side));
         GS_HIP(hipStreamWaitEvent(st, cx.ev_join, 0));
-        run_rest(st, f0, nn);
+        run_rest(st, f0, nn, plane);
+        if (coded) run_fallback(st, f0, nn);
       } else {
         GS_HIP(hipEventRecord(cx.ev_chunk[i], st));
         GS_HIP(hipStreamWaitEvent(cx.side, cx.ev_chunk[i], 0));
-        run_rest(cx.side, f0, nn);
+        run_rest(cx.side, f0, nn, plane);
+        if (coded) GS_HIP(hipEventRecord(cx.ev_plane[i % nplanes], cx.side));
       }
       f0 += nn;
     }
diff --git a/grayskull_amd/csrc/k_fused.h b/grayskull_amd/csrc/k_fused.h
--- a/grayskull_amd/csrc/k_fused.h
+++ b/grayskull_amd/csrc/k_fused.h
@@ -43,13 +43,26 @@
 #ifndef GS_FUSED_VGPR_ATTR
 #define GS_FUSED_VGPR_ATTR
 #endif
-template <int R, bool HIST = true, int RG = 0, int MINW = 1>
+enum { kFormBytes = 0, kFormSample = 1, kFormCodes = 2, kFormGated = 3 };
+struct FusedForm {
+  const uint8_t *centre = nullptr;
+  uint8_t *codes = nullptr;
+  const uint8_t *gate = nullptr;
+};
+GS_DEV uint32_t code_pack4(uint32_t c0, uint32_t c1, uint32_t c2, uint32_t c3) {
+  return (c0 | (c1 << 8)) | ((c2 | (c3 << 8)) << 4);
+}
+template <int R, bool HIST = true, int RG = 0, int MINW = 1, int FORM = kFormBytes>
 __global__ __launch_bounds__(256, MINW) GS_FUSED_VGPR_ATTR void k_blur_sobel_hist16(uint8_t *dst, const uint8_t *src,
                                                            unsigned w, unsigned h, unsigned T,
-                                                           size_t frame_bytes, unsigned *partial) {
+                                                           size_t frame_bytes, unsigned *partial, FusedForm fx = FusedForm()) {
   constexpr bool RAGGED = RG != 0;
   static_assert(!(HIST && RAGGED), "ragged rows take the histogram as a separate pass");
+  static_assert(HIST || FORM == kFormBytes || FORM == kFormGated, "the sample and the codes come with the histogram");
   constexpr int N = 2 * R + 1;
+  if constexpr (FORM == kFormGated) {
+    if (!fx.gate[blockIdx.z]) return;
+  }
   __shared__ unsigned lh[HIST ? 256 * 32 : 1];
   const unsigned tid = threadIdx.y * blockDim.x + threadIdx.x, copy = tid & 31u;
   if constexpr (HIST) {
@@ -57,8 +70,23 @@
     __syncthreads();
   }
   const Strip<false, RG> S(src, dst, w, h, frame_bytes);
-  const int y0 = 1 + (int)(S.band * T);
-  if (y0 < (int)h - 1 && !S.wave_outside()) {
+  int y0 = 1 + (int)(S.band * T);
+  bool band_ok = true;
+  if constexpr (FORM == kFormSample) {
+    const bool all = h - 2u <= 64u;
+    band_ok = S.band < (all ? 1u : 4u);
+    y0 = all ? 1 : 1 + (int)(((2u * S.band + 1u) * (h - 2u)) / 8u) - 8;
+    T = all ? h - 2u : 16u;
+  }
+  BufRsrc cbuf;
+  uint32_t lo2 = 0, ccol = kOOB;
+  if constexpr (FORM == kFormCodes) {
+    const size_t fb = frame_bytes & ~kStripXcdFlag;
+    cbuf = make_buf(fx.codes + (size_t)blockIdx.z * (fb / 2), fb / 2);
+    lo2 = uniform(edge_code_lo(fx.centre[blockIdx.z])) * 0x10001u;
+    ccol = S.in_image() ? S.x0 / 2u : kOOB / 2u;
+  }
+  if (band_ok && y0 < (int)h - 1 && !S.wave_outside()) {
     const int nrows = ((int)h - 1 - y0) < (int)T ? ((int)h - 1 - y0) : (int)T;
     const bool first = S.x0 == 0, last = S.x0 + 16 == w, inimg = S.in_image();
     bool edge[R + 2][R];
@@ -144,7 +172,8 @@
       lds_add_through(lh, mad_u32_u16_hi(Mp[k], 128u, cb), inc, through);
     };
 
-    strip_rows<NS, false, false>(S, y0, nrows, R + 1, S.load(y0 + R + 1), [&](auto I, int i, const uint32_t(&U)[12]) {
+    constexpr bool STORE = FORM == kFormBytes || FORM == kFormGated;
+    strip_rows<NS, false, false, RG, STORE>(S, y0, nrows, R + 1, S.load(y0 + R + 1), [&](auto I, int i, const uint32_t(&U)[12]) {
       constexpr int fr = (decltype(I)::value + 1) % NS, old = (decltype(I)::value + 1 + P0) % NS;
       uint32_t UB[12], M[8], Hn[10];
       blur_hsum10<R>(U, Hn);
@@ -172,6 +201,13 @@
         for (int k = 0; k < 8; k++) Mp[k] = M[k];
         livep = i < nrows ? 1u : 0u;
       }
+      if constexpr (FORM == kFormCodes) {
+        uint32_t c[8];
+#pragma unroll
+        for (int k = 0; k < 8; k++) c[k] = pk_min_u16(pk_subsat_u16(M[k], lo2), 0x000f000fu);
+        const uint32_t row = i < nrows ? (uint32_t)(y0 + i) * (w / 2u) : kRowOOB / 2u + 1u;
+        buf_store8_nt(cbuf, row + ccol, code_pack4(c[0], c[1], c[2], c[3]), code_pack4(c[4], c[5], c[6], c[7]));
+      }
       return o;
     });
     if constexpr (HIST) {
diff --git a/grayskull_amd/csrc/k_pointwise.h b/grayskull_amd/csrc/k_pointwise.h
--- a/grayskull_amd/csrc/k_pointwise.h
+++ b/grayskull_amd/csrc/k_pointwise.h
@@ -26,10 +26,7 @@
   return (gt >> 7) * 0xffu;
 }
 
-__global__ __launch_bounds__(256) void k_threshold(uint8_t *img, size_t frame_bytes,
-                                                   const uint8_t *thr_dev, unsigned thr_const, int thr_off = 0) {
-  uint8_t *base = img + (size_t)blockIdx.y * frame_bytes;
-  const unsigned t = thr_dev ? ((unsigned)((int)thr_dev[blockIdx.y] + thr_off) & 0xffu) : thr_const;
+GS_DEV void threshold_frame(uint8_t *base, size_t frame_bytes, unsigned t) {
   const uint32_t trep = t * 0x01010101u;
   const Chunking c = make_chunking(base, frame_bytes);
   for (size_t i = (size_t)blockIdx.x * 256u + threadIdx.x; i < c.nchunks;
@@ -58,6 +55,55 @@
         *q = *q > t ? 255 : 0;
       }
     }
+  }
+}
+__global__ __launch_bounds__(256) void k_threshold(uint8_t *img, size_t frame_bytes,
+                                                   const uint8_t *thr_dev, unsigned thr_const, int thr_off = 0) {
+  const unsigned t = thr_dev ? ((unsigned)((int)thr_dev[blockIdx.y] + thr_off) & 0xffu) : thr_const;
+  threshold_frame(img + (size_t)blockIdx.y * frame_bytes, frame_bytes, t);
+}
+__global__ __launch_bounds__(256) void k_threshold_gated(uint8_t *img, size_t frame_bytes, const uint8_t *thr_dev,
+                                                         const uint8_t *gate) {
+  if (!gate[blockIdx.y]) return;
+  threshold_frame(img + (size_t)blockIdx.y * frame_bytes, frame_bytes, thr_dev[blockIdx.y]);
+}
+
+__global__ __launch_bounds__(256) void k_decode_codes(uint8_t *dst, const uint8_t *codes, size_t frame_bytes,
+                                                      const uint8_t *thr, const uint8_t *centre, uint8_t *miss,
+                                                      unsigned *stats) {
+  const unsigned t = thr[blockIdx.y], lo = edge_code_lo(centre[blockIdx.y]);
+  const bool hit = t >= lo && t <= lo + 14u;
+  if (blockIdx.x == 0 && threadIdx.x == 0) {
+    miss[blockIdx.y] = hit ? 0 : 1;
+    atomicAdd(&stats[hit ? 0 : 1], 1u);
+  }
+  if (!hit) return;
+  const uint32_t add = (127u - (t - lo)) * 0x01010101u;
+  uint8_t *d = dst + (size_t)blockIdx.y * frame_bytes;
+  const uint8_t *c = codes + (size_t)blockIdx.y * (frame_bytes / 2);
+  const size_t nchunks = frame_bytes / 16;
+  for (size_t i = (size_t)blockIdx.x * 256u + threadIdx.x; i < nchunks; i += (size_t)gridDim.x * 256u) {
+#ifndef GS_EMU
+    typedef unsigned int v2u __attribute__((ext_vector_type(2)));
+    typedef unsigned int v4u __attribute__((ext_vector_type(4)));
+    const v2u q = __builtin_nontemporal_load((const v2u *)(c + i * 8));
+    const uint32_t z[2] = {q.x, q.y};
+#else
+    uint32_t z[2];
+    memcpy(z, c + i * 8, 8);
+#endif
+    uint32_t o[4];
+#pragma unroll
+    for (int k = 0; k < 2; k++) {
+      const uint32_t a = z[k] & 0x0f0f0f0fu, b = (z[k] >> 4) & 0x0f0f0f0fu;
+      const uint32_t ga = (((a + add) & 0x80808080u) >> 7) * 0xffu, gb = (((b + add) & 0x80808080u) >> 7) * 0xffu;
+      o[2 * k] = perm_b32(0u, ga, 0x03010200u), o[2 * k + 1] = perm_b32(0u, gb, 0x03010200u);
+    }
+#ifndef GS_EMU
+    __builtin_nontemporal_store(v4u{o[0], o[1], o[2], o[3]}, (v4u *)(d + i * 16));
+#else
+    memcpy(d + i * 16, o, 16);
+#endif
   }
 }
 
@@ -204,14 +250,20 @@
   }
 }
 
-__global__ __launch_bounds__(256) void k_zero_frame(uint8_t *img, unsigned w, unsigned h,
-                                                    size_t frame_bytes) {
+GS_DEV void zero_frame(uint8_t *f, unsigned w, unsigned h) {
   const unsigned i = blockIdx.x * 256u + threadIdx.x;
-  uint8_t *f = img + (size_t)blockIdx.y * frame_bytes;
   if (i < w) f[i] = 0;
   else if (i < 2 * w) f[(size_t)(h - 1) * w + (i - w)] = 0;
   else if (i < 2 * w + h) f[(size_t)(i - 2 * w) * w] = 0;
   else if (i < 2 * w + 2 * h) f[(size_t)(i - 2 * w - h) * w + (w - 1)] = 0;
+}
+__global__ __launch_bounds__(256) void k_zero_frame(uint8_t *img, unsigned w, unsigned h,
+                                                    size_t frame_bytes) {
+  zero_frame(img + (size_t)blockIdx.y * frame_bytes, w, h);
+}
+__global__ __launch_bounds__(256) void k_zero_frame_gated(uint8_t *img, unsigned w, unsigned h, size_t frame_bytes,
+                                                          const uint8_t *gate) {
+  if (gate[blockIdx.y]) zero_frame(img + (size_t)blockIdx.y * frame_bytes, w, h);
 }
 
 __global__ __launch_bounds__(256) void k_checksum(const uint8_t *img, size_t frame_bytes,
diff --git a/grayskull_amd/csrc/k_strip.h b/grayskull_amd/csrc/k_strip.h
--- a/grayskull_amd/csrc/k_strip.h
+++ b/grayskull_amd/csrc/k_strip.h
@@ -162,7 +162,7 @@
   GS_DEV U4 operator()(const U4 &o, int) const { return o; }
   GS_DEV void prefetch(int) {}
 };
-template <int RING, bool INVERT, bool EXITS = true, int RG = 0, class Body, class Fin = NoFin>
+template <int RING, bool INVERT, bool EXITS = true, int RG = 0, bool STORE = true, class Body, class Fin = NoFin>
 GS_DEV void strip_rows(const Strip<INVERT, RG> &S, int y0, int nrows, int lead, RawRow first, Body &&body,
                        Fin fin = Fin()) {
   RawRow raw = first;
@@ -181,7 +181,7 @@
       if constexpr (!EXITS) sched_fence();
       uint32_t U[12];
       S.unpack(raw, U);
-      S.store(y0 + i - 1, i > 0 && i <= nrows, fin(o_prev, y0 + i - 1));
+      if constexpr (STORE) S.store(y0 + i - 1, i > 0 && i <= nrows, fin(o_prev, y0 + i - 1));
 #if GS_STRIP_PF == 2
       raw = raw2, raw2 = S.load(y0 + i + lead + 2);
 #else
@@ -192,9 +192,13 @@
       o_prev = body(I, i, U);
     });
   }
+  if constexpr (!STORE) return;
   if constexpr (EXITS) S.store(y0 + nrows - 1, nrows > 0, fin(o_prev, y0 + nrows - 1));
   else S.store(y0 + base - 1, base == nrows && nrows > 0, fin(o_prev, y0 + base - 1));
 }
+
+GS_HD unsigned edge_code_lo(unsigned centre) { return centre < 7u ? 0u : centre - 7u > 240u ? 240u : centre - 7u; }
+
 
 GS_DEV void sobel_apairs(const uint32_t (&U)[12], uint32_t (&A)[10]) {
 #pragma unroll
diff --git a/grayskull_amd/csrc/prims.h b/grayskull_amd/csrc/prims.h
--- a/grayskull_amd/csrc/prims.h
+++ b/grayskull_amd/csrc/prims.h
@@ -127,6 +127,7 @@
   if (off < b.n) memcpy(b.base + off, &v, n);
 }
 GS_DEV void buf_store8(const BufRsrc &b, uint32_t off, uint32_t lo, uint32_t hi) { buf_store_n(b, off, lo | ((uint64_t)hi << 32), 8); }
+GS_DEV void buf_store8_nt(const BufRsrc &b, uint32_t off, uint32_t lo, uint32_t hi) { buf_store8(b, off, lo, hi); }
 GS_DEV void buf_store4(const BufRsrc &b, uint32_t off, uint32_t v) { buf_store_n(b, off, v, 4); }
 GS_DEV void buf_store2(const BufRsrc &b, uint32_t off, uint32_t v) { buf_store_n(b, off, v, 2); }
 GS_DEV void buf_store1(const BufRsrc &b, uint32_t off, uint32_t v) { buf_store_n(b, off, v, 1); }
@@ -286,6 +287,9 @@
 typedef unsigned int gs_u32x2 __attribute__((ext_vector_type(2)));
 GS_DEV void buf_store8(const BufRsrc &b, uint32_t off, uint32_t lo, uint32_t hi) {
   __builtin_amdgcn_raw_buffer_store_b64(gs_u32x2{lo, hi}, b.r, (int)off, 0, 0);
+}
+GS_DEV void buf_store8_nt(const BufRsrc &b, uint32_t off, uint32_t lo, uint32_t hi) {
+  __builtin_amdgcn_raw_buffer_store_b64(gs_u32x2{lo, hi}, b.r, (int)off, 0, GS_STORE_AUX);
 }
 GS_DEV void buf_store4(const BufRsrc &b, uint32_t off, uint32_t v) { __builtin_amdgcn_raw_buffer_store_b32(v, b.r, (int)off, 0, 0); }
 GS_DEV void buf_store2(const BufRsrc &b, uint32_t off, uint32_t v) { __builtin_amdgcn_raw_buffer_store_b16((unsigned short)v, b.r, (int)off, 0, 0); }
diff --git a/include/grayskull_hip.h b/include/grayskull_hip.h
--- a/include/grayskull_hip.h
+++ b/include/grayskull_hip.h
@@ -44,7 +44,8 @@
   GSH_TUNE_EXPERIMENT_23 = 23,
   GSH_TUNE_RETIRED_24 = 24,
   GSH_TUNE_GEOM_FORM = 25,
-  GSH_TUNE_TMATCH_CHUNK = 26
+  GSH_TUNE_TMATCH_CHUNK = 26,
+  GSH_TUNE_PIPELINE_FORM = 27
 };
 void gsh_tune(int key, int value);
 void gsh_profile(int on);
@@ -84,6 +85,7 @@
 
 void gsh_edge_pipeline_batch(uint8_t *dst, uint8_t *tmp, const uint8_t *src, unsigned w, unsigned h,
                              unsigned n, unsigned radius, unsigned *hist_scratch, uint8_t *thr);
+void gsh_edge_pipeline_stats(unsigned *coded, unsigned *fallback);
 
 void gsh_integral_batch(const uint8_t *src, unsigned w, unsigned h, unsigned n, unsigned *ii);
 
```

Result: slower. 1.367 million Mpix/s (-1.8%).
